# opensatelliteproject/xritdemod

Measured on AMD Instinct MI355X. Metric: Msamples/s in -> soft-symbols/s out (LRIT 293 ksym/s chain); % HBM roofline, higher is better.
Workload: dtype f32

## Files before the change

xritdemod_amd/csrc/clock.hip:

```cpp
#include "kernels.h"

#include <cstdlib>
#include <type_traits>
#include "scan.h"
#include "newton.h"

namespace xrit {

static_assert(CLK_CTL_DONE == NEWTON_CTL_DONE && CLK_CTL_GATED == NEWTON_CTL_GATED && CLK_CTL_TAKEOVER == NEWTON_CTL_TAKEOVER,
              "the words newton.h shares keep their numbers");

constexpr float CLK_H_T = 0.0625f;
constexpr float CLK_H_W = 1e-3f;

struct ClockResult {
    unsigned long long n_symbols;
    long long ii_final;
    int terminal_chain;
    int ok;
};

__global__ void __launch_bounds__(256) clock_om_kernel(const float2 *__restrict__ x, double2 *__restrict__ X,
                                                       long long N, int nb, double inv_sps)
{
    const int wave = threadIdx.x >> 6, lane = threadIdx.x & 63;
    const long long b = (long long)blockIdx.x * 4 + wave;
    if (b >= nb) return;
    float sr = 0.f, si = 0.f;
    for (int i = lane; i < CLK_OM_BLOCK; i += 64) {
        long long j = b * CLK_OM_BLOCK + i;
        if (j < N) {
            float2 v = x[j];
            float p = v.x * v.x + v.y * v.y;
            double ph = (double)j * inv_sps;
            ph -= floor(ph);
            float sn, cs;
            sincosf(-6.28318530717958647692f * (float)ph, &sn, &cs);
            sr += p * cs;
            si += p * sn;
        }
    }
    for (int off = 32; off > 0; off >>= 1) {
        sr += __shfl_down(sr, off, 64);
        si += __shfl_down(si, off, 64);
    }
    if (lane == 0) X[b] = make_double2((double)sr, (double)si);
}

__device__ __forceinline__ double clk_wrap(double x) { return x - 2.0 * XR_PI_D * rint(x / (2.0 * XR_PI_D)); }

struct ClkUnwrapF {
    typedef double T;
    const double2 *X;
    double *cnt;
    int nb;
    double sps;
    double off;
    int BL;
    double rot;
    __device__ T identity() const { return 0.0; }
    __device__ T combine(const T &lo, const T &hi) const { return lo + hi; }
    __device__ double ang(long long b) const
    {
        double sr = 0, si = 0;
        for (long long q = b - 2; q <= b + 2; ++q)
            if (q >= 0 && q < nb) { sr += X[q].x; si += X[q].y; }
        return atan2(si, sr);
    }
    __device__ T reduce_run(long long i0, int n) const
    {
        double s = 0, prev = i0 == 0 ? rot : ang(i0 - 1);
        for (int k = 0; k < n; ++k) {
            const double cur = ang(i0 + k);
            s += clk_wrap(cur - prev);
            prev = cur;
        }
        return s;
    }
    __device__ void apply_run(long long i0, int n, const T &pre) const
    {
        double s = pre, prev = i0 == 0 ? rot : ang(i0 - 1);
        for (int k = 0; k < n; ++k) {
            const double cur = ang(i0 + k);
            s += clk_wrap(cur - prev);
            prev = cur;
            double cb = off + ((double)(i0 + k) + 0.5) * BL;
            cnt[i0 + k] = (cb + s / (2.0 * XR_PI_D) * sps) / sps;
        }
    }
};

__device__ __forceinline__ double clk_count_at(const double *cnt, int nb, double sps, double t, double off, int BL)
{
    double fb = (t - off) / BL - 0.5;
    int b = (int)floor(fb);
    b = max(0, min(nb - 2, b));
    if (nb < 2) return cnt[0] + (t - off - 0.5 * BL) / sps;
    double c0 = cnt[b], c1 = cnt[b + 1];
    return c0 + (c1 - c0) * (fb - b);
}

__global__ void clock_guess_kernel(const double *__restrict__ cnt, int nb, double sps, ClockState *__restrict__ S,
                                   const ClockState *__restrict__ carried, int K, int NS, float omega0,
                                   const float2 *__restrict__ x, const float *__restrict__ table, long long ni,
                                   double off, int BL, int *__restrict__ dirty, int *__restrict__ ctl, int ctl_words,
                                   int *__restrict__ terminal, int *__restrict__ written)
{
    int k = blockIdx.x * blockDim.x + threadIdx.x;
    if (blockIdx.x == 0) {
        for (int i = threadIdx.x; i < ctl_words; i += blockDim.x) ctl[i] = 0;
        if (threadIdx.x == 0) *terminal = 0x7fffffff;
        __syncthreads();
    }
    if (k >= K) return;
    dirty[k] = 1;
    written[k] = 0;
    ClockState s0 = carried[0];
    if (k == 0) { S[0] = s0; ctl[CLK_CTL_GATED] = 1; return; }
    double t0 = (double)s0.ii + (double)s0.mu;
    double ca = clk_count_at(cnt, nb, sps, t0, off, BL) + 3.0 / sps;
    double target = rint(ca) + (double)k * NS;
    double t = (target - cnt[0]) * sps + off + 0.5 * BL;
    for (int it = 0; it < 4; ++it) {
        double c = clk_count_at(cnt, nb, sps, t, off, BL);
        t += (target - c) * sps;
    }
    t -= 3.0;
    if (t < 0) t = 0;
    ClockState s;
    s.ii = (long long)floor(t);
    s.mu = (float)(t - floor(t));
    s.omega = omega0;
    s.p0 = cf32{0.f, 0.f}; s.p1 = cf32{0.f, 0.f};
    s.c0 = cf32{0.f, 0.f}; s.c1 = cf32{0.f, 0.f};
    for (int back = 2; back >= 1; --back) {
        double tb = t - back * (double)omega0;
        if (tb < 0) continue;
        long long ib = (long long)floor(tb);
        if (ib >= ni) continue;
        float mub = (float)(tb - floor(tb));
        int imu = (int)rintf(mub * (float)XR_MM_NSTEPS);
        const float *row = table + imu * XR_MM_NTAPS;
        float ar = 0.f, ai = 0.f;
        for (int q = 0; q < XR_MM_NTAPS; ++q) {
            float2 v = x[ib + q];
            ar += row[XR_MM_NTAPS - 1 - q] * v.x;
            ai += row[XR_MM_NTAPS - 1 - q] * v.y;
        }
        s.p1 = s.p0; s.c1 = s.c0;
        s.p0 = cf32{ar, ai};
        s.c0 = cf32{ar > 0.f ? 1.f : 0.f, ai > 0.f ? 1.f : 0.f};
    }
    S[k] = s;
}

struct ClockPolicy {
    ClockState *S;
    const ClockState *E;
    const float4 *J;
    int *dirty;
    const int *nrun;
    unsigned *cnt;
    float trust_t, trust_w, tol_t, tol_w;
    int min_passes;
    const float4 *jmean;
    float floor_sq;
    int relay_after;

    struct Elem { ClockState e, s; float4 j; int nrun; };
    __device__ float4 jac_of(long long k) const { return jmean ? jmean[0] : J[k]; }
    __device__ Elem fetch(long long k) const { return Elem{E[k], S[k + 1], jac_of(k), nrun[k]}; }
    __device__ bool active(const Elem &el) const { return el.nrun > 0; }
    __device__ void residual(const Elem &el, float &r1, float &r2, int &aux) const
    {
        float rt = clock_tdiff(el.e, el.s);
        float m = rintf(rt / el.e.omega);
        r1 = rt - m * el.e.omega;
        r2 = el.e.omega - el.s.omega;
        aux = (int)m;
    }
    __device__ float4 jac(const Elem &el) const
    {
        float4 j = el.j;
        if (!(fabsf(j.x) < 4.f) || !(fabsf(j.y) < 16384.f) || !(fabsf(j.z) < 1.f) || !(fabsf(j.w) < 4.f))
            j = make_float4(0.f, 0.f, 0.f, 0.f);
        return j;
    }
    __device__ bool outside_trust(float d1, float d2) const
    {
        return !(fabsf(d1) <= trust_t) || !(fabsf(d2) <= trust_w);
    }
    __device__ bool distrust(float r1, float) const { return !(fabsf(r1) <= 0.5f); }
    __device__ void update(long long k, const Elem &el, float j1, float j2, float n1, float n2, int slip, int slip_k,
                           float r1, NewtonStat &st) const
    {
        const ClockState ek = el.e, old = el.s;
        const bool hist_same = ek.p0.x == old.p0.x && ek.p0.y == old.p0.y && ek.p1.x == old.p1.x &&
                               ek.p1.y == old.p1.y && ek.c0.x == old.c0.x && ek.c0.y == old.c0.y &&
                               ek.c1.x == old.c1.x && ek.c1.y == old.c1.y;
        if (!active(el)) {
            const bool same = old.ii == ek.ii && old.mu == ek.mu && old.omega == ek.omega && hist_same;
            if (!same) { S[k + 1] = ek; dirty[k + 1] = 1; st.changed += 1; }
            return;
        }
        const bool frozen = fabsf(n1) <= tol_t && fabsf(n2) <= tol_w && slip == 0 && slip_k == 0 && hist_same;
        if (frozen) return;
        ClockState nw = ek;
        clock_shift(nw, (float)slip * ek.omega + j1);
        nw.omega = ek.omega + j2;
        if (nw.ii < 0) { nw.ii = 0; nw.mu = 0.f; }
        st.open_ += 1;
        st.max_r = fmaxf(st.max_r, fabsf(r1));
        if (fabsf(r1) > 0.02f || slip_k != 0) st.large += 1;
        st.sum_sq += newton_fix(r1 * r1);
        const bool same = old.ii == nw.ii && old.mu == nw.mu && old.omega == nw.omega && hist_same;
        if (!same) { S[k + 1] = nw; dirty[k + 1] = 1; st.changed += 1; }
    }
    __device__ void decide(int *ctl) const
    {
        const unsigned changed = newton_cnt_load(cnt + CLK_CNT_CHANGED), open_ = newton_cnt_load(cnt + CLK_CNT_OPEN);
        const unsigned mr = newton_cnt_load(cnt + CLK_CNT_MAX_R), large = newton_cnt_load(cnt + CLK_CNT_LARGE);
        const unsigned long long sq = (unsigned long long)newton_cnt_load(cnt + CLK_CNT_SUM_SQ) |
                                      ((unsigned long long)newton_cnt_load(cnt + CLK_CNT_SUM_SQ + 1) << 32);
        ctl[CLK_CTL_PASSES] += 1;
        ctl[CLK_CTL_OPEN] = (int)open_;
        ctl[CLK_CTL_MAX_RESIDUAL] = (int)mr;
        const float q = newton_unfix(sq);
        const float q_prev = ctl[CLK_CTL_PASSES] == 1 ? INFINITY : __int_as_float(ctl[CLK_CTL_SUM_SQ]);
        ctl[CLK_CTL_SUM_SQ] = __float_as_int(q);
        ctl[CLK_CTL_GATED] = (large != 0 || __uint_as_float(mr) > 0.02f) ? 1 : 0;
        ctl[CLK_CTL_LARGE] = (int)large;
        const int open_prev = ctl[CLK_CTL_PASSES] == 1 ? 0x7fffffff : ctl[CLK_CTL_OPEN_LAST];
        ctl[CLK_CTL_OPEN_LAST] = (int)open_;
        if (changed == 0) { ctl[CLK_CTL_DONE] = 1; ctl[CLK_CTL_OPEN] = 0; return; }
        if (relay_after > 0 && ctl[CLK_CTL_PASSES] >= relay_after && large == 0 && !(__uint_as_float(mr) > 0.02f)) { ctl[CLK_CTL_DONE] = 1; return; }
        int memo = ctl[CLK_CTL_STALL_MEMO];
        if (ctl[CLK_CTL_PASSES] >= 3 && large != 0) memo |= 0x100;
        const bool acquiring = (memo & 0x100) != 0;
        const bool above_floor = open_ != 0u && (acquiring || q > floor_sq * (float)open_);
        const bool freezing = above_floor && open_prev != 0x7fffffff && (long long)open_prev - (long long)open_ >= 1 &&
                              200ll * ((long long)open_prev - (long long)open_) >= (long long)open_prev;
        const bool flat = q > 0.55f * q_prev;
        const int flat_runs = flat ? (memo & 0xff) + 1 : 0;
        ctl[CLK_CTL_STALL_MEMO] = (memo & 0x100) | (flat_runs > 0xff ? 0xff : flat_runs);
        const bool stalled = !freezing && (open_ >= 4096u ? flat : flat_runs >= 2);
        if (ctl[CLK_CTL_PASSES] >= min_passes && large == 0 && stalled) ctl[CLK_CTL_DONE] = 1;
    }
};

#ifndef XR_NOSTORE
#define XR_NOSTORE 0
#endif
#ifndef XR_LOAD_AUX
#define XR_LOAD_AUX 0
#endif

struct ClockTile {
    float *table;
    int *wb;
    float2 *tile;
    float2 *dump;
};

__device__ __forceinline__ ClockTile clock_tile_carve(char *smem, int grp, int ngroups, int WS)
{
    ClockTile t;
    t.table = reinterpret_cast<float *>(smem);
    t.wb = reinterpret_cast<int *>(smem + 4160) + 64 * grp;
    float2 *tiles = reinterpret_cast<float2 *>(smem + 4160 + 256 * ngroups);
    t.tile = tiles + (size_t)grp * 64 * WS;
    t.dump = tiles + (size_t)ngroups * 64 * WS + threadIdx.x;
    return t;
}

struct ClockSrc {
    __amdgpu_buffer_rsrc_t rsrc;
    int omin;
};
__device__ __forceinline__ ClockSrc clock_src(const float2 *x, long long N, int omin)
{
    ClockSrc c;
    omin = __builtin_amdgcn_readfirstlane(omin);
    c.omin = omin;
    const long long left = (N - (long long)omin) * 8;
    const unsigned bytes = left <= 0 ? 0u : (left > 0xffffffffLL ? 0xffffffffu : (unsigned)left);
    c.rsrc = __builtin_amdgcn_make_buffer_rsrc((void *)(x + omin), 0, bytes, 0x00020000);
    return c;
}

template <int NV, int IT> struct ClockFill {
    unsigned gb[IT];
    int lc[IT];
    typedef unsigned v2u __attribute__((ext_vector_type(2)));
    v2u v[IT];
    __device__ __forceinline__ void prepare(const int *origin, int nc, int WS, int omin)
    {
        const int lane = threadIdx.x & 63, wave = NV > 1 ? threadIdx.x >> 6 : 0;
        const int magic = 65536 / nc + 1;
#pragma unroll
        for (int it = 0; it < IT; ++it) {
            const int e = (it * NV + wave) * 64 + lane;
            const int row = (e * magic) >> 16, col = e - row * nc;
            const bool ok = row < 64 && origin[min(row, 63)] >= 0;
            gb[it] = ok ? (unsigned)(origin[min(row, 63)] - omin + col) * 8u : 0u;
            lc[it] = ok ? ((row * WS) << 8) | col : -1;
        }
    }
    __device__ __forceinline__ void issue(int first, const ClockSrc &src)
    {
#pragma unroll
        for (int it = 0; it < IT; ++it) v[it] = __builtin_amdgcn_raw_buffer_load_b64(src.rsrc, gb[it], first * 8, XR_LOAD_AUX);
    }
    template <int R> __device__ __forceinline__ void commit(float2 *tile, float2 *dump, int first, int ncol) const
    {
#pragma unroll
        for (int it = 0; it < IT; ++it) {
            const bool ok = (unsigned)(lc[it] & 255) < (unsigned)ncol && lc[it] >= 0;
            const int slot = (first + lc[it]) & (R - 1);
            float2 *p = tile + (lc[it] >> 8) + slot;
            const float2 val = make_float2(__uint_as_float(v[it].x), __uint_as_float(v[it].y));
            *(ok ? p : dump) = val;
            if (CLK_MIR > 0) *((ok && slot < CLK_MIR) ? p + R : dump) = val;
        }
    }
};

__device__ __forceinline__ int clock_cum(int jj, int STEP) { return (int)(((long long)jj * STEP) >> 16); }

template <int R>
__device__ __forceinline__ cf32 clock_step_ring(const cf32 *row, int &off, const float *table, ClockState &s,
                                                const ClockPar &par)
{
    cf32 wl[XR_MM_NTAPS];
    const cf32 *w = row + (off & (R - 1));
    if (CLK_MIR == 0) {
#pragma unroll
        for (int k = 0; k < XR_MM_NTAPS; ++k) wl[k] = row[(off + k) & (R - 1)];
        w = wl;
    }
    ClockState t = s;
    t.ii = 0;
    cf32 p = clock_step_w(w, table, t, par);
    off += (int)t.ii;
    t.ii = s.ii;
    s = t;
    return p;
}

__device__ __forceinline__ void clock_table_to_lds(float *dst, const float *__restrict__ src)
{
    constexpr int NEL = (XR_MM_NSTEPS + 1) * XR_MM_NTAPS;
    constexpr int NIT = (NEL + 63) / 64;
    const int nthr = blockDim.x;
    float tv[NIT];
#pragma unroll
    for (int q = 0; q < NIT; ++q) tv[q] = src[min((int)threadIdx.x + q * nthr, NEL - 1)];
#pragma unroll
    for (int q = 0; q < NIT; ++q) {
        const int i = (int)threadIdx.x + q * nthr;
        if (i < NEL) dst[i] = tv[q];
    }
}

}
#include "clock_relay.h"
namespace xrit {
struct ClockResult;
__device__ __forceinline__ double clk_count_at(const double *cnt, int nb, double sps, double t, double off, int BL);
}
#include "clock_overlap.h"
#ifdef XRIT_EXPERIMENTS
#include "../../experiments/csrc/clock_relay_wide.h"
#else
namespace xrit { constexpr int RW_REC_PAD = 0; }
#endif
namespace xrit {

__device__ __forceinline__ void clock_put(cf32 &d, const cf32 &p) { d = p; }
__device__ __forceinline__ void clock_put(float &d, const cf32 &p) { d = p.x; }

template <int WP, bool OUT, typename OutT>
__device__ __forceinline__ void clock_substep(const ClockTile &t, const float2 *__restrict__ x, int WS, int lane,
                                              int origin, int cum, int lim, int SS, int A, long long ni,
                                              const ClockPar &par, ClockState &s, int &off, bool &alive,
                                              int &produced, OutT *orow)
{
    const int rel = off - cum;
    const bool safe = !alive || (lim == SS && rel >= 0 && rel + A + XR_MM_NTAPS <= WP &&
                                 (long long)origin + off + A < ni);
    if (__all(safe)) {
        if (alive) {
            const cf32 *rowp = reinterpret_cast<const cf32 *>(t.tile + lane * WS);
            if (SS == 4) {
#pragma unroll
                for (int i = 0; i < 4; ++i) {
                    cf32 p = clock_step_ring<WP>(rowp, off, t.table, s, par);
                    if (OUT) clock_put(orow[i], p);
                }
            } else {
                for (int i = 0; i < SS; ++i) {
                    cf32 p = clock_step_ring<WP>(rowp, off, t.table, s, par);
                    if (OUT) {
#pragma unroll
                        for (int q = 0; q < 4; ++q)
                            if (q == i) clock_put(orow[q], p);
                    }
                }
            }
            s.ii = (long long)origin + off;
            produced += SS;
        }
    } else {
        for (int i = 0; i < lim; ++i) {
            if (alive && (s.ii >= ni || s.ii < 0)) alive = false;
            if (alive) {
                cf32 p = clock_step_w(reinterpret_cast<const cf32 *>(x) + s.ii, t.table, s, par);
                if (OUT) {
#pragma unroll
                    for (int q = 0; q < 4; ++q)
                        if (q == i) clock_put(orow[q], p);
                }
                ++produced;
            }
        }
        off = (int)(s.ii - origin);
    }
}

template <int NV> __device__ __forceinline__ void clock_tile_barrier()
{
    if (NV > 1) lds_barrier();
    else __builtin_amdgcn_wave_barrier();
}

template <int NV, int WP, int IT, typename Compute>
__device__ __forceinline__ void clock_pipeline(const ClockTile &t, const ClockSrc &src, int WS, int nsub, int STEP,
                                               Compute &&compute)
{
    {
        ClockFill<NV, (WP + NV - 1) / NV> w;
        w.prepare(t.wb, WP, WS, src.omin);
        w.issue(0, src);
        w.template commit<WP>(t.tile, t.dump, 0, WP);
    }
    const int nc = (STEP >> 16) + 1;
    if constexpr (IT * NV > 32) {
        ClockFill<NV, IT> f;
        f.prepare(t.wb, nc, WS, src.omin);
        clock_tile_barrier<NV>();
        int c0 = 0;
        for (int j = 0; j < nsub; ++j) {
            const int c1 = clock_cum(j + 1, STEP);
            if (j + 1 < nsub) f.issue(c0 + WP, src);
            compute(j, c0);
            clock_tile_barrier<NV>();
            if (j + 1 < nsub) f.template commit<WP>(t.tile, t.dump, c0 + WP, c1 - c0);
            clock_tile_barrier<NV>();
            c0 = c1;
        }
        return;
    }
    ClockFill<NV, IT> f0, f1;
    f0.prepare(t.wb, nc, WS, src.omin);
#pragma unroll
    for (int it = 0; it < IT; ++it) { f1.gb[it] = f0.gb[it]; f1.lc[it] = f0.lc[it]; }
    clock_tile_barrier<NV>();
    int c0 = 0, c1 = clock_cum(1, STEP);
    if (nsub > 1) f1.issue(c0 + WP, src);
    for (int j = 0; j < nsub; j += 2) {
        const int c2 = clock_cum(j + 2, STEP), c3 = clock_cum(j + 3, STEP);
        if (j + 2 < nsub) f0.issue(c1 + WP, src);
        compute(j, c0);
        clock_tile_barrier<NV>();
        if (j + 1 < nsub) f1.template commit<WP>(t.tile, t.dump, c0 + WP, c1 - c0);
        clock_tile_barrier<NV>();
        if (j + 1 >= nsub) break;
        if (j + 3 < nsub) f1.issue(c2 + WP, src);
        compute(j + 1, c1);
        clock_tile_barrier<NV>();
        if (j + 2 < nsub) f0.template commit<WP>(t.tile, t.dump, c1 + WP, c2 - c1);
        clock_tile_barrier<NV>();
        c0 = c2;
        c1 = c3;
    }
}

__device__ __forceinline__ int clock_origin_min(const int *wb)
{
    int o = wb[threadIdx.x & 63];
    o = o < 0 ? 0x7fffffff : o;
    for (int off = 32; off > 0; off >>= 1) o = min(o, __shfl_xor(o, off, 64));
    return o == 0x7fffffff ? 0 : o;
}

struct ClockPassOut {
    float *soft;
    float2 *sym;
    unsigned long long cap;
    int *valid;
    int *written;
    float4 *stage;
};

template <int NV, int WP, int NCM, bool OUTP = false>
__global__ void __launch_bounds__(NV > 1 ? 64 * NV : 512) clock_pass_kernel(const float2 *__restrict__ x, const float *__restrict__ table_g,
                                                             const ClockState *__restrict__ S, ClockState *__restrict__ E,
                                                             float4 *__restrict__ J, int *__restrict__ dirty,
                                                             int *__restrict__ nrun, long long N, long long ni, int K,
                                                             int NS, ClockPar par, int SS, int W, int WS, int A,
                                                             int STEP, const int *__restrict__ ctl, ClockPolicy pol,
                                                             AffMap *__restrict__ aggs, ClockPassOut po = ClockPassOut{})
{
    if (ctl[CLK_CTL_DONE] || (aggs != nullptr && ctl[CLK_CTL_TAKEOVER])) return;
    if (OUTP && blockIdx.x == 0 && threadIdx.x == 0) *po.valid = 1;
    extern __shared__ __attribute__((aligned(16))) char smem[];
    __shared__ float2 endv[2][NV > 1 ? 64 : 1];
    __shared__ long long ref_ii[NV > 1 ? 64 : 1];
    __shared__ int any_run;
    const int ngroups = NV > 1 ? 1 : (int)(blockDim.x >> 6);
    const int variant = NV > 1 ? threadIdx.x >> 6 : 0, grp = NV > 1 ? 0 : threadIdx.x >> 6, lane = threadIdx.x & 63;
    const ClockTile t = clock_tile_carve(smem, grp, ngroups, WS);
    const int wv = blockIdx.x * ngroups + grp;
    const int k = wv * 64 + lane;
    bool run = k < K;
    if (run) run = dirty[k] != 0 || (OUTP && po.written[k] == 0);
    if (threadIdx.x == 0) any_run = 0;
    __syncthreads();
    if (run && variant == 0) any_run = 1;
    clock_table_to_lds(t.table, table_g);
    __syncthreads();
    if (!any_run && aggs == nullptr) return;
    ClockState s{};
    int produced = 0;
    float4 jk = make_float4(0.f, 0.f, 0.f, 0.f);
    const bool walk = NV > 1 ? any_run != 0 : __any(run);
    if (walk) {
        bool alive = run;
        if (run) {
            s = S[k];
            if (NV > 1 && variant == 1) clock_shift(s, CLK_H_T);
            if (NV > 1 && variant == 2) s.omega += CLK_H_W;
        }
        if (variant == 0) t.wb[lane] = alive ? max((int)s.ii - CLK_M, 0) : -1;
        if (NV > 1) __syncthreads();
        else __builtin_amdgcn_wave_barrier();
        const int origin = t.wb[lane];
        int off = (int)(s.ii - origin);
        const int nsub = (NS + SS - 1) / SS;
        const ClockSrc src = clock_src(x, N, clock_origin_min(t.wb));
        const unsigned long long obase = (unsigned long long)k * NS;
        clock_pipeline<NV, WP, (NCM + NV - 1) / NV>(t, src, WS, nsub, STEP, [&](int j, int cum) {
            if (!OUTP) {
                clock_substep<WP, false>(t, x, WS, lane, origin, cum, min(SS, NS - j * SS), SS, A, ni, par, s, off, alive,
                                         produced, (float *)nullptr);
                return;
            }
            cf32 ps[4];
#pragma unroll
            for (int i = 0; i < 4; ++i) ps[i] = cf32{0.f, 0.f};
            const int before = produced;
            clock_substep<WP, true>(t, x, WS, lane, origin, cum, min(SS, NS - j * SS), SS, A, ni, par, s, off, alive,
                                    produced, ps);
            const int nv = produced - before;
            const unsigned long long o = obase + (unsigned long long)j * SS;
            if (po.soft && run) po.stage[((size_t)wv * nsub + j) * 64 + lane] = make_float4(ps[0].x, ps[1].x, ps[2].x, ps[3].x);
            if (nv == 4 && (NS & 3) == 0 && o + 3 < po.cap) {
                if (po.sym) {
                    *reinterpret_cast<float4 *>(po.sym + o) = make_float4(ps[0].x, ps[0].y, ps[1].x, ps[1].y);
                    *reinterpret_cast<float4 *>(po.sym + o + 2) = make_float4(ps[2].x, ps[2].y, ps[3].x, ps[3].y);
                }
            } else {
#pragma unroll
                for (int i = 0; i < 4; ++i) {
                    if (i < nv && o + i < po.cap) {
                        if (po.sym) po.sym[o + i] = make_float2(ps[i].x, ps[i].y);
                    }
                }
            }
        });
        if (NV > 1) {
            if (variant == 0) ref_ii[lane] = s.ii;
            __syncthreads();
            if (variant > 0) endv[variant - 1][lane] = make_float2((float)(s.ii - ref_ii[lane]) + s.mu, s.omega);
            __syncthreads();
        }
        if (variant == 0 && run) {
            if (NV > 1) {
                float2 et = endv[0][lane], ew = endv[1][lane];
                float tb = s.mu;
                jk.x = (et.x - tb) / CLK_H_T;
                jk.y = (ew.x - tb) / CLK_H_W;
                jk.z = (et.y - s.omega) / CLK_H_T;
                jk.w = (ew.y - s.omega) / CLK_H_W;
                J[k] = jk;
            }
            E[k] = s;
            nrun[k] = produced;
            dirty[k] = 0;
            if (OUTP) po.written[k] = 1;
        }
    }
    if (aggs == nullptr || variant != 0 || wv * 64 >= K) return;
    AffMap e = aff_identity();
    if (k < K - 1) {
        ClockPolicy::Elem el;
        el.s = S[k + 1];
        if (run) {
            el.e = s;
            el.nrun = produced;
            el.j = NV > 1 ? jk : pol.jac_of(k);
        } else {
            el.e = E[k];
            el.nrun = nrun[k];
            el.j = pol.jac_of(k);
        }
        e = newton_element(pol, el, false);
    }
    newton_wave_aggregate(e, wv, aggs);
}

template <int WP, int NCM, bool SYM>
__global__ void __launch_bounds__(512) clock_output_kernel(const float2 *__restrict__ x, const float *__restrict__ table_g,
                                                          const ClockState *__restrict__ S, ClockState *__restrict__ E,
                                                          int *__restrict__ counts, float *__restrict__ soft,
                                                          float2 *__restrict__ sym, unsigned long long cap, long long N,
                                                          long long ni, int K, int NS, ClockPar par,
                                                          int *__restrict__ terminal, int SS, int W, int WS, int A,
                                                          int STEP, const int *__restrict__ ctl)
{
    if (ctl[CLK_CTL_SYMBOLS]) return;
    extern __shared__ __attribute__((aligned(16))) char smem[];
    const int ngroups = (int)(blockDim.x >> 6), grp = threadIdx.x >> 6, lane = threadIdx.x & 63;
    const ClockTile t = clock_tile_carve(smem, grp, ngroups, WS);
    clock_table_to_lds(t.table, table_g);
    __syncthreads();
    const int k = (blockIdx.x * ngroups + grp) * 64 + lane;
    const bool mine = k < K;
    if (!__any(mine)) return;
    ClockState s{};
    if (mine) s = S[k];
    int produced = 0;
    bool alive = mine;
    t.wb[lane] = alive ? max((int)s.ii - CLK_M, 0) : -1;
    __builtin_amdgcn_wave_barrier();
    const int origin = t.wb[lane];
    int off = (int)(s.ii - origin);
    const int nsub = (NS + SS - 1) / SS;
    const ClockSrc src = clock_src(x, N, clock_origin_min(t.wb));
    const unsigned long long obase = (unsigned long long)k * NS;
    clock_pipeline<1, WP, NCM>(t, src, WS, nsub, STEP, [&](int j, int cum) {
        cf32 ps[4];
#pragma unroll
        for (int i = 0; i < 4; ++i) ps[i] = cf32{0.f, 0.f};
        const int before = produced;
        clock_substep<WP, true>(t, x, WS, lane, origin, cum, min(SS, NS - j * SS), SS, A, ni, par, s, off, alive,
                                produced, ps);
        const int nv = produced - before;
        const unsigned long long o = obase + (unsigned long long)j * SS;
        if (nv == 4 && (NS & 3) == 0 && SS == 4 && o + 3 < cap) {
            if (soft && !XR_NOSTORE) *reinterpret_cast<float4 *>(soft + o) = make_float4(ps[0].x, ps[1].x, ps[2].x, ps[3].x);
            if (SYM && sym) {
                *reinterpret_cast<float4 *>(sym + o) = make_float4(ps[0].x, ps[0].y, ps[1].x, ps[1].y);
                *reinterpret_cast<float4 *>(sym + o + 2) = make_float4(ps[2].x, ps[2].y, ps[3].x, ps[3].y);
            }
        } else {
#pragma unroll
            for (int i = 0; i < 4; ++i) {
                if (i < nv && o + i < cap) {
                    if (soft) soft[o + i] = ps[i].x;
                    if (SYM && sym) sym[o + i] = make_float2(ps[i].x, ps[i].y);
                }
            }
        }
    });
    if (!mine) return;
    E[k] = s;
    counts[k] = produced;
    if (produced < NS) atomicMin(terminal, k);
}

constexpr int CLK_STAGE_MAX_NS = 512;
__global__ void __launch_bounds__(256) clock_unstage_kernel(const float4 *__restrict__ stage, float *__restrict__ soft,
                                                            const int *__restrict__ nrun, const int *__restrict__ ctl,
                                                            unsigned long long cap, int K, int NS)
{
    if (!ctl[CLK_CTL_SYMBOLS]) return;
    extern __shared__ __attribute__((aligned(16))) char smem[];
    float *tile = reinterpret_cast<float *>(smem);
    int *cnt = reinterpret_cast<int *>(tile + 64 * (NS + 1));
    const int wv = blockIdx.x, nsub = NS / 4;
    if (threadIdx.x < 64) cnt[threadIdx.x] = wv * 64 + (int)threadIdx.x < K ? nrun[wv * 64 + threadIdx.x] : 0;
    for (int e = threadIdx.x; e < nsub * 64; e += 256) {
        const float4 v = stage[(size_t)wv * nsub * 64 + e];
        const int j = e >> 6, c = e & 63;
        float *row = tile + c * (NS + 1) + 4 * j;
        row[0] = v.x; row[1] = v.y; row[2] = v.z; row[3] = v.w;
    }
    __syncthreads();
    const unsigned long long base = (unsigned long long)wv * 64 * NS;
    for (int e = threadIdx.x; e < 64 * NS; e += 256) {
        const int c = e / NS, i = e - c * NS;
        if (i < cnt[c] && base + e < cap) soft[base + e] = tile[c * (NS + 1) + i];
    }
}

__global__ void __launch_bounds__(256) clock_terminal_kernel(const int *__restrict__ nrun, const int *__restrict__ ctl,
                                                             int *__restrict__ terminal, int K, int NS)
{
    if (!ctl[CLK_CTL_SYMBOLS]) return;
    const int k = blockIdx.x * 256 + threadIdx.x;
    const bool short_ = k < K && nrun[k] < NS;
    const unsigned long long m = __ballot(short_);
    if (m && (threadIdx.x & 63) == 0) atomicMin(terminal, k + __builtin_ctzll(m));
}

__global__ void __launch_bounds__(1024) clock_finalize_kernel(const ClockState *__restrict__ E,
                                                              const int *__restrict__ counts_out,
                                                              const int *__restrict__ nrun,
                                                              const int *__restrict__ terminal,
                                                              const int *__restrict__ ctl,
                                                              const ClockState *__restrict__ carried_in,
                                                              ClockState *__restrict__ carried_out,
                                                              ClockResult *__restrict__ res,
                                                              const float2 *__restrict__ x,
                                                              float2 *__restrict__ tail_out, long long N, int K, int NS)
{
    __shared__ long long s_ii;
    const int *counts = ctl[CLK_CTL_SYMBOLS] ? nrun : counts_out;
    if (threadIdx.x == 0) {
        int k = *terminal;
        ClockState s;
        if (k < 0 || k >= K) {
            res->ok = 0;
            res->n_symbols = 0;
            res->terminal_chain = -1;
            s = carried_in[0];
        } else {
            res->ok = 1;
            res->terminal_chain = k;
            res->n_symbols = (unsigned long long)k * NS + (unsigned long long)counts[k];
            s = E[k];
        }
        long long ii = s.ii;
        if (ii > N) ii = N;
        if (ii < 0) ii = 0;
        res->ii_final = ii;
        s_ii = ii;
        s.ii = 0;
        carried_out[0] = s;
    }
    __syncthreads();
    const long long ii = s_ii;
    const long long carry = N - ii;
    if (threadIdx.x < carry) tail_out[threadIdx.x] = x[ii + threadIdx.x];
}

__global__ void __launch_bounds__(1024) clock_tail_kernel(const float2 *__restrict__ tail, float2 *__restrict__ x, int carry)
{
    if ((int)threadIdx.x < carry) x[threadIdx.x] = tail[threadIdx.x];
}

constexpr int CLK_SER_W = 2048;

__global__ void __launch_bounds__(64) clock_serial_kernel(const float2 *__restrict__ x, const float *__restrict__ table_g,
                                                          const ClockState *__restrict__ carried_in,
                                                          ClockState *__restrict__ carried_out,
                                                          ClockResult *__restrict__ res, float *__restrict__ soft,
                                                          float2 *__restrict__ sym, unsigned long long cap, long long N,
                                                          long long ni, ClockPar par, float2 *__restrict__ tail_out)
{
    __shared__ float table[(XR_MM_NSTEPS + 1) * XR_MM_NTAPS];
    __shared__ cf32 win[CLK_SER_W];
    clock_table_to_lds(table, table_g);
    const int lane = threadIdx.x;
    ClockState s = carried_in[0];
    long long base = -(long long)CLK_SER_W;
    unsigned long long oo = 0;
    __syncthreads();
    while (s.ii < ni && s.ii >= 0 && oo < cap) {
        if (s.ii < base || s.ii + XR_MM_NTAPS > base + CLK_SER_W) {
            __syncthreads();
            base = s.ii;
            for (int i = lane; i < CLK_SER_W; i += 64) {
                const long long j = base + i;
                const float2 v = x[j < N ? j : N - 1];
                win[i] = cf32{v.x, v.y};
            }
            __syncthreads();
        }
        ClockState t = s;
        t.ii = 0;
        const cf32 p = clock_step_w(win + (int)(s.ii - base), table, t, par);
        s.ii += t.ii;
        t.ii = s.ii;
        s = t;
        if (lane == 0) {
            if (soft) soft[oo] = p.x;
            if (sym) sym[oo] = make_float2(p.x, p.y);
        }
        ++oo;
    }
    long long ii = s.ii;
    if (ii > N) ii = N;
    if (ii < 0) ii = 0;
    if (lane == 0) {
        res->ok = (s.ii >= ni || s.ii < 0) ? 1 : 0;
        res->terminal_chain = 0;
        res->n_symbols = oo;
        res->ii_final = ii;
        ClockState c = s;
        c.ii = 0;
        carried_out[0] = c;
    }
    const long long carry = N - ii;
    for (long long i = lane; i < carry && i < 1024; i += 64) tail_out[i] = x[ii + i];
}


__global__ void clk_fill_int_kernel(int *p, int v, int n)
{
    int i = blockIdx.x * blockDim.x + threadIdx.x;
    if (i < n) p[i] = v;
}

__global__ void __launch_bounds__(256) clock_reset_kernel(unsigned *counters, int words, int *terminal)
{
    for (int i = threadIdx.x; i < words; i += 256) counters[i] = 0u;
    if (threadIdx.x == 0 && terminal) *terminal = 0x7fffffff;
}

__global__ void __launch_bounds__(256) clock_jmean_kernel(const float4 *__restrict__ J, int K, float4 *__restrict__ out)
{
    __shared__ double acc[4][256];
    __shared__ int cnt[256];
    const int k0 = K / 8, k1 = K - K / 8;
    double a = 0, b = 0, c = 0, d = 0;
    int n = 0;
    for (int k = k0 + (int)threadIdx.x; k < k1; k += 256) {
        const float4 j = J[k];
        if (fabsf(j.x) < 4.f && fabsf(j.y) < 16384.f && fabsf(j.z) < 1.f && fabsf(j.w) < 4.f) {
            a += j.x; b += j.y; c += j.z; d += j.w;
            ++n;
        }
    }
    acc[0][threadIdx.x] = a; acc[1][threadIdx.x] = b; acc[2][threadIdx.x] = c; acc[3][threadIdx.x] = d;
    cnt[threadIdx.x] = n;
    __syncthreads();
    for (int off = 128; off > 0; off >>= 1) {
        if ((int)threadIdx.x < off) {
            for (int q = 0; q < 4; ++q) acc[q][threadIdx.x] += acc[q][threadIdx.x + off];
            cnt[threadIdx.x] += cnt[threadIdx.x + off];
        }
        __syncthreads();
    }
    if (threadIdx.x == 0) {
        const double inv = cnt[0] > 0 ? 1.0 / cnt[0] : 0.0;
        out[0] = make_float4((float)(acc[0][0] * inv), (float)(acc[1][0] * inv), (float)(acc[2][0] * inv), (float)(acc[3][0] * inv));
        reinterpret_cast<int *>(out + 1)[0] = cnt[0];
    }
}

int ClockStage::init(float omega, float gain_omega, float mu, float gain_mu, float omega_rel_limit, int chain_syms,
                     int max_passes_)
{
    sps = omega;
    par.omega_mid = omega;
    par.omega_lim = omega * omega_rel_limit;
    par.gain_omega = gain_omega;
    par.gain_mu = gain_mu;
    mu0 = mu;
    NS = chain_syms > 0 ? (chain_syms < 32 ? 32 : chain_syms) : 64;
    auto_ns = chain_syms <= 0;
    max_passes = max_passes_ > 0 ? max_passes_ : 192;
    min_passes = max_passes < 4 ? max_passes : 4;
    std::vector<float> tb((XR_MM_NSTEPS + 1) * XR_MM_NTAPS);
    design_mmse_table(tb.data());
    XR_TRY(table.reserve(tb.size() * sizeof(float)));
    XR_HIP(hipMemcpy(table.p, tb.data(), tb.size() * sizeof(float), hipMemcpyHostToDevice));
    XR_TRY(st.reserve(2 * sizeof(ClockState)));
    ClockState s0{};
    s0.ii = 0; s0.mu = mu; s0.omega = omega;
    ClockState both[2] = {s0, s0};
    XR_HIP(hipMemcpy(st.p, both, sizeof both, hipMemcpyHostToDevice));
    XR_TRY(tail.reserve(2 * 1024 * sizeof(float2)));
    XR_TRY(jmean.reserve(64));
    jmean_valid = false;
    XR_TRY(counters.reserve((size_t)(max_passes + 12) * 8 * sizeof(unsigned)));
    XR_HIP(hipHostMalloc((void **)&h_res, 128));
    {
        int dev = 0, v = 0;
        XR_HIP(hipGetDevice(&dev));
        if (hipDeviceGetAttribute(&v, hipDeviceAttributeMultiprocessorCount, dev) == hipSuccess && v > 0) cu_count = v;
        if (hipDeviceGetAttribute(&v, hipDeviceAttributeMaxSharedMemoryPerMultiprocessor, dev) == hipSuccess && v >= 65536)
            lds_per_cu = v;
    }
    ov_enabled = getenv("XRIT_NO_OVERLAP") == nullptr;
    if (const char *e = getenv("XRIT_OV_HIST")) { const int v = atoi(e); if (v >= 1024) ov_hist = v; }
#ifdef XRIT_EXPERIMENTS
    if (const char *e = getenv("XRIT_OV_MIN")) { const long long v = atoll(e); if (v > 0) ov_min = v; }
    if (const char *e = getenv("XRIT_OV_SMALL_RING")) ov_small_ring = atoi(e) != 0;
    if (const char *e = getenv("XRIT_OV_MINL")) { const int v = atoi(e); if (v >= 1024) ov_min_range = v; }
    if (const char *e = getenv("XRIT_OV_MINW")) { const int v = atoi(e); if (v >= 1) ov_min_walkers = v; }
    if (const char *e = getenv("XRIT_OV_LRATIO")) { const double v = atof(e); if (v >= 0.125 && v <= 16.0) ov_lratio = v; }
#endif
    {
        ov_pad_need = clock_ov_pad_need(*this);
        xpad = clock_xpad(*this);
        XR_TRY(ov_claim.reserve(RELAY_CLAIM_WORDS * sizeof(unsigned)));
        XR_HIP(hipMemset(ov_claim.p, 0, RELAY_CLAIM_WORDS * sizeof(unsigned)));
        for (auto &j : ov)
            if (hipEventCreateWithFlags(&j.ev_walk, hipEventDisableTiming) != hipSuccess ||
                hipEventCreateWithFlags(&j.ev_guess, hipEventDisableTiming) != hipSuccess) { set_error("hipEventCreate failed"); return XRIT_E_HIP; }
    }
    force_gated = getenv("XRIT_GATED_SOLVE") != nullptr;
    relay_global = getenv("XRIT_RELAY_GLOBAL") != nullptr;
    trace_env = getenv("XRIT_TRACE") != nullptr;
#ifdef XRIT_EXPERIMENTS
    if (const char *e = getenv("XRIT_NO_HANDOFF")) relay_no_handoff = atoi(e) != 0 ? 1 : 0;
    if (const char *e = getenv("XRIT_RELAY_WAVES")) relay_waves = atoi(e);
    if (const char *e = getenv("XRIT_RELAY_TEAMS")) relay_teams_per_cu = atoi(e) > 0 ? atoi(e) : 1;
    relay_no_rec = getenv("XRIT_RELAY_NO_REC") != nullptr;
    relay_no_claim = getenv("XRIT_RELAY_NO_CLAIM") != nullptr;
    if (const char *e = getenv("XRIT_RELAY_REC01")) relay_rec01 = atoi(e) != 0;
    if (const char *e = getenv("XRIT_RELAY_APX")) { int a0 = -1, a1 = -1; if (sscanf(e, "%d,%d", &a0, &a1) >= 1) { relay_apx_cfg[0] = a0; relay_apx_cfg[1] = a1; } }
    if (const char *e = getenv("XRIT_AUTO_PASSES")) auto_passes = atoi(e);
    if (const char *e = getenv("XRIT_AUTO_LONG_SEG")) auto_long_seg = atoi(e);
    if (const char *e = getenv("XRIT_RELAY_PER_CU")) { relay_per_cu = atoi(e) > 0 ? atoi(e) : 3; relay_per_cu_set = true; }
    no_meanj = getenv("XRIT_NO_MEANJ") != nullptr;
    pass_writes = getenv("XRIT_NO_PASS_OUTPUT") == nullptr;
    ng_max = getenv("XRIT_CLOCK_NG") ? atoi(getenv("XRIT_CLOCK_NG")) : 8;
#endif
    return XRIT_OK;
}

__global__ void clock_state_reset_kernel(ClockState *st, float mu, float omega)
{
    ClockState s{};
    s.ii = 0; s.mu = mu; s.omega = omega;
    st[0] = s;
    st[1] = s;
}

int ClockStage::reset(hipStream_t s)
{
    hipLaunchKernelGGL(clock_state_reset_kernel, dim3(1), dim3(1), 0, s, st.as<ClockState>(), mu0, par.omega_mid);
    jobs.reset();
    if (ov_claim.p) (void)hipMemsetAsync(ov_claim.p, 0, RELAY_CLAIM_WORDS * sizeof(unsigned), s);
    passes = 0;
    last_passes = -1;
    batch = 7;
    relay_batch = 96;
    jmean_valid = false;
    last_symbols = 0;
    return XRIT_OK;
}

void ClockStage::release()
{
#ifdef XRIT_RELAY_TIMING
    if (getenv("XRIT_WALKER_PHASES")) {
        unsigned long long hd[16] = {0}, z[16] = {0};
        if (hipDeviceSynchronize() == hipSuccess && hipMemcpyFromSymbol(hd, HIP_SYMBOL(relay_dbg), sizeof hd) == hipSuccess && hd[6]) {
            (void)hipMemcpyToSymbol(HIP_SYMBOL(relay_dbg), z, sizeof z);
            const double st = (double)hd[6];
            fprintf(stderr, "[xrit] overlap walkers over the handle's life, cycles per step: ring wait %.0f, setup %.0f, guess rounds %.0f, literal step + verdict %.0f, "
                            "stage + commit %.0f, loop %.0f; sum %.0f (%llu steps; the ring's fill level read %.3f times per step, %.3f sleeps per step)\n", hd[0] / st, hd[1] / st, hd[2] / st, hd[3] / st, hd[4] / st,
                    hd[5] / st, (hd[0] + hd[1] + hd[2] + hd[3] + hd[4] + hd[5]) / st, hd[6], hd[7] / st, hd[8] / st);
        }
    }
#endif
    for (auto &b : xbuf) b.release();
    for (auto &j : ov) {
        j.om.release(); j.om_work.release(); j.segs.release(); j.S.release(); j.stage.release(); j.aux.release();
        if (j.ev_walk) (void)hipEventDestroy(j.ev_walk);
        if (j.ev_guess) (void)hipEventDestroy(j.ev_guess);
        j.ev_walk = nullptr; j.ev_guess = nullptr;
    }
    ov_claim.release();
    table.release(); st.release(); S.release(); E.release(); J.release(); om.release();
    work.release(); counters.release(); sym.release(); dlin.release(); flags.release(); tail.release(); wsolve.release(); jmean.release();
    relay.release(); relay_rec.release(); alt.release(); stage.release(); om_work.release();
    if (h_res) (void)hipHostFree(h_res);
    h_res = nullptr;
}

double2 *ClockStage::om_slot(int nb, int BL)
{
    const int owner = jobs.om_owner();
    DevBuf &buf = owner >= 0 ? ov[owner].om : om;
    if (nb < 1 || buf.reserve((size_t)nb * (sizeof(double2) + sizeof(double))) != XRIT_OK) return nullptr;
    jobs.om_noted(nb, BL);
    return buf.as<double2>();
}

static int clock_unwrap(DevBuf &buf, DevBuf &wk, int nb, int BL, double sps, hipStream_t s)
{
    const int nbB = scan_blocks(nb);
    XR_TRY(wk.reserve((size_t)(nbB + 2) * sizeof(double)));
    double2 *X = buf.as<double2>();
    double *cnt = reinterpret_cast<double *>(buf.as<char>() + (size_t)nb * sizeof(double2));
    ClkUnwrapF uf{X, cnt, nb, sps, 0.0, BL, 0.0};
    hipLaunchKernelGGL(scan_reduce_kernel<ClkUnwrapF>, dim3(nbB), dim3(SCAN_BLOCK), 0, s, uf, (long long)nb, wk.as<double>());
    hipLaunchKernelGGL(scan_apply_lookback_kernel<ClkUnwrapF>, dim3(nbB), dim3(SCAN_BLOCK), 0, s, uf, (long long)nb, wk.as<double>());
    XR_HIP(hipGetLastError());
    return XRIT_OK;
}

int ClockStage::om_scan(hipStream_t s)
{
    if (!jobs.om_scan_here()) return XRIT_OK;
    XR_TRY(clock_unwrap(om, om_work, jobs.om_nb, jobs.om_BL, (double)sps, s));
    jobs.om_scan_done();
    return XRIT_OK;
}

int ClockStage::input_slot(size_t n, float2 **slot, hipStream_t s)
{
    const ClockSlotPick p = jobs.pick_buffer();
    if (p.b < 0) { set_error("%s", p.err); return XRIT_E_INVALID; }
    for (int q = 0; q < NXB; ++q)
        if (p.wait_guess[q]) XR_HIP(hipStreamWaitEvent(s, ov[q].ev_guess, 0));
    if (p.forget) jobs.hist.forget();
    XR_TRY(xbuf[p.b].reserve((xpad + n + 64 + 16) * sizeof(float2)));
    *slot = xbuf[p.b].as<float2>() + xpad;
    jobs.hand_out(p.b, n, ov_eligible(n));
    return XRIT_OK;
}

static inline int *clock_ctl(const DevBuf &b) { return b.as<int>(); }
static inline ClockResult *clock_res(const DevBuf &b) { return reinterpret_cast<ClockResult *>(b.as<unsigned>() + CLK_RES_WORD); }
static inline unsigned *clock_cnt(const DevBuf &b, int pass) { return b.as<unsigned>() + CLK_CTL_WORDS + (size_t)pass * CLK_CNT_WORDS; }

template <typename KernelT> static void clock_allow_lds(KernelT kernel, size_t bytes)
{
    if (bytes > 48 * 1024)
        (void)hipFuncSetAttribute(reinterpret_cast<const void *>(kernel), hipFuncAttributeMaxDynamicSharedMemorySize, (int)bytes);
}

__global__ void __launch_bounds__(256) clock_relay_finalize_kernel(const RelaySeg *__restrict__ e0,
                                                                    const RelaySeg *__restrict__ e1,
                                                                    const unsigned *__restrict__ changed, int enq, int G,
                                                                    int Lseg, const ClockState *__restrict__ carried_in,
                                                                    ClockState *__restrict__ carried_out,
                                                                    ClockResult *__restrict__ res,
                                                                    const float2 *__restrict__ x,
                                                                    float2 *__restrict__ tail_out, long long N, int *ctl, int force,
                                                                    const unsigned long long *__restrict__ moments)
{
    if (!ctl[CLK_CTL_DONE] && !force) return;
    __shared__ int s_term, s_buf, s_stuck;
    __shared__ long long s_ii;
    if (threadIdx.x == 0) {
        int ran = enq, closed = 0;
        for (int p = 0; p < enq; ++p)
            if (changed[RELAY_STAT * p + RELAY_STAT_CHANGED] == 0u) { ran = p + 1; closed = 1; break; }
        ctl[CLK_CTL_RELAY_PASSES] = ran;
        ctl[CLK_CTL_RELAY_CLOSED] = closed;
        {
            const unsigned *c = changed + RELAY_STAT * (ran - 1);
            const unsigned long long sq = (unsigned long long)c[RELAY_STAT_MOVE_SQ] | ((unsigned long long)c[RELAY_STAT_MOVE_SQ + 1] << 32);
            ctl[CLK_CTL_RELAY_SHIFT_SQ] = __float_as_int(c[RELAY_STAT_MOVED] ? (float)((double)sq / 1099511627776.0 / (double)c[RELAY_STAT_MOVED]) : 0.0f);
            ctl[CLK_CTL_RELAY_MOVE_MAX] = (int)(c[RELAY_STAT_MOVE_MAX] >= 0x80000000u ? 0x7f800000u : c[RELAY_STAT_MOVE_MAX]);
        }
        s_buf = (ran - 1) & 1;
        s_term = 0x7fffffff;
        s_stuck = 0;
    }
    __syncthreads();
    const RelaySeg *e = s_buf ? e1 : e0;
    for (int i = threadIdx.x; i < G; i += (int)blockDim.x) {
        if (e[i].flags & RELAY_EXHAUSTED) atomicMin(&s_term, i);
        if (e[i].flags & RELAY_STUCK) s_stuck = 1;
    }
    __syncthreads();
    if (threadIdx.x == 0) {
        ClockState s;
        const int k = s_stuck ? G : s_term;
        ctl[CLK_CTL_STUCK] = s_stuck;
        if (k >= G) {
            res->ok = 0;
            res->n_symbols = 0;
            res->terminal_chain = -1;
            s = carried_in[0];
        } else {
            res->ok = 1;
            res->terminal_chain = k;
            res->n_symbols = (unsigned long long)k * (unsigned long long)Lseg + (unsigned long long)e[k].n_done;
            s = e[k].s;
        }
        {
            const double nsym = res->ok ? (double)res->n_symbols : 0.0;
            const double a1 = nsym > 0 ? (double)moments[0] / 1048576.0 / nsym : 0.0, a2 = nsym > 0 ? (double)moments[1] / 1048576.0 / nsym : 0.0;
            const double var = a2 - a1 * a1;
            ctl[CLK_CTL_SNR2] = __float_as_int(nsym > 0 && var > 0 ? (float)(a1 * a1 / var) : 1e30f);
        }
        long long ii = s.ii;
        if (ii > N) ii = N;
        if (ii < 0) ii = 0;
        res->ii_final = ii;
        s_ii = ii;
        s.ii = 0;
        carried_out[0] = s;
    }
    __syncthreads();
    const long long ii = s_ii;
    long long carry = N - ii;
    if (carry > 1024) {
        carry = 1024;
        if (threadIdx.x == 0) res->ok = 0;
    }
    for (long long i = threadIdx.x; i < carry; i += blockDim.x) tail_out[i] = x[ii + i];
}

int ClockStage::relay_w_plan() const
{
#ifdef XRIT_EXPERIMENTS
    if (!relay_global && relay_waves >= 2) {
        if (relay_waves >= 4 && relay_span(par, RW_OWN * 4) + 8 <= RelayWide<4>::MAX_SPAN) return 4;
        if (relay_span(par, RW_OWN * 2) + 8 <= RelayWide<2>::MAX_SPAN) return 2;
    }
#endif
    return 0;
}

int ClockStage::relay_cut()
{
    Job &j = job;
    j.cps = j.segs.cps;
    j.G = j.segs.G;
    XR_TRY(relay.reserve((size_t)j.G * 3 * sizeof(RelaySeg) + ((size_t)j.G + 1 + 8) * RELAY_STAT * sizeof(unsigned) + 2 * sizeof(unsigned long long) +
                         RELAY_CLAIM_WORDS * sizeof(unsigned)));
    if (!relay_no_rec) XR_TRY(relay_rec.reserve(((size_t)j.G * j.cps * NS + RW_REC_PAD) * sizeof(unsigned)));
    relay_segments = j.G;
    relay_seg_chains = j.cps;
    return XRIT_OK;
}

int ClockStage::enqueue_relay(int count, bool restart, hipStream_t s, Profiler *prof)
{
    Job &j = job;
    const int limit = clock_relay_limit(j.G, j.relay_budget);
    RelaySeg *segs = relay.as<RelaySeg>();
    unsigned *changed = reinterpret_cast<unsigned *>(segs + 3 * (size_t)j.G);
    RelayArgs a{};
    a.x = xbase(); a.table = table.as<float>(); a.N = j.N; a.ni = j.ni;
    a.first = st.as<ClockState>() + jobs.cur; a.S = S.as<ClockState>();
    a.K = j.K; a.cps = j.cps; a.NS = NS; a.G = j.G;
    a.start = segs; a.ends[0] = segs + j.G; a.ends[1] = segs + 2 * (size_t)j.G;
    const ClockLattice lat = clock_lattice(par.omega_mid);
    a.q_om = lat.q_om; a.q_mu = lat.q_mu;
    a.soft = j.soft; a.sym = j.sym; a.cap = (unsigned long long)j.cap; a.par = par;
    a.changed = changed; a.ctl = j.relay_force ? nullptr : clock_ctl(counters);
    a.rec = relay_no_rec ? nullptr : relay_rec.as<unsigned>();
    a.moments = reinterpret_cast<unsigned long long *>(changed + ((size_t)j.G + 1 + 8) * RELAY_STAT);
    a.simd_claim = relay_no_claim ? nullptr : reinterpret_cast<unsigned *>(a.moments + 2);

    if (restart) {
        j.relay_enq = 0;
        const int words = RELAY_STAT * (j.G + 3) > RELAY_CLAIM_WORDS ? RELAY_STAT * (j.G + 3) : RELAY_CLAIM_WORDS;
        hipLaunchKernelGGL(clock_relay_init_kernel, dim3(div_up((size_t)words, 256)), dim3(256), 0, s, segs, j.G, changed,
                           j.G + 3, clock_ctl(counters), a.moments, a.simd_claim);
    }
    const int span = relay_span(par, 64);
    const bool lds_walk = relay_ring_ok(par) && !relay_global;
    {
        ProfScope ps(prof, "clock_relay", s);
        for (int q = 0; q < count && j.relay_enq < limit; ++q, ++j.relay_enq) {
            const int apx = j.relay_enq < 2 ? j.relay_apx[j.relay_enq] : 0;
            a.sym_skip = j.no_handoff && j.relay_enq == 0 && limit >= 2 && !apx;
            a.rec_write = relay_rec01 || !(j.no_handoff && j.relay_enq == 0);
            a.rec_use = (relay_rec01 || !(j.no_handoff && j.relay_enq == 1)) ? 3 : 0;
#ifdef XRIT_EXPERIMENTS
#define XR_RELAY_WIDE(WV)                                                                                             \
    do {                                                                                                              \
        const int wspan = relay_span(par, RW_OWN * WV);                                                               \
        if (j.sym) hipLaunchKernelGGL((clock_relay_wide_kernel<true, WV>), dim3(j.G), dim3(64 * WV), 0, s, a, j.relay_enq, wspan);       \
        else hipLaunchKernelGGL((clock_relay_wide_kernel<false, WV>), dim3(j.G), dim3(64 * WV), 0, s, a, j.relay_enq, wspan);            \
    } while (0)
            if (j.relay_w == 4) XR_RELAY_WIDE(4);
            else if (j.relay_w == 2) XR_RELAY_WIDE(2);
            else
#undef XR_RELAY_WIDE
#endif
            if (lds_walk && j.sym) hipLaunchKernelGGL((clock_relay_kernel<true, true>), dim3(j.G), dim3(128), 0, s, a, j.relay_enq, span, apx);
            else if (lds_walk) hipLaunchKernelGGL((clock_relay_kernel<false, true>), dim3(j.G), dim3(128), 0, s, a, j.relay_enq, span, apx);
            else if (j.sym) hipLaunchKernelGGL((clock_relay_kernel<true, false>), dim3(j.G), dim3(64), 0, s, a, j.relay_enq, span, apx);
            else hipLaunchKernelGGL((clock_relay_kernel<false, false>), dim3(j.G), dim3(64), 0, s, a, j.relay_enq, span, apx);
        }
        hipLaunchKernelGGL(clock_relay_finalize_kernel, dim3(1), dim3(64), 0, s, a.ends[0], a.ends[1], changed,
                           j.relay_enq, j.G, j.cps * NS, st.as<ClockState>() + jobs.cur, st.as<ClockState>() + (jobs.cur ^ 1),
                           clock_res(counters), a.x, tail.as<float2>() + 1024 * (jobs.cur ^ 1), j.N, clock_ctl(counters), j.relay_force ? 1 : 0,
                           a.moments);
    }
    XR_HIP(hipGetLastError());
    XR_HIP(hipMemcpyAsync(h_res, counters.p, CLK_CTL_WORDS * sizeof(unsigned), hipMemcpyDeviceToHost, s));
    return XRIT_OK;
}

int ClockStage::enqueue_passes(int count, hipStream_t s, Profiler *prof)
{
    const Job &j = job;
    ClockPolicy pol{S.as<ClockState>(), E.as<ClockState>(), J.as<float4>(), j.dirty, j.nrun, nullptr,
                    0.75f, 0.01f, tol_t, tol_w, min_passes, j.mean_j ? jmean.as<float4>() : nullptr,
                    9e-8f * (sps > 4.2534f ? (sps / 4.2534f) * (sps / 4.2534f) : 1.0f),
                    j.relay && (long long)j.cps * NS >= 2048 ? 2 : 0};
    const unsigned nw = div_up((size_t)j.K, 64);
    const float2 *x = xbase();
    const bool wave = !job.gated;
    AffMap *aggs = wave ? wsolve.as<AffMap>() : nullptr;
    NewtonStat *wslots = reinterpret_cast<NewtonStat *>(wsolve.as<AffMap>() + nw + 1);
    for (int q = 0; q < count && job.enqueued < max_passes; ++q, ++job.enqueued) {
        const int p = job.enqueued;
        pol.cnt = clock_cnt(counters, p);
        const bool jac = p < jac_passes && !j.mean_j;
        {
            ProfScope ps(prof, jac ? "clock_pass_jac" : "clock_pass", s);
#define XR_CLK_PASS(NV, WPV, NCM, OUTV)                                                                               \
    do {                                                                                                              \
        const size_t lds = NV > 1 ? j.tile_bytes3 : j.tile_bytes;                                                     \
        clock_allow_lds(clock_pass_kernel<NV, WPV, NCM, OUTV>, lds);                                                  \
        hipLaunchKernelGGL((clock_pass_kernel<NV, WPV, NCM, OUTV>), dim3(NV > 1 ? nw : div_up(nw, j.NG)),             \
                           dim3(NV > 1 ? 64 * NV : 64 * j.NG), lds, s, x, table.as<float>(), S.as<ClockState>(),      \
                           E.as<ClockState>(), J.as<float4>(), j.dirty, j.nrun, j.N, j.ni, j.K, NS, par, j.SS, j.W,   \
                           j.WS, j.A, j.STEP, clock_ctl(counters), pol, aggs, po);                                    \
    } while (0)
#define XR_CLK_PASS_NV(NV, OUTV)                                                                                      \
    do {                                                                                                              \
        if (!j.wide && narrow) XR_CLK_PASS(NV, 32, 20, OUTV);                                                         \
        else if (!j.wide) XR_CLK_PASS(NV, 32, 32, OUTV);                                                              \
        else XR_CLK_PASS(NV, 64, 64, OUTV);                                                                           \
    } while (0)
            const bool narrow = (j.STEP >> 16) + 1 <= 20;
            const bool writes = !jac && !j.relay && p >= j.write_from && j.SS == 4 && (NS & 3) == 0 && NS <= CLK_STAGE_MAX_NS;
            const ClockPassOut po{j.soft, j.sym, (unsigned long long)j.cap, clock_ctl(counters) + CLK_CTL_SYMBOLS, j.written,
                                  stage.as<float4>()};
            if (jac) XR_CLK_PASS_NV(3, false);
            else if (writes) XR_CLK_PASS_NV(1, true);
            else XR_CLK_PASS_NV(1, false);
#undef XR_CLK_PASS_NV
#undef XR_CLK_PASS
        }
        {
            ProfScope ps(prof, "clock_solve", s);
            if (wave) {
                newton_apply_waves(pol, (long long)j.K - 1, aggs, clock_ctl(counters), wslots, s);
            } else if (newton_solve(pol, (long long)j.K - 1, work.as<AffMap>(), dlin.as<float2>(), clock_ctl(counters), s) != 0) {
                set_error("clock hand-off: %d chains exceed the solver's block budget", j.K);
                return XRIT_E_INVALID;
            }
        }
    }
    XR_HIP(hipGetLastError());
    return XRIT_OK;
}

int ClockStage::enqueue_output(hipStream_t s, Profiler *prof, bool again)
{
    const Job &j = job;
    const float2 *x = xbase();
    const ClockState *st_in = st.as<ClockState>() + jobs.cur;
    ClockState *st_out = st.as<ClockState>() + (jobs.cur ^ 1);
    float2 *tail_out = tail.as<float2>() + 1024 * (jobs.cur ^ 1);
    const unsigned nw = div_up((size_t)j.K, 64);
    {
        ProfScope ps(prof, "clock_output", s);
        if (again) hipLaunchKernelGGL(clk_fill_int_kernel, dim3(1), dim3(1), 0, s, j.terminal, 0x7fffffff, 1);
#define XR_CLK_OUT_S(WPV, NCM, SYMV)                                                                                  \
    do {                                                                                                              \
        clock_allow_lds(clock_output_kernel<WPV, NCM, SYMV>, j.tile_bytes);                                           \
        hipLaunchKernelGGL((clock_output_kernel<WPV, NCM, SYMV>), dim3(div_up(nw, j.NG)), dim3(64 * j.NG),            \
                           j.tile_bytes, s, x, table.as<float>(), S.as<ClockState>(), E.as<ClockState>(), j.counts,   \
                           j.soft, j.sym, (unsigned long long)j.cap, j.N, j.ni, j.K, NS, par, j.terminal, j.SS, j.W,  \
                           j.WS, j.A, j.STEP, clock_ctl(counters));                                                   \
    } while (0)
#define XR_CLK_OUT(WPV, NCM)                              \
    do {                                                  \
        if (j.sym) XR_CLK_OUT_S(WPV, NCM, true);          \
        else XR_CLK_OUT_S(WPV, NCM, false);               \
    } while (0)
        const bool narrow = (j.STEP >> 16) + 1 <= 20;
        if (!j.wide && narrow) XR_CLK_OUT(32, 20);
        else if (!j.wide) XR_CLK_OUT(32, 32);
        else XR_CLK_OUT(64, 64);
#undef XR_CLK_OUT_S
#undef XR_CLK_OUT
        if (j.soft && j.SS == 4 && (NS & 3) == 0 && pass_writes && NS <= CLK_STAGE_MAX_NS) {
            const size_t lds = (size_t)64 * (NS + 1) * sizeof(float) + 64 * sizeof(int);
            clock_allow_lds(clock_unstage_kernel, lds);
            hipLaunchKernelGGL(clock_unstage_kernel, dim3(nw), dim3(256), lds, s, stage.as<float4>(), j.soft, j.nrun,
                               clock_ctl(counters), (unsigned long long)j.cap, j.K, NS);
        }
        hipLaunchKernelGGL(clock_terminal_kernel, dim3(div_up((size_t)j.K, 256)), dim3(256), 0, s, j.nrun, clock_ctl(counters),
                           j.terminal, j.K, NS);
        hipLaunchKernelGGL(clock_finalize_kernel, dim3(1), dim3(1024), 0, s, E.as<ClockState>(), j.counts, j.nrun, j.terminal,
                           clock_ctl(counters), st_in, st_out, clock_res(counters), x, tail_out, j.N, j.K, NS);
    }
    XR_HIP(hipGetLastError());
    XR_HIP(hipMemcpyAsync(h_res, counters.p, CLK_CTL_WORDS * sizeof(unsigned), hipMemcpyDeviceToHost, s));
    return XRIT_OK;
}


static inline unsigned *ov_stat(ClockStage::OvJob &d) { return d.aux.as<unsigned>(); }
static inline unsigned long long *ov_moments(ClockStage::OvJob &d) { return reinterpret_cast<unsigned long long *>(d.aux.as<unsigned>() + 8); }
static inline unsigned long long *ov_offs(ClockStage::OvJob &d) { return reinterpret_cast<unsigned long long *>(d.aux.as<char>() + 64); }
static inline int *ov_j0(ClockStage::OvJob &d, int G) { return reinterpret_cast<int *>(d.aux.as<char>() + 64 + (size_t)G * sizeof(unsigned long long)); }

int ClockStage::ov_launch(int job, hipStream_t sw, bool ahead, Profiler *prof)
{
    const ClockJob &j = jobs.job[job];
    OvJob &d = ov[job];
    const ClockLaunchHist h = jobs.launch_hist(job, ahead, ov_pad_need);
    if (h.err) { set_error("%s", h.err); return XRIT_E_INVALID; }
    if (h.wait_guess >= 0) XR_HIP(hipStreamWaitEvent(sw, ov[h.wait_guess].ev_guess, 0));
    size_t h_n = 0;
    {
        const ClockOvPlan plan = clock_ov_plan(*this, j.n, jobs.carry, h.have, ahead);
        if (plan.err[0]) { set_error("%s", plan.err); return XRIT_E_INVALID; }
        jobs.planned(job, plan, ahead);
        XR_TRY(d.segs.reserve((size_t)j.G * sizeof(OverlapSeg)));
        XR_TRY(d.S.reserve((size_t)j.G * sizeof(ClockState)));
        XR_TRY(d.stage.reserve((size_t)j.G * (size_t)j.stride * sizeof(float) + 256));
        XR_TRY(d.aux.reserve(64 + (size_t)j.G * sizeof(int) + 8 + (size_t)j.G * sizeof(unsigned long long)));
    }
    float2 *data = xbuf[job].as<float2>() + xpad;
    float2 *base = data - j.padN;
    if (!j.w0_carried) {
        if (const char *e = ClockJobs::hist_refusal(h, j)) { set_error("%s", e); return XRIT_E_INVALID; }
        h_n = jobs.job[h.job].n;
        const float2 *hend = xbuf[h.xb].as<float2>() + xpad + h_n;
        XR_HIP(hipMemcpyAsync(base, hend - j.padN, (size_t)j.padN * sizeof(float2), hipMemcpyDeviceToDevice, sw));
    } else if (j.padN > 0) {
        hipLaunchKernelGGL(clock_tail_kernel, dim3(1), dim3(1024), 0, sw, tail.as<float2>() + 1024 * jobs.cur, base, j.padN);
    }
    int nb = j.nb;
    const int BL = j.om_ext ? j.BL : CLK_OM_BLOCK;
    if (!j.om_ext) {
        nb = (int)((j.n + CLK_OM_BLOCK - 1) / CLK_OM_BLOCK);
        XR_TRY(d.om.reserve((size_t)nb * (sizeof(double2) + sizeof(double))));
        hipLaunchKernelGGL(clock_om_kernel, dim3(div_up((size_t)nb, 4)), dim3(256), 0, sw, data, d.om.as<double2>(), (long long)j.n, nb,
                           1.0 / (double)sps);
    }
    if (!j.om_scanned && nb >= 1) XR_TRY(clock_unwrap(d.om, d.om_work, nb, BL, (double)sps, sw));
    const double *cnt = reinterpret_cast<const double *>(d.om.as<char>() + (size_t)nb * sizeof(double2));
    const double *cnt_prev = nullptr;
    int nb_prev = 0;
    if (!j.w0_carried && h.job >= 0) {
        const ClockJob &p = jobs.job[h.job];
        cnt_prev = reinterpret_cast<const double *>(ov[h.job].om.as<char>() + (size_t)p.nb * sizeof(double2));
        nb_prev = p.nb;
        if (p.BL != BL) { set_error("clock recovery: timing curves of consecutive calls differ in their block length"); return XRIT_E_INVALID; }
    }
    OverlapArgs a{};
    a.x = base; a.table = table.as<float>(); a.N = j.N; a.ni = j.ni;
    a.start = d.S.as<ClockState>(); a.G = j.G; a.store0 = j.store0; a.first_bound = j.first_bound; a.Ls = j.Ls; a.early = j.early;
    a.stride = j.stride; a.stage = d.stage.as<float>(); a.segs = d.segs.as<OverlapSeg>(); a.par = par;
    const ClockLattice lat = clock_lattice(par.omega_mid);
    a.q_om = lat.q_om; a.q_mu = lat.q_mu;
    a.stat = ov_stat(d); a.moments = ov_moments(d); a.simd_claim = relay_no_claim ? nullptr : ov_claim.as<unsigned>();
    const int span = relay_span(par, 64);
    {
        ProfScope ps(prof, "clock_guess", sw);
        hipLaunchKernelGGL(clock_overlap_guess_kernel, dim3(div_up((size_t)j.G, 256)), dim3(256), 0, sw, cnt, nb, cnt_prev, nb_prev,
                           (long long)h_n, BL, (double)sps, par.omega_mid, base, table.as<float>(), j.ni, j.padN, j.hist, j.G, j.store0,
                           j.first_bound, j.Ls, st.as<ClockState>() + jobs.cur, j.w0_carried ? 1 : 0, j.w0_ii, 0, d.S.as<ClockState>(),
                           a.stat, a.moments);
    }
    XR_HIP(hipEventRecord(d.ev_guess, sw));
    {
        ProfScope ps(prof, "clock_overlap", sw);
        if (ov_small_ring && span + 8 <= 1024 - RELAY_XCH - 72) hipLaunchKernelGGL(clock_overlap_kernel<1024>, dim3(j.G), dim3(128), 0, sw, a, span);
        else hipLaunchKernelGGL(clock_overlap_kernel<RELAY_RX>, dim3(j.G), dim3(128), 0, sw, a, span);
    }
    XR_HIP(hipGetLastError());
    XR_HIP(hipEventRecord(d.ev_walk, sw));
    jobs.launched(job, h, nb, BL);
    return XRIT_OK;
}

int ClockStage::ov_restart(int job)
{
    if (jobs.restart_waits(job)) XR_HIP(hipEventSynchronize(ov[job].ev_walk));
    jobs.restarted(job);
    return XRIT_OK;
}

int ClockStage::ov_fallback(size_t *n_out, hipStream_t s, Profiler *prof, bool to_closure)
{
    const int job = jobs.overlap_fell_back();
    const int rc = run_chains(xbuf[job].as<float2>() + xpad - jobs.carry, to_closure ? 1 : 0, jobs.job[job].n, ov_soft, nullptr, ov_cap, n_out, s, prof);
    if (rc == XRIT_OK) jobs.ended_fallback(job);
    ov_fell_back = true;
    return rc;
}

int ClockStage::ov_finalize(int job, float *soft_out, size_t cap, hipStream_t s, Profiler *prof)
{
    const ClockJob &j = jobs.job[job];
    OvJob &d = ov[job];
    XR_HIP(hipStreamWaitEvent(s, d.ev_walk, 0));
    jobs.w0_known(job);
    {
        ProfScope ps(prof, "clock_joints", s);
        hipLaunchKernelGGL(clock_reset_kernel, dim3(1), dim3(256), 0, s, counters.as<unsigned>(), CLK_CTL_WORDS, (int *)nullptr);
        hipLaunchKernelGGL(clock_overlap_scan_kernel, dim3(1), dim3(256), 0, s, d.segs.as<OverlapSeg>(), j.G, j.stride,
                           st.as<ClockState>() + jobs.cur, j.w0_ii, j.w0_carried ? 1 : 0, par.omega_mid, ov_j0(d, j.G), ov_offs(d),
                           st.as<ClockState>() + (jobs.cur ^ 1), clock_res(counters), xbuf[job].as<float2>() + xpad - j.padN,
                           tail.as<float2>() + 1024 * (jobs.cur ^ 1), j.N, clock_ctl(counters), ov_moments(d), (unsigned long long)cap);
        if (soft_out)
            hipLaunchKernelGGL(clock_overlap_copy_kernel, dim3(div_up((size_t)j.stride, 1024), j.G), dim3(256), 0, s, d.stage.as<float>(),
                               d.segs.as<OverlapSeg>(), ov_j0(d, j.G), ov_offs(d), j.stride, soft_out, (unsigned long long)cap, clock_res(counters));
    }
    XR_HIP(hipGetLastError());
    XR_HIP(hipMemcpyAsync(h_res, counters.p, CLK_CTL_WORDS * sizeof(unsigned), hipMemcpyDeviceToHost, s));
    jobs.finalizing(job);
    return XRIT_OK;
}

void ClockStage::call_reset(size_t n)
{
    passes = 0;
    unconverged = 0;
    large_open = 0;
    max_residual = 0;
    ov_fell_back = false;
    jobs.call_reset(n);
}

int ClockStage::begin(size_t n, float *soft_out, float2 *sym_out, size_t cap, hipStream_t s, Profiler *prof)
{
    call_reset(n);
    if (const char *e = jobs.call_job(n, sym_out != nullptr)) { set_error("%s", e); return XRIT_E_INVALID; }
    if (jobs.ov_cur >= 0) return begin_overlap(n, soft_out, cap, s, prof);
    return begin_chains(nullptr, exact, n, soft_out, sym_out, cap, s, prof);
}

int ClockStage::begin_overlap(size_t n, float *soft_out, size_t cap, hipStream_t s, Profiler *prof)
{
    job = Job{};
    job.n = n; job.soft = soft_out; job.cap = cap; job.exact = exact;
    jobs.begun_overlap();
    ov_soft = soft_out; ov_cap = cap;
    const int q = jobs.ov_cur;
    if (jobs.job[q].state == CLK_JOB_SLOT) XR_TRY(ov_launch(q, s, false, prof));
    return ov_finalize(q, soft_out, cap, s, prof);
}

int ClockStage::begin_chains(float2 *base, int exact_, size_t n, float *soft_out, float2 *sym_out, size_t cap, hipStream_t s, Profiler *prof)
{
    ClockKnobs k = *this;
    k.exact = exact_;
    const int relay_w = relay_w_plan();
    job = Job{};
    Job &j = job;
    static_cast<ClockChainPlan &>(j) = clock_chain_plan(k, n, jobs.carry, last_passes, relay_w);
    j.n = n; j.soft = soft_out; j.sym = sym_out; j.cap = cap; j.base = base; j.exact = exact_; j.relay_w = relay_w;
    if (j.N >= (1LL << 31)) { set_error("%s", j.err); return XRIT_E_INVALID; }
    jobs.chains_buffer(!base);
    if (!base) XR_TRY(xbuf[jobs.xb].reserve((size_t)(xpad + n + 64 + 16) * sizeof(float2)));
    const ClockOm om_in = jobs.begun_chains();
    if (jobs.carry)
        hipLaunchKernelGGL(clock_tail_kernel, dim3(1), dim3(1024), 0, s, tail.as<float2>() + 1024 * jobs.cur, xbase(), (int)jobs.carry);
    if (j.err[0]) { set_error("%s", j.err); return XRIT_E_INVALID; }
    if (j.short_input) return begin_short(s);
    if (serial) return begin_serial(s, prof);
    NS = j.NS;
    return launch_chains(om_in.ext, om_in.scanned, s, prof);
}

int ClockStage::begin_short(hipStream_t s)
{
    const Job &j = job;
    if (j.N > 0)
        XR_HIP(hipMemcpyAsync(tail.as<float2>() + 1024 * (jobs.cur ^ 1), xbase(), (size_t)j.N * sizeof(float2),
                              hipMemcpyDeviceToDevice, s));
    XR_HIP(hipMemcpyAsync(st.as<ClockState>() + (jobs.cur ^ 1), st.as<ClockState>() + jobs.cur, sizeof(ClockState),
                          hipMemcpyDeviceToDevice, s));
    return XRIT_OK;
}

int ClockStage::begin_serial(hipStream_t s, Profiler *prof)
{
    const Job &j = job;
    hipLaunchKernelGGL(clock_reset_kernel, dim3(1), dim3(256), 0, s, counters.as<unsigned>(), CLK_CTL_WORDS, (int *)nullptr);
    {
        ProfScope ps(prof, "clock_serial", s);
        hipLaunchKernelGGL(clock_serial_kernel, dim3(1), dim3(64), 0, s, xbase(), table.as<float>(),
                           st.as<ClockState>() + jobs.cur, st.as<ClockState>() + (jobs.cur ^ 1), clock_res(counters), j.soft,
                           j.sym, (unsigned long long)j.cap, j.N, j.ni, par, tail.as<float2>() + 1024 * (jobs.cur ^ 1));
    }
    XR_HIP(hipGetLastError());
    XR_HIP(hipMemcpyAsync(h_res, counters.p, CLK_CTL_WORDS * sizeof(unsigned), hipMemcpyDeviceToHost, s));
    return XRIT_OK;
}

int ClockStage::launch_chains(bool ext, bool scanned, hipStream_t s, Profiler *prof)
{
    Job &j = job;
    const int K = j.K;
    float2 *x = xbase();
    const int BL = ext ? jobs.om_BL : CLK_OM_BLOCK;
    const double om_off = ext ? (double)jobs.carry : 0.0;
    const int nb = ext ? jobs.om_nb : (int)((j.N + CLK_OM_BLOCK - 1) / CLK_OM_BLOCK);
    XR_TRY(S.reserve((size_t)K * sizeof(ClockState)));
    XR_TRY(E.reserve((size_t)K * sizeof(ClockState)));
    XR_TRY(J.reserve((size_t)K * sizeof(float4)));
    XR_TRY(flags.reserve((size_t)(4 * K + 4) * sizeof(int)));
    if (pass_writes) XR_TRY(stage.reserve(((size_t)div_up((size_t)K, 64) * 64 * NS + 64) * sizeof(float)));
    XR_TRY(om.reserve((size_t)nb * (sizeof(double2) + sizeof(double))));
    const int nbK = scan_blocks(K), nbB = scan_blocks(nb);
    const int nbmax = nbK > nbB ? nbK : nbB;
    XR_TRY(dlin.reserve((size_t)(K + 1) * sizeof(float2)));
    const int nbN = newton_blocks(K) > nbmax ? newton_blocks(K) : nbmax;
    XR_TRY(work.reserve((size_t)(3 * nbN + 8) * sizeof(AffMap)));
    {
        const size_t nw = div_up((size_t)K, 64);
        XR_TRY(wsolve.reserve(newton_waves_bytes(nw)));
        j.gated = force_gated;
        j.mean_j = jmean_valid && jmean_ns == NS && K >= 256 && !force_gated && !no_meanj;
    }
    if (j.relay) XR_TRY(relay_cut());
    j.dirty = flags.as<int>();
    j.counts = flags.as<int>() + K;
    j.nrun = flags.as<int>() + 2 * K;
    j.terminal = flags.as<int>() + 3 * K;
    j.written = flags.as<int>() + 3 * K + 4;
    double2 *X = om.as<double2>();
    double *cnt = reinterpret_cast<double *>(om.as<char>() + (size_t)nb * sizeof(double2));
    const ClockState *st_in = st.as<ClockState>() + jobs.cur;
    if (K <= 1) hipLaunchKernelGGL(clock_reset_kernel, dim3(1), dim3(256), 0, s, counters.as<unsigned>(), (max_passes + 5) * 8, j.terminal);
    if (K > 1) {
        {
            ProfScope ps(prof, "clock_guess", s);
            if (!ext)
                hipLaunchKernelGGL(clock_om_kernel, dim3(div_up((size_t)nb, 4)), dim3(256), 0, s, x, X, j.N, nb,
                                   1.0 / (double)sps);
            if (!scanned) XR_TRY(clock_unwrap(om, work, nb, BL, (double)sps, s));
            hipLaunchKernelGGL(clock_guess_kernel, dim3(div_up((size_t)K, 256)), dim3(256), 0, s, cnt, nb, (double)sps,
                               S.as<ClockState>(), st_in, K, NS, par.omega_mid, x, table.as<float>(), j.ni, om_off, BL, j.dirty,
                               clock_ctl(counters), (max_passes + 5) * 8, j.terminal, j.written);
        }
        if (j.no_handoff) j.relay_force = true;
        else XR_TRY(enqueue_passes(batch < max_passes ? batch : max_passes, s, prof));
    } else {
        XR_HIP(hipMemcpyAsync(S.p, st_in, sizeof(ClockState), hipMemcpyDeviceToDevice, s));
    }
    if (j.relay && K > 1) {
        if (before_relay) XR_TRY(before_relay(0));
        int rc_relay = enqueue_relay(relay_batch, true, s, prof);
        if (rc_relay == XRIT_OK && before_relay) rc_relay = before_relay(1);
        return rc_relay;
    }
    return enqueue_output(s, prof);
}

bool ClockStage::closed() const
{
    if (job.short_input || job.K <= 1 || job.no_handoff) return true;
    return reinterpret_cast<const int *>(h_res)[CLK_CTL_DONE] != 0;
}

int ClockStage::finish(size_t *n_out, hipStream_t s, Profiler *prof)
{
    *n_out = 0;
    jobs.call_ended();
    if (jobs.ov_cur >= 0) return finish_overlap(n_out, s, prof);
    if (job.short_input) {
        jobs.ended_short(job.N);
        last_symbols = 0;
        return XRIT_OK;
    }
    return finish_chains(n_out, s, prof);
}

int ClockStage::finish_overlap(size_t *n_out, hipStream_t s, Profiler *prof)
{
    const ClockJob &oj = jobs.job[jobs.ov_cur];
    const int *hc = reinterpret_cast<const int *>(h_res);
    ClockResult r;
    memcpy(&r, reinterpret_cast<const unsigned *>(h_res) + CLK_RES_WORD, sizeof r);
    snr_estimate = clock_ctl_float(hc, CLK_CTL_SNR2);
    ov_walkers = oj.G;
    ov_joint_max = clock_ctl_float(hc, CLK_CTL_OV_JOINT_MAX);
    relay_passes = 1;
    relay_closed = false;
    relay_auto = false;
    relay_segments = oj.G;
    relay_seg_chains = 0;
    passes = 0;
    unconverged = 0; max_residual = 0; large_open = 0;
    if (trace_env) XR_TRY(trace_overlap(jobs.ov_cur, r));
    const ClockOvVerdict v = clock_overlap_look(*this, hc);
    if (v == CLK_OV_WATCHDOG) { set_error("clock recovery: a walker gave up waiting for its sample ring (watchdog)"); (void)jobs.overlap_released(); return XRIT_E_HIP; }
    if (v != CLK_OV_TAKE) return ov_fallback(n_out, s, prof, v == CLK_OV_FALLBACK_TO_CLOSURE);
    const int jb = jobs.overlap_released();
    if (!r.ok) {
        if ((size_t)r.n_symbols > ov_cap) { set_error("clock recovery produced %zu symbols, capacity %zu", (size_t)r.n_symbols, ov_cap); return XRIT_E_CAPACITY; }
        set_error("clock recovery: the walkers did not reach the end of the input");
        return XRIT_E_INVALID;
    }
    jobs.flip();
    if (const char *e = jobs.carried(oj.N - r.ii_final)) { set_error("%s", e); return XRIT_E_INVALID; }
    last_symbols = (size_t)r.n_symbols;
    *n_out = last_symbols;
    jobs.ended_overlap(jb);
    return XRIT_OK;
}

int ClockStage::finish_handoff(hipStream_t s, Profiler *prof)
{
    const int *hctl = reinterpret_cast<const int *>(h_res);
    const int give_up = job.exact != -1 && max_passes > 48 ? 48 : max_passes;
    while (hctl[CLK_CTL_DONE] == 0 && job.enqueued < give_up) {
        if (hctl[CLK_CTL_TAKEOVER]) job.gated = true;
        XR_TRY(enqueue_passes(4, s, prof));
        XR_HIP(hipMemcpyAsync(h_res, counters.p, CLK_CTL_WORDS * sizeof(unsigned), hipMemcpyDeviceToHost, s));
        XR_HIP(hipStreamSynchronize(s));
    }
    job.relay_force = hctl[CLK_CTL_DONE] == 0;
    if (job.relay && job.K > 1) XR_TRY(enqueue_relay(relay_batch, true, s, prof));
    else XR_TRY(enqueue_output(s, prof, true));
    XR_HIP(hipStreamSynchronize(s));
    return XRIT_OK;
}

int ClockStage::finish_relay(hipStream_t s, Profiler *prof)
{
    const int *hctl = reinterpret_cast<const int *>(h_res);
    const ClockKnobs k = call_knobs();
    ClockRelayLook c;
    c.relay_force = job.relay_force; c.no_handoff = job.no_handoff; c.relay_long = job.relay_long; c.G = job.G;
    for (;;) {
        c.relay_auto = relay_auto; c.relay_enq = job.relay_enq; c.relay_budget = job.relay_budget;
        const ClockRelayStep v = clock_relay_look(k, hctl, c);
        c.first = false;
        relay_auto = v.relay_auto;
        job.relay_budget = v.relay_budget;
        if (v.snr_seen) snr_estimate = v.snr2;
        if (v.verdict == CLK_RELAY_TAKE || v.verdict == CLK_RELAY_NO_SIGNAL) break;
        if (v.verdict == CLK_RELAY_TO_CLOSURE) continue;
        XR_TRY(enqueue_relay(v.verdict == CLK_RELAY_FOUR_MORE ? 4 : (relay_batch < 32 ? 32 : relay_batch), false, s, prof));
        XR_HIP(hipStreamSynchronize(s));
    }
    relay_passes = hctl[CLK_CTL_RELAY_PASSES];
    relay_closed = hctl[CLK_CTL_RELAY_CLOSED] != 0;
    if (trace_env) XR_TRY(trace_relay());
    relay_batch = clock_next_relay_batch(relay_passes);
    return XRIT_OK;
}

int ClockStage::finish_chains(size_t *n_out, hipStream_t s, Profiler *prof)
{
    const int *hctl = reinterpret_cast<const int *>(h_res);
    const bool in_batch = closed();
    if (!in_batch) XR_TRY(finish_handoff(s, prof));
    relay_passes = 0;
    relay_closed = false;
    relay_auto = false;
    if (clock_handoff_to_closure(call_knobs(), hctl, job.K, job.relay)) {
        job.relay = relay_auto = true;
        job.relay_force = hctl[CLK_CTL_DONE] == 0;
        job.relay_budget = 0;
        job.segs = clock_relay_segments(call_knobs(), job.K, NS, job.no_handoff, job.relay_budget, job.relay_w);
        XR_TRY(relay_cut());
        XR_TRY(enqueue_relay(relay_batch, true, s, prof));
        XR_HIP(hipStreamSynchronize(s));
    }
    if (job.relay && job.K > 1) XR_TRY(finish_relay(s, prof));
    passes = job.K > 1 ? hctl[CLK_CTL_PASSES] : 0;
    if (job.K > 1) {
        last_passes = passes;
        batch = clock_next_batch(passes, job.relay);
    }
    if (job.K > 1) {
        const bool clean = in_batch && hctl[CLK_CTL_TAKEOVER] == 0 && hctl[CLK_CTL_LARGE] == 0 && passes <= 12;
        if (job.mean_j && !clean) jmean_valid = false;
        else if (!job.mean_j && !job.gated && clean && job.K >= 1024 && jac_passes > 0 && !job.no_handoff) {
            hipLaunchKernelGGL(clock_jmean_kernel, dim3(1), dim3(256), 0, s, J.as<float4>(), job.K, jmean.as<float4>());
            jmean_valid = true;
            jmean_ns = NS;
        }
    }
    unconverged = job.K > 1 ? (unsigned)hctl[CLK_CTL_OPEN] : 0;
    large_open = job.K > 1 ? (unsigned)hctl[CLK_CTL_LARGE] : 0;
    max_residual = clock_ctl_float(hctl, CLK_CTL_MAX_RESIDUAL);
    if (trace_env && job.K > 1) XR_TRY(trace_passes());
    ClockResult r;
    memcpy(&r, reinterpret_cast<const unsigned *>(h_res) + CLK_RES_WORD, sizeof r);
    jobs.flip();
    if (!r.ok && serial) {
        set_error("clock recovery produced more than the %zu symbols the output holds", job.cap);
        return XRIT_E_CAPACITY;
    }
    if (!r.ok && job.relay && hctl[CLK_CTL_STUCK]) {
        set_error("clock recovery: a relay walker gave up waiting for its sample ring or its team (watchdog)");
        return XRIT_E_HIP;
    }
    if (!r.ok) {
        set_error("clock recovery: chain budget exhausted before the end of the input");
        return XRIT_E_INVALID;
    }
    if (const char *e = jobs.carried(job.N - r.ii_final)) { set_error("%s", e); return XRIT_E_INVALID; }
    last_symbols = (size_t)r.n_symbols;
    *n_out = last_symbols;
    if (last_symbols > job.cap) {
        set_error("clock recovery produced %zu symbols, capacity %zu", last_symbols, job.cap);
        return XRIT_E_CAPACITY;
    }
    jobs.ended_chains(!job.base);
    return XRIT_OK;
}

int ClockStage::trace_overlap(int job, const ClockResult &r) const
{
    const ClockJob &oj = jobs.job[job];
    const int *hc = reinterpret_cast<const int *>(h_res);
    unsigned hs[8];
    XR_HIP(hipMemcpy(hs, ov[job].aux.p, sizeof hs, hipMemcpyDeviceToHost));
    fprintf(stderr, "[xrit] overlap: %d walkers over ranges of %d samples behind %d samples of history (%s), %u steps, %.2f guess rounds per step; "
                    "joints: %d do not fit, largest distance %.3e sample; 2 Es/N0 = %.1f; %llu symbols%s\n",
            oj.G, oj.Ls, oj.hist, oj.w0_carried ? "walker 0 from the carried state" : "walker 0 warms up in the burst before", hs[0],
            hs[0] ? (double)hs[1] / hs[0] : 0.0, hc[CLK_CTL_OV_BAD_JOINTS], (double)ov_joint_max, (double)snr_estimate, (unsigned long long)r.n_symbols, r.ok ? "" : " -- NOT taken");
#ifdef XRIT_RELAY_TIMING
    unsigned long long hd[16] = {0}, z[16] = {0};
    XR_HIP(hipMemcpyFromSymbol(hd, HIP_SYMBOL(relay_dbg), sizeof hd));
    XR_HIP(hipMemcpyToSymbol(HIP_SYMBOL(relay_dbg), z, sizeof z));
    const double st = hd[6] ? (double)hd[6] : 1.0;
    fprintf(stderr, "[xrit] overlap walkers, cycles per step: ring wait %.0f, setup %.0f, guess rounds %.0f, literal step + verdict %.0f, "
                    "stage + commit %.0f, loop %.0f; sum %.0f (%llu steps)\n", hd[0] / st, hd[1] / st, hd[2] / st, hd[3] / st, hd[4] / st,
            hd[5] / st, (hd[0] + hd[1] + hd[2] + hd[3] + hd[4] + hd[5]) / st, hd[6]);
#endif
    return XRIT_OK;
}

int ClockStage::trace_relay() const
{
    if (job.exact == 0) fprintf(stderr, "[xrit] relay: the first pass's soft symbols show 2 Es/N0 = %.1f (to closure below %.1f)\n", (double)snr_estimate, (double)auto_snr);
    std::vector<unsigned> hc((size_t)relay_passes * RELAY_STAT);
    const unsigned *changed = reinterpret_cast<const unsigned *>(relay.as<RelaySeg>() + 3 * (size_t)job.G);
    XR_HIP(hipMemcpy(hc.data(), changed, hc.size() * sizeof(unsigned), hipMemcpyDeviceToHost));
    for (int p = 0; p < relay_passes; ++p) {
        const unsigned *c = &hc[(size_t)RELAY_STAT * p];
        float mv;
        memcpy(&mv, &c[RELAY_STAT_MOVE_MAX], sizeof mv);
        const unsigned long long sq = (unsigned long long)c[RELAY_STAT_MOVE_SQ] | ((unsigned long long)c[RELAY_STAT_MOVE_SQ + 1] << 32);
        const bool mark = c[RELAY_STAT_MOVE_MAX] >= 0x80000000u;
        fprintf(stderr, "[xrit] relay pass %d: segments walked %u of %d, steps %u, rounds %u (%.2f per step); starts moved by %.3e sample rms, %.3e at most%s\n", p,
                c[RELAY_STAT_CHANGED], job.G, c[RELAY_STAT_STEPS], c[RELAY_STAT_ROUNDS], c[RELAY_STAT_STEPS] ? (double)c[RELAY_STAT_ROUNDS] / c[RELAY_STAT_STEPS] : 0.0,
                c[RELAY_STAT_MOVED] ? sqrt((double)sq / 1099511627776.0 / (double)c[RELAY_STAT_MOVED]) : 0.0,
                mark ? 0.0 : (double)mv, mark ? " (watchdog mark)" : "");
    }
#ifdef XRIT_RELAY_TIMING
    unsigned long long hd[16] = {0}, z[16] = {0};
    XR_HIP(hipMemcpyFromSymbol(hd, HIP_SYMBOL(relay_dbg), sizeof hd));
    XR_HIP(hipMemcpyToSymbol(HIP_SYMBOL(relay_dbg), z, sizeof z));
    std::vector<unsigned> wd((size_t)RELAY_WDBG_PASSES * RELAY_WDBG_SEGS * RELAY_WDBG_WORDS);
    XR_HIP(hipMemcpyFromSymbol(wd.data(), HIP_SYMBOL(relay_wdbg), wd.size() * sizeof(unsigned)));
    for (int p = 0; p < relay_passes && p < RELAY_WDBG_PASSES && job.relay_w == 0; ++p)
        for (int g = 0; g < job.G && g < RELAY_WDBG_SEGS; ++g) {
            const unsigned *w = &wd[((size_t)p * RELAY_WDBG_SEGS + g) * RELAY_WDBG_WORDS];
            fprintf(stderr, "[xrit] walker %d %d %u %u %u %u %u %u\n", p, g, w[0], w[1], w[2], w[3], w[4], w[5]);
        }
    if (job.relay_w > 0) {
        const double st = hd[7] ? (double)hd[7] : 1.0, un = hd[9] ? (double)hd[9] : 1.0;
        (void)un;
        fprintf(stderr, "[xrit] relay team (wave 1) cycles per step: rings %.0f, setup %.0f, interpolate..scan %.0f, meeting + sums %.0f, "
                        "positions..verdict %.0f, meeting + verdicts %.0f, commit + loop %.0f (%llu steps)\n",
                hd[0] / st, hd[1] / st, hd[2] / st, hd[3] / st, hd[4] / st, hd[5] / st, hd[6] / st, hd[7]);
    }
    for (int o = 0; o < 16 && job.relay_w == 0; o += 8) {
        const double st = hd[o + 6] ? (double)hd[o + 6] : 1.0;
        fprintf(stderr, "[xrit] relay walker cycles per step, passes %s: wait %.0f, setup %.0f, rounds %.0f, verify %.0f, commit %.0f, loop head %.0f (%llu steps)\n",
                o ? ">= 8" : "< 8", hd[o] / st, hd[o + 1] / st, hd[o + 2] / st, hd[o + 3] / st, hd[o + 4] / st, hd[o + 5] / st, hd[o + 6]);
    }
#endif
    return XRIT_OK;
}

int ClockStage::trace_passes() const
{
    std::vector<unsigned> hc((size_t)passes * CLK_CNT_WORDS);
    XR_HIP(hipMemcpy(hc.data(), clock_cnt(counters, 0), hc.size() * sizeof(unsigned), hipMemcpyDeviceToHost));
    for (int p = 0; p < passes; ++p) {
        const unsigned *c = &hc[(size_t)p * CLK_CNT_WORDS];
        float mr;
        unsigned long long qf;
        memcpy(&mr, &c[CLK_CNT_MAX_R], 4);
        memcpy(&qf, &c[CLK_CNT_SUM_SQ], 8);
        const float q = (float)((double)qf / 1099511627776.0);
        fprintf(stderr, "[xrit] clock pass %d: K=%d changed=%u open=%u max_r=%.3e large=%u rms_r=%.3e\n", p, job.K,
                c[CLK_CNT_CHANGED], c[CLK_CNT_OPEN], mr, c[CLK_CNT_LARGE], c[CLK_CNT_OPEN] ? sqrtf(q / c[CLK_CNT_OPEN]) : 0.f);
    }
    return XRIT_OK;
}

__global__ void __launch_bounds__(256) clock_negate_kernel(float2 *__restrict__ x, size_t n)
{
    const size_t i = (size_t)blockIdx.x * 256 + threadIdx.x;
    if (i < n) { float2 v = x[i]; x[i] = make_float2(-v.x, -v.y); }
}

__global__ void clock_flip_state_kernel(ClockState *st)
{
    ClockState s = st[0];
    s.p0 = cf32{-s.p0.x, -s.p0.y};
    s.p1 = cf32{-s.p1.x, -s.p1.y};
    s.c0 = cf32{s.p0.x > 0.f ? 1.f : 0.f, s.p0.y > 0.f ? 1.f : 0.f};
    s.c1 = cf32{s.p1.x > 0.f ? 1.f : 0.f, s.p1.y > 0.f ? 1.f : 0.f};
    st[0] = s;
}

int ClockStage::run(size_t n, float *soft_out, float2 *sym_out, size_t cap, size_t *n_out, hipStream_t s,
                    Profiler *prof)
{
    XR_TRY(begin(n, soft_out, sym_out, cap, s, prof));
    XR_HIP(hipStreamSynchronize(s));
    return finish(n_out, s, prof);
}

int ClockStage::run_chains(float2 *base, int exact_, size_t n, float *soft_out, float2 *sym_out, size_t cap, size_t *n_out, hipStream_t s, Profiler *prof)
{
    call_reset(n);
    XR_TRY(begin_chains(base, exact_, n, soft_out, sym_out, cap, s, prof));
    XR_HIP(hipStreamSynchronize(s));
    const int rc = finish(n_out, s, prof);
    job.base = nullptr;
    return rc;
}

static constexpr size_t CLK_ALT_SLOT = sizeof(ClockState) + 1024 * sizeof(float2);

int ClockStage::redo_flipped(float *soft_out, float2 *sym_out, size_t cap, size_t *n_out, hipStream_t s, Profiler *prof)
{
    *n_out = 0;
    if (!jobs.redo_ok) { set_error("clock recovery: no finished call to run again"); return XRIT_E_INVALID; }
    const bool from_alt = jobs.step_back_flipped();
    float2 *data = xdata();
    const size_t n = jobs.prev_n, carry = jobs.carry;
    if (from_alt) {
        XR_HIP(hipMemcpyAsync(st.as<ClockState>() + jobs.cur, alt.p, sizeof(ClockState), hipMemcpyDeviceToDevice, s));
        XR_HIP(hipMemcpyAsync(tail.as<float2>() + 1024 * jobs.cur, alt.as<char>() + sizeof(ClockState), 1024 * sizeof(float2),
                              hipMemcpyDeviceToDevice, s));
    } else {
        hipLaunchKernelGGL(clock_flip_state_kernel, dim3(1), dim3(1), 0, s, st.as<ClockState>() + jobs.cur);
        if (carry) hipLaunchKernelGGL(clock_negate_kernel, dim3(div_up(carry, 256)), dim3(256), 0, s, tail.as<float2>() + 1024 * jobs.cur, carry);
    }
    if (n) hipLaunchKernelGGL(clock_negate_kernel, dim3(div_up(n, 256)), dim3(256), 0, s, data, n);
    XR_HIP(hipGetLastError());
    return run_chains(data - carry, exact, n, soft_out, sym_out, cap, n_out, s, prof);
}

__global__ void __launch_bounds__(1024) clock_carry_pack_kernel(unsigned char *__restrict__ rec, const ClockState *__restrict__ st,
                                                                const float2 *__restrict__ tail, int carry)
{
    if (threadIdx.x == 0) {
        unsigned *h = reinterpret_cast<unsigned *>(rec);
        h[0] = 1u; h[1] = (unsigned)carry; h[2] = 0u; h[3] = 0u;
        *reinterpret_cast<ClockState *>(rec + 16) = *st;
    }
    float2 *t = reinterpret_cast<float2 *>(rec + ClockStage::CARRY_HEAD);
    t[threadIdx.x] = (int)threadIdx.x < carry ? tail[threadIdx.x] : make_float2(0.f, 0.f);
}

__global__ void __launch_bounds__(1024) clock_carry_unpack_kernel(const unsigned char *__restrict__ rec, ClockState *__restrict__ st,
                                                                  float2 *__restrict__ tail, int carry)
{
    if (threadIdx.x == 0) *st = *reinterpret_cast<const ClockState *>(rec + 16);
    const float2 *t = reinterpret_cast<const float2 *>(rec + ClockStage::CARRY_HEAD);
    if ((int)threadIdx.x < carry) tail[threadIdx.x] = t[threadIdx.x];
}

static_assert(16 + sizeof(ClockState) <= ClockStage::CARRY_HEAD, "the carried record's head holds a ClockState");

int ClockStage::export_carry(void *d_rec, int which, hipStream_t s)
{
    if (jobs.in_flight) { set_error("clock recovery: a call is in flight"); return XRIT_E_INVALID; }
    if (which != 0 && !jobs.redo_ok) { set_error("clock recovery: no finished call whose start state is still held"); return XRIT_E_INVALID; }
    const int slot = which == 0 ? jobs.cur : jobs.cur ^ 1;
    const size_t c = which == 0 ? jobs.carry : jobs.prev_carry;
    hipLaunchKernelGGL(clock_carry_pack_kernel, dim3(1), dim3(1024), 0, s, static_cast<unsigned char *>(d_rec), st.as<ClockState>() + slot,
                       tail.as<float2>() + 1024 * slot, (int)c);
    XR_HIP(hipGetLastError());
    return XRIT_OK;
}

bool ClockStage::last_walk_exact() const
{
    if (!jobs.redo_ok || jobs.ov_cur >= 0 || job.short_input) return false;
    return serial || (job.relay && (relay_closed || job.G == 1));
}

int ClockStage::redo_from(const void *d_rec, size_t carry_rec, float *soft_out, float2 *sym_out, size_t cap, size_t *n_out, hipStream_t s, Profiler *prof)
{
    *n_out = 0;
    if (!jobs.redo_ok) { set_error("clock recovery: no finished call to run again"); return XRIT_E_INVALID; }
    if (carry_rec > 1024) { set_error("clock recovery: a carried record with %zu unread samples", carry_rec); return XRIT_E_INVALID; }
    jobs.step_back_from(carry_rec);
    float2 *data = xdata();
    hipLaunchKernelGGL(clock_carry_unpack_kernel, dim3(1), dim3(1024), 0, s, static_cast<const unsigned char *>(d_rec), st.as<ClockState>() + jobs.cur,
                       tail.as<float2>() + 1024 * jobs.cur, (int)carry_rec);
    XR_HIP(hipGetLastError());
    return run_chains(data - carry_rec, exact, jobs.prev_n, soft_out, sym_out, cap, n_out, s, prof);
}

int ClockStage::make_alt(hipStream_t s, Profiler *prof)
{
    jobs.alt_valid = false;
    if (!jobs.redo_ok) { set_error("clock recovery: no finished call to run again"); return XRIT_E_INVALID; }
    XR_TRY(alt.reserve(2 * CLK_ALT_SLOT));
    char *keep = alt.as<char>() + CLK_ALT_SLOT;
    const size_t carry_keep = jobs.carry;
    XR_HIP(hipMemcpyAsync(keep, st.as<ClockState>() + jobs.cur, sizeof(ClockState), hipMemcpyDeviceToDevice, s));
    XR_HIP(hipMemcpyAsync(keep + sizeof(ClockState), tail.as<float2>() + 1024 * jobs.cur, 1024 * sizeof(float2), hipMemcpyDeviceToDevice, s));
    size_t k = 0;
    XR_TRY(redo_flipped(nullptr, nullptr, (size_t)1 << 40, &k, s, prof));
    XR_HIP(hipMemcpyAsync(alt.p, st.as<ClockState>() + jobs.cur, sizeof(ClockState), hipMemcpyDeviceToDevice, s));
    XR_HIP(hipMemcpyAsync(alt.as<char>() + sizeof(ClockState), tail.as<float2>() + 1024 * jobs.cur, 1024 * sizeof(float2), hipMemcpyDeviceToDevice, s));
    XR_HIP(hipMemcpyAsync(st.as<ClockState>() + jobs.cur, keep, sizeof(ClockState), hipMemcpyDeviceToDevice, s));
    XR_HIP(hipMemcpyAsync(tail.as<float2>() + 1024 * jobs.cur, keep + sizeof(ClockState), 1024 * sizeof(float2), hipMemcpyDeviceToDevice, s));
    jobs.alt_made(carry_keep);
    return XRIT_OK;
}

}
```

xritdemod_amd/csrc/clock_overlap.h:

```cpp
#pragma once

#include "clock_relay.h"

namespace xrit {

constexpr int OV_HEAD = 8;
constexpr int OV_EXHAUSTED = 2;
constexpr int OV_EMPTY = 4;
constexpr int OV_STUCK = 8;

struct OverlapSeg {
    ClockState end;
    int count;
    int flags;
    int head_ii[OV_HEAD];
    float head_mu[OV_HEAD];
    int pad_[2];
};
static_assert(sizeof(OverlapSeg) == 128, "OverlapSeg is a 128-byte record");

struct OverlapArgs {
    const float2 *x;
    const float *table;
    long long N, ni;
    const ClockState *start;
    int G;
    int store0;
    int first_bound, Ls;
    int early;
    int stride;
    float *stage;
    OverlapSeg *segs;
    ClockPar par;
    int q_om, q_mu;
    unsigned *stat;
    unsigned long long *moments;
    unsigned *simd_claim;
};

__device__ __forceinline__ int overlap_bound(const OverlapArgs &a, int s)
{
    return s <= 0 ? a.store0 : (s >= a.G ? 0x7fffffff : a.first_bound + (s - 1) * a.Ls);
}

template <int RX>
__global__ void __launch_bounds__(128) clock_overlap_kernel(OverlapArgs a, int span)
{
    __shared__ float table[(XR_MM_NSTEPS + 1) * XR_MM_NTAPS];
    __shared__ cf32 xr[RX + RELAY_XMIR];
    __shared__ int sh_xhi, sh_pos_ii, sh_done, sh_simd[2], sh_swap, sh_claim;
    clock_table_to_lds(table, a.table);
    const int s = blockIdx.x, lane = threadIdx.x & 63;
    int role = __builtin_amdgcn_readfirstlane((int)(threadIdx.x >> 6));

    ClockState T = a.start[s];
    T.ii = __builtin_amdgcn_readfirstlane((int)T.ii);
    T.mu = relay_lane(T.mu, 0); T.omega = relay_lane(T.omega, 0);
    T.p0 = cf32{relay_lane(T.p0.x, 0), relay_lane(T.p0.y, 0)}; T.p1 = cf32{relay_lane(T.p1.x, 0), relay_lane(T.p1.y, 0)};
    const int ni_w = (int)(a.ni < 0x7fffffffLL ? a.ni : 0x7fffffffLL);
    const int lo = s == 0 ? a.store0 : overlap_bound(a, s) - a.early;
    const int hi = overlap_bound(a, s + 1);
    const int x_lo = (int)(T.ii > 4 ? T.ii - 4 : 0);
    if (threadIdx.x == 0) { sh_xhi = x_lo; sh_pos_ii = (int)T.ii; sh_done = 0; }
    __syncthreads();
    if ((int)T.ii >= ni_w || (int)T.ii < 0) {
        if (threadIdx.x == 0) {
            OverlapSeg e{};
            e.end = T;
            e.flags = OV_EMPTY;
            a.segs[s] = e;
        }
        return;
    }
    unsigned *claim = nullptr;
    if (a.simd_claim) {
        const unsigned hw = __builtin_amdgcn_s_getreg((4) | (0 << 6) | (31 << 11));
        const unsigned xcc = __builtin_amdgcn_s_getreg((20) | (0 << 6) | (31 << 11));
        if (lane == 0) sh_simd[threadIdx.x >> 6] = (int)((hw >> 4) & 3u);
        __syncthreads();
        claim = a.simd_claim + ((((xcc & 7u) << 8) | ((hw >> 8) & 255u)) & (RELAY_CLAIM_WORDS - 1));
        if (threadIdx.x == 0) {
            const unsigned b0 = 1u << sh_simd[0], b1 = 1u << sh_simd[1];
            int swap = 0, mine = -1;
            if (!(atomicOr(claim, b0) & b0)) mine = sh_simd[0];
            else if (b1 != b0 && !(atomicOr(claim, b1) & b1)) { mine = sh_simd[1]; swap = 1; }
            sh_swap = swap;
            sh_claim = mine;
        }
        __syncthreads();
        role ^= __builtin_amdgcn_readfirstlane(sh_swap);
    }
    const cf32 *xs = reinterpret_cast<const cf32 *>(a.x);

    if (role == 1) {
        const long long nlast = a.N > 0 ? a.N - 1 : 0;
        const long long xend = hi < 0x7fffffff ? (long long)hi + span + 16 : nlast + span + 16;
        int x_hi = x_lo;
        unsigned rounds = 0;
        while (!relay_ld(&sh_done)) {
            if (++rounds > (1u << 24)) { if (lane == 0) a.stat[2] = 0xc0000000u | (unsigned)s; break; }
            const int pii = relay_ld(&sh_pos_ii);
            const bool fx = x_hi + RELAY_XCH - RX <= pii && (long long)x_hi <= xend && (long long)x_hi <= nlast + span + 16;
            if (!fx) { __builtin_amdgcn_s_sleep(4); continue; }
            cf32 vx[RELAY_XCH / 64];
#pragma unroll
            for (int q = 0; q < RELAY_XCH / 64; ++q) {
                const long long i = (long long)x_hi + lane + 64 * q;
                vx[q] = xs[i < nlast ? i : nlast];
            }
#pragma unroll
            for (int q = 0; q < RELAY_XCH / 64; ++q) {
                const int slot = (x_hi + lane + 64 * q) & (RX - 1);
                xr[slot] = vx[q];
                if (slot < RELAY_XMIR) xr[RX + slot] = vx[q];
            }
            x_hi += RELAY_XCH;
            if (lane == 0) relay_st(&sh_xhi, x_hi);
        }
        return;
    }

    const float gkw = a.par.gain_omega * (16777216.0f / (float)a.q_om), gkm = a.par.gain_mu * (16777216.0f / (float)a.q_mu);
    const int sh_om = 31 - __builtin_clz((unsigned)a.q_om), sh_mu = 31 - __builtin_clz((unsigned)a.q_mu);
    const int stride = __builtin_amdgcn_readfirstlane(a.stride);
    float *stage = a.stage + (size_t)s * (size_t)stride;
    OverlapSeg *seg = a.segs + s;
    int n_st = 0;
    unsigned steps = 0, rounds_total = 0;
    bool exhausted = false, stuck = false;
    int x_hi = x_lo;
    float m1 = 0.f, m2 = 0.f;
#ifdef XRIT_RELAY_TIMING
    unsigned long long tacc[6] = {0, 0, 0, 0, 0, 0}, tlast = __builtin_amdgcn_s_memtime();
    unsigned n_refresh = 0, n_spin = 0;
#endif
    for (;;) {
        RELAY_TICK(5);
        const int ii0 = (int)T.ii;
        if ((unsigned)ii0 >= (unsigned)ni_w) { exhausted = true; break; }
        if (ii0 >= hi) break;
        ++steps;
        const int need_x = ii0 + span + 8;
        if (x_hi < need_x) {
            int spins = 0;
#ifdef XRIT_RELAY_TIMING
            ++n_refresh;
#endif
#pragma nounroll
            while (x_hi < need_x) {
                x_hi = relay_ld(&sh_xhi);
                if (x_hi >= need_x) break;
#ifdef XRIT_RELAY_TIMING
                ++n_spin;
#endif
                __builtin_amdgcn_s_sleep(2);
                if (++spins > (1 << 22)) { if (lane == 0) a.stat[2] = 0x80000000u | (unsigned)s; stuck = true; break; }
            }
            if (stuck) break;
        }
        RELAY_TICK(0);
        const int mu0u = (int)(T.mu * 16777216.0f), W0 = (int)(T.omega * 16777216.0f);
        const int wint = W0 >> 24, wfrac = W0 & 0xffffff;
        const int fr0 = mu0u + lane * wfrac, bii = ii0 + lane * wint;
        int cii = bii + (fr0 >> 24), carm;
        float cmu = (float)(fr0 & 0xffffff) * (1.0f / 16777216.0f), com = T.omega;
        if (lane == 0) cmu = T.mu;
        carm = (int)rintf(cmu * (float)XR_MM_NSTEPS);
        cf32 p0{0.f, 0.f};
        float mm = 0.f;
        ClockState hs{};
        bool stale = false, inrange = true;
        RELAY_TICK(1);
        for (int round = 0; round < RELAY_ROUNDS; ++round) {
            ++rounds_total;
            inrange = cii >= ii0 && cii + XR_MM_NTAPS <= need_x;
            cf32 w[XR_MM_NTAPS];
            const cf32 *wp = xr + (cii & (RX - 1));
#pragma unroll
            for (int q = 0; q < XR_MM_NTAPS; ++q) w[q] = wp[q];
            p0 = clock_interp_arm(w, table, carm);
            hs.p0 = cf32{relay_shr1_from(p0.x, T.p0.x), relay_shr1_from(p0.y, T.p0.y)};
            hs.p1 = cf32{relay_shr1_from(hs.p0.x, T.p1.x), relay_shr1_from(hs.p0.y, T.p1.y)};
            hs.c0 = cf32{hs.p0.x > 0.f ? 1.f : 0.f, hs.p0.y > 0.f ? 1.f : 0.f};
            hs.c1 = cf32{hs.p1.x > 0.f ? 1.f : 0.f, hs.p1.y > 0.f ? 1.f : 0.f};
            mm = clock_timing_error(p0, hs);
            const int dW = (int)rintf(mm * gkw) << sh_om;
            const int dM = (int)rintf(mm * gkm) << sh_mu;
            const int C = relay_scan(dW, lane);
            const int E = C + dM;
            const int D = relay_scan(E, lane) - E;
            const int fr = fr0 + D;
            int nii = bii + (fr >> 24);
            float nmu = (float)(fr & 0xffffff) * (1.0f / 16777216.0f);
            float nom = (float)(W0 + C - dW) * (1.0f / 16777216.0f);
            if (lane == 0) { nii = ii0; nmu = T.mu; nom = T.omega; }
            const int narm = (int)rintf(nmu * (float)XR_MM_NSTEPS);
            stale = nii != cii || narm != carm;
            cii = nii; carm = narm; cmu = nmu; com = nom;
            if (!__any(stale)) break;
        }
        RELAY_TICK(2);
        ClockState st = hs;
        st.ii = cii; st.mu = cmu; st.omega = com;
        clock_advance(mm, p0, st, a.par);
        const int nxt_ii = relay_dpp<0x130>(cii);
        const float nxt_mu = relay_shl1(cmu), nxt_om = relay_shl1(com);
        const bool exists = (unsigned)cii < (unsigned)ni_w;
        const bool good = !stale && inrange;
        const bool ok = good && exists && lane < 63 && (int)st.ii == nxt_ii && st.mu == nxt_mu && st.omega == nxt_om;
        const unsigned long long okm = __ballot(ok), exm = __ballot(exists), gdm = __ballot(good), him = __ballot(cii >= hi),
                                 lom = __ballot(cii >= lo);
        const int m = ~okm ? __builtin_ctzll(~okm) : 64;
        const int e = ~exm ? __builtin_ctzll(~exm) : 64;
        const int g = ~gdm ? __builtin_ctzll(~gdm) : 64;
        const int h = him ? __builtin_ctzll(him) : 64;
        int nv = m + 1 < 64 ? m + 1 : 64;
        nv = nv < g ? nv : g;
        nv = nv < h ? nv : h;
        if (e < nv) { nv = e; exhausted = true; }
        RELAY_TICK(3);
        if (nv > 0) {
            const int l0 = lom ? __builtin_ctzll(lom) : 64;
            if (lane >= l0 && lane < nv) {
                const int o = n_st + lane - l0;
                if (o < stride) stage[o] = p0.x;
                if (o < OV_HEAD) { seg->head_ii[o] = cii; seg->head_mu[o] = cmu; }
                m1 += fabsf(p0.x);
                m2 += p0.x * p0.x;
            }
            if (l0 < nv) n_st += nv - l0;
            const int src = nv - 1;
            ClockState nt;
            nt.ii = __builtin_amdgcn_readlane((int)st.ii, src);
            nt.mu = relay_lane(st.mu, src);
            nt.omega = relay_lane(st.omega, src);
            nt.p0 = cf32{relay_lane(st.p0.x, src), relay_lane(st.p0.y, src)};
            nt.p1 = cf32{relay_lane(st.p1.x, src), relay_lane(st.p1.y, src)};
            T = nt;
            if (lane == 0) relay_st(&sh_pos_ii, (int)T.ii);
        }
        RELAY_TICK(4);
        if (exhausted || nv == 0) { exhausted = true; break; }
    }
#ifdef XRIT_RELAY_TIMING
    if (lane == 0) {
        for (int q = 0; q < 6; ++q) atomicAdd(&relay_dbg[q], tacc[q]);
        atomicAdd(&relay_dbg[6], (unsigned long long)steps);
        atomicAdd(&relay_dbg[7], (unsigned long long)n_refresh);
        atomicAdd(&relay_dbg[8], (unsigned long long)n_spin);
    }
#endif
    for (int off = 32; off > 0; off >>= 1) { m1 += __shfl_xor(m1, off, 64); m2 += __shfl_xor(m2, off, 64); }
    if (lane == 0) {
        relay_st(&sh_done, 1);
        if (claim && sh_claim >= 0) atomicAnd(claim, ~(1u << sh_claim));
        atomicAdd(&a.stat[0], steps);
        atomicAdd(&a.stat[1], rounds_total);
        atomicAdd(&a.stat[3], 1u);
        atomicAdd(&a.moments[0], (unsigned long long)((double)m1 * 1048576.0));
        atomicAdd(&a.moments[1], (unsigned long long)((double)m2 * 1048576.0));
        T.c0 = cf32{T.p0.x > 0.f ? 1.f : 0.f, T.p0.y > 0.f ? 1.f : 0.f};
        T.c1 = cf32{T.p1.x > 0.f ? 1.f : 0.f, T.p1.y > 0.f ? 1.f : 0.f};
        seg->end = T;
        seg->count = n_st < stride ? n_st : stride;
        seg->flags = (stuck ? OV_STUCK : 0) | (exhausted && !stuck ? OV_EXHAUSTED : 0) | (n_st > stride ? OV_STUCK : 0);
    }
}

__global__ void clock_overlap_guess_kernel(const double *__restrict__ cnt, int nb, const double *__restrict__ cnt_prev, int nb_prev,
                                           long long n_prev, int BL, double sps, float omega0, const float2 *__restrict__ x,
                                           const float *__restrict__ table, long long ni, int padN, int hist, int G,
                                           int store0, int first_bound, int Ls, const ClockState *__restrict__ carried,
                                           int w0_carried, int w0_ii, int valid_lo, ClockState *__restrict__ S,
                                           unsigned *__restrict__ stat, unsigned long long *__restrict__ moments)
{
    const int s = blockIdx.x * blockDim.x + threadIdx.x;
    if (blockIdx.x == 0) {
        if (threadIdx.x < 8) stat[threadIdx.x] = 0u;
        if (threadIdx.x < 2) moments[threadIdx.x] = 0ull;
    }
    if (s >= G) return;
    if (s == 0 && w0_carried) {
        ClockState c = carried[0];
        c.ii = w0_ii;
        S[0] = c;
        return;
    }
    const int bound = s == 0 ? store0 : first_bound + (s - 1) * Ls;
    double t = (double)bound - (double)hist;
    if (t < (double)valid_lo + 3.0 + 2.0 * sps) t = (double)valid_lo + 3.0 + 2.0 * sps;
    const bool prev = t < (double)padN && cnt_prev != nullptr && nb_prev > 0;
    const double *c = prev ? cnt_prev : cnt;
    const int nbc = prev ? nb_prev : nb;
    const double org = prev ? (double)padN - (double)n_prev : (double)padN;
    double u = t - org;
    const double target = rint(clk_count_at(c, nbc, sps, u, 0.0, BL));
    for (int it = 0; it < 4; ++it) u += (target - clk_count_at(c, nbc, sps, u, 0.0, BL)) * sps;
    t = u + org - 3.0;
    if (t < (double)valid_lo) t = (double)valid_lo;
    ClockState st;
    st.ii = (long long)floor(t);
    st.mu = (float)(t - floor(t));
    st.omega = omega0;
    st.p0 = cf32{0.f, 0.f}; st.p1 = cf32{0.f, 0.f};
    st.c0 = cf32{0.f, 0.f}; st.c1 = cf32{0.f, 0.f};
    if (st.ii >= ni) { st.ii = 0x7fffffff; S[s] = st; return; }
    for (int back = 2; back >= 1; --back) {
        const double tb = t - back * (double)omega0;
        if (tb < (double)valid_lo) continue;
        const long long ib = (long long)floor(tb);
        if (ib >= ni) continue;
        const float mub = (float)(tb - floor(tb));
        const int imu = (int)rintf(mub * (float)XR_MM_NSTEPS);
        const float *row = table + imu * XR_MM_NTAPS;
        float ar = 0.f, ai = 0.f;
        for (int q = 0; q < XR_MM_NTAPS; ++q) {
            const float2 v = x[ib + q];
            ar += row[XR_MM_NTAPS - 1 - q] * v.x;
            ai += row[XR_MM_NTAPS - 1 - q] * v.y;
        }
        st.p1 = st.p0; st.c1 = st.c0;
        st.p0 = cf32{ar, ai};
        st.c0 = cf32{ar > 0.f ? 1.f : 0.f, ai > 0.f ? 1.f : 0.f};
    }
    S[s] = st;
}

__global__ void __launch_bounds__(256) clock_overlap_scan_kernel(const OverlapSeg *__restrict__ segs, int G, int stride,
                                                                  const ClockState *__restrict__ carried_in, int w0_ii,
                                                                  int w0_carried, float omega_mid, int *__restrict__ j0,
                                                                  unsigned long long *__restrict__ offs,
                                                                  ClockState *__restrict__ carried_out, ClockResult *__restrict__ res,
                                                                  const float2 *__restrict__ x, float2 *__restrict__ tail_out,
                                                                  long long N, int *__restrict__ ctl,
                                                                  const unsigned long long *__restrict__ moments,
                                                                  unsigned long long cap)
{
    __shared__ unsigned long long part[256];
    __shared__ int s_term, s_bad, s_stuck;
    __shared__ unsigned s_far;
    __shared__ long long s_ii;
    if (threadIdx.x == 0) { s_term = 0x7fffffff; s_bad = 0; s_stuck = 0; s_far = 0u; }
    __syncthreads();
    for (int s = threadIdx.x; s < G; s += blockDim.x) {
        const OverlapSeg e = segs[s];
        int pick = 0;
        if (e.flags & OV_STUCK) s_stuck = 1;
        if (e.flags & (OV_EXHAUSTED | OV_EMPTY)) atomicMin(&s_term, s);
        if (!(e.flags & OV_EMPTY) && !(s == 0 && w0_carried)) {
            double want;
            if (s == 0) want = (double)w0_ii + (double)carried_in[0].mu;
            else { const ClockState p = segs[s - 1].end; want = (double)p.ii + (double)p.mu; }
            double best = 1e30;
            const int nh = e.count < OV_HEAD ? e.count : OV_HEAD;
            for (int q = 0; q < nh; ++q) {
                const double d = fabs((double)e.head_ii[q] + (double)e.head_mu[q] - want);
                if (d < best) { best = d; pick = q; }
            }
            const bool front_ended = s > 0 && (segs[s - 1].flags & (OV_EXHAUSTED | OV_EMPTY)) != 0;
            if (!front_ended) {
                if (nh == 0 || !(best < 0.25 * (double)omega_mid)) atomicAdd(&s_bad, 1);
                else atomicMax(&s_far, __float_as_uint((float)best));
            }
        }
        j0[s] = pick;
    }
    __syncthreads();
    const int term = s_term;
    unsigned long long run = 0;
    {
        const int per = (G + (int)blockDim.x - 1) / (int)blockDim.x;
        const int b = threadIdx.x * per, e = b + per < G ? b + per : G;
        unsigned long long sum = 0;
        for (int s = b; s < e; ++s) sum += (s <= term && segs[s].count > j0[s]) ? (unsigned long long)(segs[s].count - j0[s]) : 0ull;
        part[threadIdx.x] = sum;
        __syncthreads();
        if (threadIdx.x == 0) {
            unsigned long long acc = 0;
            for (int q = 0; q < (int)blockDim.x; ++q) { const unsigned long long v = part[q]; part[q] = acc; acc += v; }
            run = acc;
        }
        __syncthreads();
        unsigned long long acc = part[threadIdx.x];
        for (int s = b; s < e; ++s) {
            offs[s] = acc;
            acc += (s <= term && segs[s].count > j0[s]) ? (unsigned long long)(segs[s].count - j0[s]) : 0ull;
            if (s > term) offs[s] = ~0ull;
        }
    }
    __syncthreads();
    if (threadIdx.x == 0) {
        ClockState st;
        ctl[CLK_CTL_RELAY_PASSES] = 1;
        ctl[CLK_CTL_RELAY_CLOSED] = 0;
        ctl[CLK_CTL_RELAY_SHIFT_SQ] = 0;
        ctl[CLK_CTL_STUCK] = s_stuck;
        ctl[CLK_CTL_RELAY_MOVE_MAX] = 0;
        ctl[CLK_CTL_OV_BAD_JOINTS] = s_bad;
        ctl[CLK_CTL_OV_JOINT_MAX] = (int)s_far;
        ctl[CLK_CTL_WALKERS] = G;
        const bool ok = term < G && !s_stuck && s_bad == 0 && run <= cap;
        if (!ok) {
            res->ok = 0;
            res->n_symbols = term < G ? run : 0ull;
            res->terminal_chain = -1;
            st = carried_in[0];
            st.ii = w0_ii;
        } else {
            res->ok = 1;
            res->terminal_chain = term;
            res->n_symbols = run;
            st = segs[term].end;
        }
        {
            const double nsym = (double)run;
            const double a1 = nsym > 0 ? (double)moments[0] / 1048576.0 / nsym : 0.0, a2 = nsym > 0 ? (double)moments[1] / 1048576.0 / nsym : 0.0;
            const double var = a2 - a1 * a1;
            ctl[CLK_CTL_SNR2] = __float_as_int(nsym > 0 && var > 0 ? (float)(a1 * a1 / var) : 1e30f);
        }
        long long ii = st.ii;
        if (ii > N) ii = N;
        if (ii < 0) ii = 0;
        res->ii_final = ii;
        s_ii = ii;
        st.ii = 0;
        carried_out[0] = st;
    }
    __syncthreads();
    const long long ii = s_ii;
    long long carry = N - ii;
    if (carry > 1024) {
        carry = 1024;
        if (threadIdx.x == 0) res->ok = 0;
    }
    for (long long i = threadIdx.x; i < carry; i += blockDim.x) tail_out[i] = x[ii + i];
}

__global__ void __launch_bounds__(256) clock_overlap_copy_kernel(const float *__restrict__ stage, const OverlapSeg *__restrict__ segs,
                                                                  const int *__restrict__ j0, const unsigned long long *__restrict__ offs,
                                                                  int stride, float *__restrict__ soft, unsigned long long cap,
                                                                  const ClockResult *__restrict__ res)
{
    if (!res->ok) return;
    const int s = blockIdx.y;
    const unsigned long long off = offs[s];
    if (off == ~0ull) return;
    const int first = j0[s], len = segs[s].count - first;
    const float *src = stage + (size_t)s * (size_t)stride + first;
#pragma unroll
    for (int q = 0; q < 4; ++q) {
        const int i = (int)blockIdx.x * 1024 + q * 256 + (int)threadIdx.x;
        if (i < len && off + (unsigned long long)i < cap) soft[off + (unsigned long long)i] = src[i];
    }
}

}
```

xritdemod_amd/csrc/clock_plan.h:

```cpp
#pragma once

#include <math.h>
#include <stddef.h>
#include <stdio.h>

#include "clock_ctl.h"

namespace xrit {

#define XR_MM_NTAPS  8
#define XR_MM_NSTEPS 128
#define XR_MM_FUDGE  16
constexpr int CLK_OM_BLOCK = 256;
constexpr int CLK_M = 2;
constexpr int CLK_SLACK = 3;
#ifndef XR_CLK_MIR
#define XR_CLK_MIR (XR_MM_NTAPS - 1)
#endif
constexpr int CLK_MIR = XR_CLK_MIR;
constexpr int CLK_ROW_EXTRA = CLK_MIR > 0 ? CLK_MIR : 1;
constexpr int RELAY_RX = 2048;
constexpr int RELAY_XCH = 512;
constexpr int RELAY_CLAIM_WORDS = 2048;

struct ClockPar { float omega_mid, omega_lim, gain_omega, gain_mu; };

struct ClockKnobs {
    ClockPar par{};
    float sps = 0;
    int NS = 64;
    int cu_count = 256;
    long long lds_per_cu = 160 * 1024;
    bool auto_ns = true;
    bool serial = false;
    int max_passes = 48, min_passes = 4;
    bool pass_writes = true;
    int ng_max = 8;
    int exact = 0;
    float auto_rms = 3e-4f;
    int auto_passes = 3;
    long long auto_guess_min = 6000000;
    int auto_long_seg = 49152;
    int one_walk_max = 0;
    long long one_walk_limit() const { return one_walk_max > 0 ? (long long)one_walk_max : 3LL * (auto_long_seg / 2); }
    float auto_shift = 6e-4f;
    float auto_snr = 10.0f;
    float auto_snr_floor = 2.0f;
    long long auto_min = 1;
    bool relay_by_default() const { return exact >= 1 || (exact == 0 && auto_passes > 0); }
    int relay_window = 0;
    bool relay_global = false;
    int relay_per_cu = 3;
    bool relay_per_cu_set = false;
    int relay_no_handoff = -1;
    bool relay_quick = false;
    int relay_apx_cfg[2] = {-1, -1};
    int relay_waves = 1;
    int relay_teams_per_cu = 1;
    bool ov_allow = true;
    bool ov_enabled = true;
    long long ov_min = 1000000;
    int ov_hist = 49152;
    int ov_min_range = 8192;
    int ov_min_walkers = 240;
    bool ov_small_ring = false;
    double ov_lratio = 1.0;
};

inline size_t clock_tile_bytes(int WS, int ngroups, int threads)
{
    return 4160 + 256 * (size_t)ngroups + ((size_t)ngroups * 64 * WS + threads) * 2 * sizeof(float);
}

inline int relay_span(const ClockPar &par, int symbols)
{
    return (int)ceil((double)symbols * ((double)par.omega_mid + (double)par.omega_lim + 0.004)) + 24;
}
inline bool relay_ring_ok(const ClockPar &par) { return relay_span(par, 64) + 8 <= RELAY_RX - RELAY_XCH - 72; }

struct ClockLattice { int q_om, q_mu; };
inline ClockLattice clock_lattice(float omega_mid)
{
    const float om = omega_mid, su = omega_mid + 0.5f;
    const double u = 1.0 / 16777216.0;
    ClockLattice l;
    l.q_om = (int)((double)(nextafterf(om, INFINITY) - om) / u);
    l.q_mu = (int)((double)(nextafterf(su, INFINITY) - su) / u);
    if (l.q_om < 1) l.q_om = 1;
    if (l.q_mu < 1) l.q_mu = 1;
    return l;
}

struct ClockRelaySegs { int cps = 0, G = 0; };
inline ClockRelaySegs clock_relay_segments(const ClockKnobs &k, int K, int NS, bool no_handoff, int relay_budget, int relay_w)
{
    int auto_per_cu = 2;
    if (no_handoff && k.exact == 0)
        for (int p = 4; p > 2; --p)
            if ((long long)K * NS / ((long long)p * k.cu_count) >= k.auto_long_seg) { auto_per_cu = p; break; }
    const int per_cu = relay_w > 0 ? k.relay_teams_per_cu : (no_handoff && !k.relay_per_cu_set ? auto_per_cu : k.relay_per_cu);
    int cps = k.relay_window > 0 ? k.relay_window : (K + per_cu * k.cu_count - 1) / (per_cu * k.cu_count);
    int min_syms = relay_budget > 0 ? 16384 : 2048;
    if (no_handoff && k.exact == 0 && !k.relay_per_cu_set) {
        const long long all = (long long)K * NS;
        min_syms = all <= k.one_walk_limit() ? (int)all : k.auto_long_seg / 2;
    }
    if (k.relay_window <= 0 && cps * NS < min_syms) cps = (min_syms + NS - 1) / NS;
    if (cps < 1) cps = 1;
    ClockRelaySegs r;
    r.cps = cps;
    r.G = (K + cps - 1) / cps;
    return r;
}
inline int clock_relay_limit(int G, int relay_budget)
{
    const int hard = G + 1;
    return relay_budget > 0 ? (relay_budget < hard ? relay_budget : hard) : hard;
}

struct ClockChainPlan {
    char err[128] = {0};
    long long N = 0, ni = 0;
    bool short_input = false;
    int SS = 0, W = 0, WS = 0, A = 0, STEP = 0; bool wide = false;
    int NG = 1, waves_cu = 0;
    size_t tile_bytes = 0, tile_bytes3 = 0;
    int NS = 64, K = 0;
    bool relay = false;
    bool no_handoff = false;
    int relay_budget = 0;
    int relay_apx[2] = {0, 0};
    bool relay_long = false;
    int write_from = 0x7fffffff;
    ClockRelaySegs segs;
};

inline ClockChainPlan clock_chain_plan(const ClockKnobs &k, size_t n, size_t carry, int last_passes, int relay_w = 0)
{
    ClockChainPlan j;
    const ClockPar &par = k.par;
    j.NS = k.NS;
    j.N = (long long)(carry + n);
    j.ni = j.N - XR_MM_NTAPS - XR_MM_FUDGE;
    if (j.N >= (1LL << 31)) { snprintf(j.err, sizeof j.err, "clock recovery: more than 2^31 samples in one call"); return j; }
    if (j.ni <= 0) {
        j.short_input = true;
        if (j.N > 1024) snprintf(j.err, sizeof j.err, "clock recovery: unread tail exceeds the hand-over buffer");
        return j;
    }
    if (k.serial) { j.K = 1; return j; }
    const double min_omega = (double)par.omega_mid - (double)par.omega_lim;
    const double max_adv = (double)par.omega_mid + (double)par.omega_lim + 0.004;
    static const int tries[6][2] = {{32, 4}, {32, 2}, {32, 1}, {64, 4}, {64, 2}, {64, 1}};
    int SS = 1, A = 0, R = 64;
    for (int q = 0; q < 6; ++q) {
        R = tries[q][0];
        SS = tries[q][1];
        A = (int)ceil(SS * max_adv) + 1;
        if (CLK_M + CLK_SLACK + A + XR_MM_NTAPS <= R) break;
    }
    j.wide = R > 32;
    j.SS = SS; j.W = R; j.A = A;
    j.STEP = (int)floor((double)SS * (double)par.omega_mid * 65536.0);
    j.WS = R + CLK_ROW_EXTRA;
    j.tile_bytes3 = clock_tile_bytes(j.WS, 1, 192);
    j.NG = 1;
    for (int ng = 1; ng <= 8 && ng <= k.ng_max; ++ng) {
        const long long need = (long long)clock_tile_bytes(j.WS, ng, 64 * ng);
        if (need > k.lds_per_cu) break;
        long long wv = (long long)ng * (k.lds_per_cu / need);
        if (wv > 8) wv = 8;
        if (wv >= j.waves_cu) { j.waves_cu = (int)wv; j.NG = ng; }
    }
    if (j.waves_cu < 1) { snprintf(j.err, sizeof j.err, "clock recovery: a ring of %d samples per chain does not fit LDS", R); return j; }
    j.tile_bytes = clock_tile_bytes(j.WS, j.NG, 64 * j.NG);
    if (k.auto_ns) {
        const long long resident = (long long)k.cu_count * j.waves_cu;
        const double symbols = (double)j.N / min_omega;
        j.NS = 64;
        for (int g = 1; g <= 64; ++g) {
            const double chains = (double)(g * resident * 64 - 4);
            int ns = (int)ceil(symbols / chains);
            ns = (ns + 15) & ~15;
            if (ns <= 256) { j.NS = ns < 64 ? 64 : ns; break; }
        }
    }
    const int NS = j.NS;
    const int K = (int)((double)j.N / (min_omega * NS)) + 3;
    j.K = K;
    const int exact = k.exact;
    j.relay = exact >= 1 || (exact == 0 && k.auto_passes > 0 && (long long)K * NS >= k.auto_min);
    j.relay_budget = exact > 1 ? exact : (exact == 1 ? 0 : k.auto_passes);
    const long long all_syms = (long long)K * NS;
    j.no_handoff = j.relay && (k.relay_no_handoff >= 0 ? k.relay_no_handoff != 0
                                                       : exact == 0 && (all_syms <= k.one_walk_limit() || all_syms >= k.auto_guess_min));
    if (j.relay) j.segs = clock_relay_segments(k, K, NS, j.no_handoff, j.relay_budget, relay_w);
    if (j.no_handoff && exact == 0) {
        const long long L = (long long)j.segs.cps * NS;
        j.relay_budget = L >= k.auto_long_seg ? 2 : (L >= k.auto_long_seg / 2 ? 3 : 4);
        if (k.relay_quick && j.relay_budget >= 3 && j.segs.G > j.relay_budget && relay_w == 0) {
            for (int p = 0; p < 2 && p < j.relay_budget - 1; ++p) j.relay_apx[p] = p == j.relay_budget - 2 ? 2 : 1;
        }
    }
    for (int p = 0; p < 2; ++p) if (k.relay_apx_cfg[p] >= 0 && j.relay && j.segs.G > 1) j.relay_apx[p] = k.relay_apx_cfg[p];

    j.relay_long = j.relay && !j.no_handoff && exact == 0 && k.auto_passes >= 3 && (long long)j.segs.cps * NS >= k.auto_long_seg;
    if (j.relay_long) j.relay_budget = 2;
    j.write_from = k.pass_writes ? (last_passes - 1 > 3 ? last_passes - 1 : 3) : 0x7fffffff;
    return j;
}

inline int clock_ov_pad_need(const ClockKnobs &k)
{
    const double wmax = (double)k.par.omega_mid + (double)k.par.omega_lim + 0.004;
    int need = (int)ceil((double)k.ov_hist * wmax) + XR_MM_NTAPS + XR_MM_FUDGE + 6 * (int)ceil(wmax) + 64;
    return (need + 15) & ~15;
}
inline size_t clock_xpad(const ClockKnobs &k)
{
    const int need = clock_ov_pad_need(k);
    return k.ov_enabled && relay_ring_ok(k.par) && (size_t)need > 1024 ? (size_t)need : 1024;
}
inline bool clock_ov_eligible(const ClockKnobs &k, size_t xpad, bool fixed_base, size_t n)
{
    if (!k.ov_enabled || !k.ov_allow || k.exact != 0 || k.relay_quick || k.serial || k.relay_global || fixed_base) return false;
    if (k.relay_no_handoff == 0 || k.auto_passes <= 0) return false;
    if (k.relay_window > 0) return false;
    if ((size_t)clock_ov_pad_need(k) > xpad) return false;
    if (n >= ((size_t)1 << 31) - xpad - 4096) return false;
    return (double)n / (double)k.par.omega_mid >= (double)k.ov_min;
}

struct ClockOvPlan {
    char err[128] = {0};
    long long N = 0, ni = 0;
    int padN = 0;
    int G = 0, Ls = 0, first_bound = 0, store0 = 0, early = 0, stride = 0, hist = 0;
    bool w0_carried = false;
    int w0_ii = 0;
};
inline ClockOvPlan clock_ov_plan(const ClockKnobs &k, size_t n, size_t carry, bool have_hist, bool ahead)
{
    ClockOvPlan j;
    const ClockPar &par = k.par;
    const double wmax = (double)par.omega_mid + (double)par.omega_lim + 0.004, wmin = (double)par.omega_mid - (double)par.omega_lim;
    const int cw = (int)ceil(wmax);
    j.hist = (int)ceil((double)k.ov_hist * (double)par.omega_mid);
    j.early = (int)ceil(1.5 * wmax) + 2;
    if (ahead && !have_hist) { snprintf(j.err, sizeof j.err, "clock recovery: an overlap job cannot start ahead without the history of the call in front"); return j; }
    if (have_hist) {
        j.padN = clock_ov_pad_need(k);
        j.w0_carried = false;
        j.w0_ii = ahead ? 0 : j.padN - (int)carry;
        j.store0 = j.padN - (XR_MM_NTAPS + XR_MM_FUDGE) - cw - 2;
    } else {
        if (carry > 1024) { snprintf(j.err, sizeof j.err, "clock recovery: carry of %zu samples exceeds the hand-over buffer", carry); return j; }
        j.padN = (int)carry;
        j.w0_carried = true;
        j.w0_ii = 0;
        j.store0 = 0;
    }
    j.N = (long long)j.padN + (long long)n;
    j.ni = j.N - XR_MM_NTAPS - XR_MM_FUDGE;
    const double nsym = (double)n / (double)par.omega_mid;
    double gt = nsym / ((double)k.ov_hist * k.ov_lratio);
    if (gt < (double)k.ov_min_walkers) gt = (double)k.ov_min_walkers;
    if (nsym / gt < (double)k.ov_min_range) gt = nsym / (double)k.ov_min_range;
    if (gt > 2.5 * k.cu_count) gt = 2.5 * k.cu_count;
    if (gt < 1.0) gt = 1.0;
    long long Ls = (long long)ceil((double)n / gt);
    Ls = (Ls + 63) & ~63LL;
    if (Ls < 4096) Ls = 4096;
    j.Ls = (int)Ls;
    const long long w0_start = j.w0_carried ? 0 : (long long)j.store0 - j.hist;
    long long fb = w0_start + j.hist + Ls;
    if (fb < (long long)j.padN + Ls) fb = (long long)j.padN + Ls;
    j.first_bound = (int)fb;
    const long long lim = j.N - Ls / 4;
    j.G = fb <= lim ? 2 + (int)((lim - fb) / Ls) : 1;
    const long long last_start = j.G >= 2 ? fb + (long long)(j.G - 2) * Ls : (long long)j.store0;
    long long longest = fb - j.store0;
    if (j.G >= 2 && Ls + j.early > longest) longest = Ls + j.early;
    if (j.N - last_start + j.early > longest) longest = j.N - last_start + j.early;
    if (j.G == 1) longest = j.N - j.store0;
    long long stride = (long long)ceil((double)longest / wmin) + 64;
    stride = (stride + 63) & ~63LL;
    if (stride * j.G >= (1LL << 31)) { snprintf(j.err, sizeof j.err, "clock recovery: call too long for the overlap plan"); return j; }
    j.stride = (int)stride;
    return j;
}

inline bool clock_handoff_to_closure(const ClockKnobs &k, const int *ctl, int K, bool relay)
{
    if (!((k.exact == 0 || k.exact <= -2) && K > 1 && !relay)) return false;
    const float q = clock_ctl_float(ctl, CLK_CTL_SUM_SQ);
    const int open_ = ctl[CLK_CTL_OPEN_LAST];
    return ctl[CLK_CTL_DONE] == 0 || (open_ > 0 && q > k.auto_rms * k.auto_rms * (float)open_);
}

struct ClockRelayLook {
    bool first = true;
    bool relay_auto = false;
    bool relay_force = false, no_handoff = false, relay_long = false;
    int relay_enq = 0, G = 0, relay_budget = 0;
};
enum ClockRelayVerdict {
    CLK_RELAY_TAKE,
    CLK_RELAY_TO_CLOSURE,
    CLK_RELAY_FOUR_MORE,
    CLK_RELAY_NO_SIGNAL,
    CLK_RELAY_CONTINUE,
};
struct ClockRelayStep {
    ClockRelayVerdict verdict;
    bool relay_auto; int relay_budget;
    bool snr_seen; float snr2;
};
inline ClockRelayStep clock_relay_look(const ClockKnobs &k, const int *ctl, const ClockRelayLook &c)
{
    ClockRelayStep r{CLK_RELAY_TAKE, c.relay_auto, c.relay_budget, false, 0.f};
    const bool closed = ctl[CLK_CTL_RELAY_CLOSED] != 0;
    if (c.first && k.exact == 0 && !c.relay_auto && !closed) {
        float shift_sq = clock_ctl_float(ctl, CLK_CTL_RELAY_SHIFT_SQ);
        const float snr2 = clock_ctl_float(ctl, CLK_CTL_SNR2);
        r.snr_seen = true; r.snr2 = snr2;
        const bool signal = snr2 >= k.auto_snr_floor;
        bool to_closure = signal && ((c.relay_force && !c.no_handoff) || !(snr2 >= k.auto_snr));
        if (!signal || to_closure || c.relay_long || c.no_handoff) shift_sq = 0.0f;
        if (c.no_handoff && signal && !to_closure && !(clock_ctl_float(ctl, CLK_CTL_RELAY_MOVE_MAX) < 0.25f * k.sps)) to_closure = true;
        if (to_closure) { r.verdict = CLK_RELAY_TO_CLOSURE; r.relay_auto = true; r.relay_budget = 0; return r; }
        if (!(shift_sq <= k.auto_shift * k.auto_shift) && c.relay_enq < c.G + 1) {
            r.verdict = CLK_RELAY_FOUR_MORE; r.relay_auto = true; r.relay_budget = c.relay_enq + 4;
            return r;
        }
    }
    if (closed || c.relay_enq >= clock_relay_limit(c.G, c.relay_budget)) return r;
    if (c.relay_auto && k.exact != 1 && !(clock_ctl_float(ctl, CLK_CTL_SNR2) >= k.auto_snr_floor)) { r.verdict = CLK_RELAY_NO_SIGNAL; return r; }
    r.verdict = CLK_RELAY_CONTINUE;
    return r;
}

enum ClockOvVerdict { CLK_OV_TAKE, CLK_OV_FALLBACK, CLK_OV_FALLBACK_TO_CLOSURE, CLK_OV_WATCHDOG };
inline ClockOvVerdict clock_overlap_look(const ClockKnobs &k, const int *ctl)
{
    if (ctl[CLK_CTL_STUCK]) return CLK_OV_WATCHDOG;
    const float snr2 = clock_ctl_float(ctl, CLK_CTL_SNR2);
    const bool signal = snr2 >= k.auto_snr_floor;
    if ((signal && !(snr2 >= k.auto_snr)) || ctl[CLK_CTL_OV_BAD_JOINTS] > 0) return signal ? CLK_OV_FALLBACK_TO_CLOSURE : CLK_OV_FALLBACK;
    return CLK_OV_TAKE;
}

inline int clock_next_relay_batch(int relay_passes)
{
    const int want = relay_passes + relay_passes / 4 + 8;
    return want < 32 ? 32 : (want > 4096 ? 4096 : want);
}
inline int clock_next_batch(int passes, bool relay)
{
    const int want = passes + 1;
    const int least = relay && passes <= 2 ? 3 : 5;
    return want < least ? least : (want > 32 ? 32 : want);
}

}
```

xritdemod_amd/csrc/kernels.h:

```cpp
#pragma once

#include <functional>

#include "common.h"
#include "framer_host.h"
#include "lock_host.h"
#include "clock_jobs.h"
#include "clock_plan.h"
#include "loop_core.h"
#include "taps.h"

namespace xrit {

struct FirStage {
    int T = 0, D = 1, RC = 3, W = 0, Wpad = 0, threads = 256, tile_len = 0, cur = 0;
    bool pad = false;
    bool mfma_dec = false;
    bool no_static_dec = false, no_static_mf = false;
    int prio = 0;
    bool poly = false;
    bool exact = false, ex_pad = false;
    int ex_threads = 256, ex_opt = 2, ex_tile_len = 0;
    size_t ex_lds = 0;
    DevBuf rt;
    std::vector<float> taps_host;
    int set_exact(bool on);
#ifndef XRIT_POLY_PR
#define XRIT_POLY_PR 16
#endif
    static constexpr int POLY_PR = XRIT_POLY_PR, POLY_NQ = 32;
    size_t lds_bytes = 0;
    DevBuf g;
    DevBuf mfb;
    DevBuf hist[2];
    int init(const float *taps, int ntaps, int decim);
    int reset(hipStream_t s);
    void release();
    int run(const void *in, int sample_type, float2 *out, size_t n_out, hipStream_t s, Profiler *prof,
            float2 *stat = nullptr, int statL = 0, const struct AgcEpilogue *agc = nullptr,
            const struct AgcFill *fill = nullptr, bool use_exact = false);
    FirStage *twin = nullptr;
    bool last_twin = false;
    FirStage() = default;
    FirStage(const FirStage &) = delete;
    FirStage &operator=(const FirStage &) = delete;
    bool agc_fill_supported(int per_lane) const;
    bool stat_supported(int statL) const;
    bool agc_supported() const;
};

constexpr int AGC_RUN_MAX_PER_LANE = 5;
struct AgcFill {
    const float2 *x;
    const struct AgcMap *pre_run;
    const float *state_in;
    float *state_out;
    float rate, ref, maxg;
    int per_lane;
};
struct AgcEpilogue {
    struct AgcMap *maps;
    float *state_out;
    float rate, ref, maxg;
};

struct RtlIngestStage {
    float alpha = 0;
    DevBuf state;
    DevBuf aggs;
    int cur = 0;
    int init(float sample_rate);
    int reset(hipStream_t s);
    void release();
    int run(const void *in_u8, float2 *out, size_t n_complex, hipStream_t s, Profiler *prof);
};

struct AgcStage {
    float rate = 0, ref = 0, maxg = 0;
    DevBuf state;
    DevBuf aggs;
    int cur = 0;
    int init(float rate, float reference, float gain, float max_gain);
    int reset(hipStream_t s);
    float gain0 = 1.0f;
    void release();
    int run(const float2 *in, float2 *out, size_t n, hipStream_t s, Profiler *prof, bool use_exact = false);
    bool exact = false;
    DevBuf joints;
    int ex_walkers = 2048, ex_mode = 3;
    int run_exact(const float2 *in, float2 *out, size_t n, hipStream_t s, Profiler *prof);
    unsigned *ex_cnt = nullptr;
    int exact_counters(unsigned *out8, hipStream_t s);
    int fused_begin(size_t n, int per_lane, hipStream_t s, AgcEpilogue *epi);
    int fused_finish(const float2 *in, float2 *out, size_t n, int per_lane, hipStream_t s, Profiler *prof);
    int fused_reduce(const float2 *in, size_t n, int per_lane, hipStream_t s, Profiler *prof);
    int fused_scan(const float2 *in, float2 *fallback, size_t n, int per_lane, hipStream_t s, Profiler *prof, AgcFill *fill);
    int gain(float *g, hipStream_t s);
    int fallback_flag(float *flag, hipStream_t s);
    int request_flag(hipStream_t s);
    int request_flag_at(const float *flag, hipStream_t s);
    float requested_flag() const { return h_flag ? *h_flag : 0.0f; }
    float *h_flag = nullptr;
};

struct CostasStage {
    CostasGains gains{};
    int L = 256;
    int max_passes = 32;
    float trust = 1.0f, tol_phase = 1e-5f, tol_freq = 3e-8f;
    DevBuf state;
    DevBuf S, E, J, stat, sub, dlin, work, flags, counters, wsolve, rescue;
    bool model_step = true;
    float model_accept = 5e-3f;
    bool force_gated = false;
    int final_warm = 0;
    bool keep_spare = false, trace_env = false, no_serial_walk = false;
    int rescue_after = 32;
    long long rescue_max_samples = 4 << 20;
    unsigned rescues = 0;
    bool walked = false;
    int serial_rescue(hipStream_t s, Profiler *prof);
    unsigned *h_counters = nullptr;
    int cur = 0;
    int passes = 0;
    unsigned unconverged = 0;
    float max_residual = 0;
    int init(float loop_bw, int chain_len, int max_passes);
    int reset(hipStream_t s);
    void release();
    int run(const float2 *in, float2 *out, size_t n, hipStream_t s, Profiler *prof, const float2 *sub_ext = nullptr,
            double2 *om = nullptr, long long om_off = 0, double inv_sps = 0.0);
    int begin(const float2 *in, float2 *out, size_t n, hipStream_t s, Profiler *prof, const float2 *sub_ext,
              double2 *om, long long om_off, double inv_sps, bool use_exact = false);
    bool closed() const;
    int finish(hipStream_t s, Profiler *prof, bool *redone);
    int enqueue_passes(int count, hipStream_t s, Profiler *prof);
    int enqueue_final(hipStream_t s, Profiler *prof);
    struct Job {
        const float2 *in = nullptr; float2 *out = nullptr; size_t n = 0; int K = 0; int enqueued = 0;
        double2 *om = nullptr; long long om_off = 0; double inv_sps = 0;
        bool gated = false;
        bool rescued = false;
        bool exact = false;
        float model_accept = 0;
    } job;
    int batch = 4;
    int stable = 0, last_passes = -1;
    int get_state(float *phase, float *freq, hipStream_t s);
    bool exact = false;
    int ex_mode = 3;
    int ex_hist = -1;
    int ex_prio = 1;
    int ex_walkers = 2048;
    DevBuf xj, xbs, xcnt;
    unsigned *h_xcnt = nullptr;
    int ex_W = 0, ex_rounds = 0;
    bool ex_args_valid = false;
    unsigned ex_open = 0, ex_nonconverged = 0;
    unsigned long long ex_blocks = 0, ex_picard = 0, ex_segs = 0, ex_fallbacks = 0;
    int exact_plan(size_t n, int *Lw, int *W, int *H) const;
    int enqueue_exact(hipStream_t s, Profiler *prof);
    int finish_exact(hipStream_t s, Profiler *prof, bool *redone);
    int flip_phase(hipStream_t s);
};

int launch_loop_sincosf(const float *d_x, float *d_sin, float *d_cos, size_t n, hipStream_t s);

struct ClockResult;
struct ClockStage : ClockKnobs {
    float mu0 = 0.5f;
    int jac_passes = 1;
    float tol_t = 2e-6f, tol_w = 2e-7f;
    bool force_gated = false;
    bool relay_no_rec = false;
    bool relay_no_claim = false;
    bool relay_rec01 = true;
    bool trace_env = false;
    bool no_meanj = false;
    std::function<int(int)> before_relay;
    static constexpr size_t CARRY_HEAD = 64, CARRY_BYTES = 64 + 1024 * sizeof(float2);
    size_t xpad = 1024;
    int ov_pad_need = 0;

    int batch = 7;
    int last_passes = -1;
    int relay_batch = 96;
    bool jmean_valid = false;
    int jmean_ns = 0;

    ClockJobs jobs;

    struct Job : ClockChainPlan {
        size_t n = 0, cap = 0; float *soft = nullptr; float2 *sym = nullptr;
        float2 *base = nullptr;
        int exact = 0;
        int enqueued = 0;
        bool mean_j = false;
        bool gated = false;
        int *dirty = nullptr, *counts = nullptr, *nrun = nullptr, *terminal = nullptr, *written = nullptr;
        int G = 0, cps = 0, relay_enq = 0;
        int relay_w = 0;
        bool relay_force = false;
    } job;
    struct OvJob {
        DevBuf om, om_work, segs, S, stage, aux;
        hipEvent_t ev_walk = nullptr;
        hipEvent_t ev_guess = nullptr;
    } ov[NXB];
    float *ov_soft = nullptr; size_t ov_cap = 0;

    int passes = 0;
    unsigned unconverged = 0;
    unsigned large_open = 0;
    float max_residual = 0;
    size_t last_symbols = 0;
    float snr_estimate = 0.f;
    bool relay_auto = false;
    int relay_passes = 0;
    bool relay_closed = false;
    int relay_segments = 0, relay_seg_chains = 0;
    bool ov_fell_back = false;
    int ov_walkers = 0;
    float ov_joint_max = 0.f;

    DevBuf table;
    DevBuf xbuf[NXB];
    DevBuf st;
    DevBuf S, E, J, om, work, counters, sym, dlin, flags, wsolve, jmean;
    DevBuf om_work;
    DevBuf tail;
    void *h_res = nullptr;
    DevBuf relay;
    DevBuf relay_rec;
    DevBuf stage;
    DevBuf alt;
    DevBuf ov_claim;
    float2 *xdata() const { return xbuf[jobs.xb].as<float2>() + xpad; }
    float2 *xbase() const { return job.base ? job.base : xdata() - jobs.carry; }

    int init(float omega, float gain_omega, float mu, float gain_mu, float omega_rel_limit, int chain_syms,
             int max_passes);
    int reset(hipStream_t s);
    void release();
    int input_slot(size_t n, float2 **slot, hipStream_t s);
    double2 *om_slot(int nb, int BL);
    int om_scan(hipStream_t s);
    int run(size_t n, float *soft_out, float2 *sym_out, size_t cap, size_t *n_out, hipStream_t s, Profiler *prof);
    int redo_flipped(float *soft_out, float2 *sym_out, size_t cap, size_t *n_out, hipStream_t s, Profiler *prof);
    int export_carry(void *d_rec, int which, hipStream_t s);
    int redo_from(const void *d_rec, size_t carry_rec, float *soft_out, float2 *sym_out, size_t cap, size_t *n_out, hipStream_t s, Profiler *prof);
    bool last_walk_exact() const;
    int make_alt(hipStream_t s, Profiler *prof);
    int begin(size_t n, float *soft_out, float2 *sym_out, size_t cap, hipStream_t s, Profiler *prof);
    bool closed() const;
    int finish(size_t *n_out, hipStream_t s, Profiler *prof);
    bool ov_eligible(size_t n) const { return clock_ov_eligible(*this, xpad, false, n); }
    int ov_launch(int job, hipStream_t sw, bool ahead, Profiler *prof);
    int ov_restart(int job);

    int run_chains(float2 *base, int exact_, size_t n, float *soft_out, float2 *sym_out, size_t cap, size_t *n_out, hipStream_t s, Profiler *prof);
    int begin_chains(float2 *base, int exact_, size_t n, float *soft_out, float2 *sym_out, size_t cap, hipStream_t s, Profiler *prof);
    int begin_short(hipStream_t s);
    int begin_serial(hipStream_t s, Profiler *prof);
    void call_reset(size_t n);
    ClockKnobs call_knobs() const { ClockKnobs k = *this; k.exact = job.exact; return k; }
    int begin_overlap(size_t n, float *soft_out, size_t cap, hipStream_t s, Profiler *prof);
    int launch_chains(bool ext, bool scanned, hipStream_t s, Profiler *prof);
    int finish_overlap(size_t *n_out, hipStream_t s, Profiler *prof);
    int finish_chains(size_t *n_out, hipStream_t s, Profiler *prof);
    int finish_handoff(hipStream_t s, Profiler *prof);
    int finish_relay(hipStream_t s, Profiler *prof);
    int enqueue_passes(int count, hipStream_t s, Profiler *prof);
    int enqueue_output(hipStream_t s, Profiler *prof, bool again = false);
    int enqueue_relay(int count, bool restart, hipStream_t s, Profiler *prof);
    int relay_w_plan() const;
    int relay_cut();
    int ov_finalize(int job, float *soft_out, size_t cap, hipStream_t s, Profiler *prof);
    int ov_fallback(size_t *n_out, hipStream_t s, Profiler *prof, bool to_closure);
    int trace_overlap(int job, const struct ClockResult &r) const;
    int trace_relay() const;
    int trace_passes() const;
};

int launch_sync_correlate(const int8_t *data, size_t n, const unsigned long long *words, int nwords, unsigned frame,
                          xrit_sync_hit *hits, hipStream_t s);
int launch_sync_fix(const int8_t *data, size_t n, const xrit_sync_hit *hits, unsigned frame, unsigned min_corr,
                    int8_t *frames, unsigned char *valid, hipStream_t s);
int launch_quantize_i8(const float *in, int8_t *out, size_t n, hipStream_t s);
constexpr int FRAME_SYMBOLS = 16384, CADU_BYTES = 1024, BLOCK_BYTES = 1020, VCDU_BYTES = 892, ZONE_BYTES = 884;
constexpr int NVC = 64;
constexpr size_t MAX_ROWS_PER_CALL = (size_t)1 << 24;
struct Carver {
    char *p;
    size_t n = 0;
    template <class T> T *take(size_t count, size_t align)
    {
        T *r = p ? reinterpret_cast<T *>(p + n) : nullptr;
        n += (count * sizeof(T) + align - 1) & ~(align - 1);
        return r;
    }
    size_t used() const { return n; }
};
size_t viterbi_slot_bytes();
int launch_viterbi(const int8_t *frames, const unsigned char *valid, size_t nf, int hrit, int8_t *carry, int *prev, int *last,
                   unsigned long long *dec, unsigned slots, unsigned char *cadu, unsigned *verr, hipStream_t s);
int launch_rs(const unsigned char *cadu, const unsigned char *valid, const unsigned *verr, size_t nf, unsigned char *block,
              xrit_frame_info *info, hipStream_t s);
constexpr int DEMUX_TILE = 1024;
struct DemuxState {
    long long last[NVC], received[NVC], lost[NVC];
    unsigned long long frames, dropped, sum_vit, sum_rs, lost_total;
};
struct DemuxScratch {
    unsigned *cnt; int *firstc, *lastc; unsigned *tsum;
    unsigned *base; int *P; unsigned long long *tin;
    long long *vcb;
};
size_t demux_scratch_carve(void *p, size_t nf, DemuxScratch &sc);
int launch_demux(const xrit_sync_hit *hits, const unsigned char *cadu, size_t cadu_stride, const unsigned char *block,
                 const xrit_frame_info *info, size_t nf, DemuxState *state, DemuxScratch &sc, unsigned char *vcdu,
                 unsigned *offsets, xrit_frame_stats *records, hipStream_t s);
struct FramerCall {
    unsigned long long base;
    unsigned carry, total, cursor, count;
};
struct FramerScratch {
    unsigned *bits;
    unsigned *bmax;
    uint4 *rec;
    unsigned *nrec;
    uint2 *wout;
    uint4 *rows;
    unsigned char *flags;
    FramerCall *call;
};
struct LockPar {
    unsigned recheck;
    unsigned span;
    unsigned first;
    unsigned r0;
    unsigned short0;
};
size_t framer_scratch_carve(void *p, size_t n, unsigned frame, unsigned seg_chunks, FramerScratch &sc);
int launch_framer_bits(const FramerPar &par, const FramerState *state, const int8_t *carry_in, const int8_t *symbols,
                       FramerScratch &sc, hipStream_t s);
int launch_framer_gather(const FramerPar &par, const FramerCall *call, const int8_t *carry_in, const int8_t *symbols,
                         const uint4 *rows, int8_t *carry_out, int8_t *frames, unsigned char *valid, xrit_sync_hit *hits,
                         unsigned long long *start, hipStream_t s);
int launch_plain_joints(const FramerPar &par, FramerState *state, FramerScratch &sc, unsigned *count, hipStream_t s);
int launch_lock_walk(const FramerPar &par, const LockPar &lp, const LockState *state, FramerScratch &sc, hipStream_t s);
int launch_lock_joints(const FramerPar &par, const LockPar &lp, LockState *state, FramerScratch &sc, unsigned *count, hipStream_t s);
int launch_lock_commit(const FramerPar &par, const LockPar &lp, LockState *state, FramerScratch &sc, const xrit_frame_info *info,
                       unsigned char *mode, hipStream_t s);
constexpr unsigned PACKETS_PEND_MAX = 65541;
constexpr unsigned PACKETS_TILE = 1024;
constexpr unsigned PACKETS_PEND_STRIDE = 65544;
struct PacketsState {
    unsigned long long packets[64], crc_failures[64], fill_packets[64], discarded[64], bad_fhp[64], rows[64];
    int last[64];
    unsigned pend_len[64], first_counter[64];
};
struct PacketsScratch {
    unsigned *rowA;
    uint2 *spanB;
    uint2 *newp;
    unsigned *state_disc;
    unsigned *plocal, *blocal;
    uint2 *tsum;
    unsigned *tbase_c;
    unsigned long long *tbase_b;
    unsigned *crcfail;
};
size_t packets_scratch_carve(void *p, size_t max_rows, PacketsScratch &sc);
int launch_packets(const unsigned char *vcdu, const unsigned *offsets, size_t max_rows, PacketsState *state,
                   unsigned char *pend, PacketsScratch &sc, unsigned char *bytes, size_t max_bytes, xrit_packet *packets,
                   size_t max_packets, unsigned *pkt_offsets, xrit_packets_summary *summary, hipStream_t s);
constexpr unsigned FILES_KEYS = 64 * 2048;
constexpr unsigned FILES_TILE = 2048;
constexpr unsigned FILES_TSUM = 10;
struct FilesScratch {
    unsigned *order;
    unsigned *kstart, *kcount;
    unsigned *kpieces, *krecs;
    unsigned long long *kbytes;
    unsigned long long *tsum, *tbase;
    unsigned *kcnt;
    unsigned long long *psrc, *pdst;
    unsigned *plen;
};
size_t files_scratch_carve(void *p, size_t max_in, FilesScratch &sc);
int launch_files(const unsigned char *in_bytes, size_t n_in_bytes, const xrit_packet *packets, const unsigned *pkt_offsets,
                 size_t max_in, xrit_file_key *keys, xrit_files_counters *counters, FilesScratch &sc, unsigned char *bytes,
                 size_t max_bytes, xrit_file_piece *pieces, size_t max_pieces, xrit_file_record *files, size_t max_files,
                 xrit_files_summary *summary, hipStream_t s);
constexpr int RICE_FORM_LANE = 1, RICE_FORM_WAVE = 2;
int launch_rice(const unsigned char *bytes, size_t n_bytes, const void *desc, size_t stride, size_t n_lines, int n, int J, int S,
                void *out, unsigned char *status, int form, hipStream_t s);
constexpr unsigned IMAGES_TILE = 1024;
constexpr unsigned IMAGES_TSUM = 6;
struct ImageMark;
struct ImagesScratch {
    ImageMark *mark;
    unsigned *rlines;
    unsigned long long *rbytes;
    unsigned *rfaults;
    unsigned long long *tsum, *tbase;
    unsigned long long *call;
    unsigned char *lstatus;
};
size_t images_scratch_carve(void *p, size_t max_files_in, size_t max_pieces_in, ImagesScratch &sc);
int launch_images(const unsigned char *bytes, size_t n_bytes, const xrit_file_piece *pieces, size_t max_pieces_in,
                  const xrit_file_record *files, size_t max_files_in, const xrit_files_summary *fsum, xrit_image_key *keys,
                  xrit_images_counters *counters, ImagesScratch &sc, unsigned char *out, size_t max_bytes, xrit_image_line *lines,
                  size_t max_lines, xrit_image_file *image_files, xrit_images_summary *summary, hipStream_t s);
struct CanvasHead;
struct CanvasPlace;
struct CanvasBounds {
    unsigned long long n_bytes, max_pieces, max_files, n_image_bytes, max_lines;
};
struct CanvasState {
    xrit_canvas_slot *slots;
    xrit_canvas_segment *segs;
    xrit_canvas_key_state *keys;
    xrit_canvas_counters *counters;
    unsigned char *pixels;
    unsigned n_slots;
    size_t slot_bytes;
};
struct CanvasScratch {
    CanvasHead *heads;
    CanvasPlace *place;
    unsigned long long *call;
};
size_t canvas_scratch_carve(void *p, size_t max_files_in, CanvasScratch &sc);
int launch_canvas(const unsigned char *bytes, const xrit_file_piece *pieces, const xrit_file_record *files, const xrit_files_summary *fsum,
                  const unsigned char *image_bytes, const xrit_image_line *lines, const xrit_image_file *image_files,
                  const xrit_images_summary *isum, const CanvasBounds &b, const CanvasState &st, CanvasScratch &sc,
                  xrit_canvas_file *canvas_files, xrit_canvas_slot *out_slots, xrit_canvas_summary *summary, hipStream_t s);
int launch_canvas_release(const CanvasState &st, unsigned slot, hipStream_t s);
struct AcquireScratch {
    float2 *spectra;
    double *power;
};
size_t acquire_scratch_carve(void *p, unsigned segments, AcquireScratch &sc);
int launch_acquire_mix(const void *in, int type, size_t n, float2 *out, xrit_acquire_state *st, hipStream_t s);
int launch_acquire_set_inc(xrit_acquire_state *st, long long inc, hipStream_t s);
int launch_acquire_estimate(const void *in, int type, unsigned segments, const xrit_acquire_params &par, const float2 *tw, const float *win,
                            const AcquireScratch &sc, int apply, xrit_acquire_state *st, xrit_acquire_estimate_record *rec, hipStream_t s);
int launch_convert(const void *in, int type, float2 *out, size_t n, hipStream_t s);
int launch_synth(const xrit_synth_params &p, uint64_t start, size_t n, float2 *out, hipStream_t s);
int launch_read_bw(const void *buf, size_t bytes, int reps, hipStream_t s, double *gbs);

}
```

Baseline: 154,400.

## Add guided two-phase overlap walkers that replay the next walker's recorded symbol positions

```diff
diff --git a/xritdemod_amd/csrc/clock.hip b/xritdemod_amd/csrc/clock.hip
--- a/xritdemod_amd/csrc/clock.hip
+++ b/xritdemod_amd/csrc/clock.hip
@@ -896,6 +896,7 @@
     }
     ov_enabled = getenv("XRIT_NO_OVERLAP") == nullptr;
     if (const char *e = getenv("XRIT_OV_HIST")) { const int v = atoi(e); if (v >= 1024) ov_hist = v; }
+    if (const char *e = getenv("XRIT_OV_GUIDE")) { const int v = atoi(e); if (v >= 0 && v <= 2) ov_guide = v; }
 #ifdef XRIT_EXPERIMENTS
     if (const char *e = getenv("XRIT_OV_MIN")) { const long long v = atoll(e); if (v > 0) ov_min = v; }
     if (const char *e = getenv("XRIT_OV_SMALL_RING")) ov_small_ring = atoi(e) != 0;
@@ -972,6 +973,7 @@
     for (auto &b : xbuf) b.release();
     for (auto &j : ov) {
         j.om.release(); j.om_work.release(); j.segs.release(); j.S.release(); j.stage.release(); j.aux.release();
+        j.rec.release(); j.anchor.release(); j.hand.release();
         if (j.ev_walk) (void)hipEventDestroy(j.ev_walk);
         if (j.ev_guess) (void)hipEventDestroy(j.ev_guess);
         j.ev_walk = nullptr; j.ev_guess = nullptr;
@@ -1319,7 +1321,7 @@
         if (plan.err[0]) { set_error("%s", plan.err); return XRIT_E_INVALID; }
         jobs.planned(job, plan, ahead);
         XR_TRY(d.segs.reserve((size_t)j.G * sizeof(OverlapSeg)));
-        XR_TRY(d.S.reserve((size_t)j.G * sizeof(ClockState)));
+        XR_TRY(d.S.reserve(((size_t)j.G + 1) * sizeof(ClockState)));
         XR_TRY(d.stage.reserve((size_t)j.G * (size_t)j.stride * sizeof(float) + 256));
         XR_TRY(d.aux.reserve(64 + (size_t)j.G * sizeof(int) + 8 + (size_t)j.G * sizeof(unsigned long long)));
     }
@@ -1358,19 +1360,36 @@
     const ClockLattice lat = clock_lattice(par.omega_mid);
     a.q_om = lat.q_om; a.q_mu = lat.q_mu;
     a.stat = ov_stat(d); a.moments = ov_moments(d); a.simd_claim = relay_no_claim ? nullptr : ov_claim.as<unsigned>();
+    a.guide = ov_guide;
+    if (ov_guide) {
+        const ClockOvGuide g = clock_ov_guide_plan(*this, j);
+        XR_TRY(d.rec.reserve(g.entries * sizeof(unsigned)));
+        XR_TRY(d.anchor.reserve(g.anchors * sizeof(int)));
+        XR_TRY(d.hand.reserve(((size_t)j.G + 1) * sizeof(OverlapHand)));
+        a.rec = d.rec.as<unsigned>(); a.anchor = d.anchor.as<int>(); a.hand = d.hand.as<OverlapHand>();
+        a.rec_stride = g.rec_stride; a.guide_cap = g.guide_cap; a.guide_span = g.guide_span;
+    }
     const int span = relay_span(par, 64);
     {
         ProfScope ps(prof, "clock_guess", sw);
-        hipLaunchKernelGGL(clock_overlap_guess_kernel, dim3(div_up((size_t)j.G, 256)), dim3(256), 0, sw, cnt, nb, cnt_prev, nb_prev,
+        hipLaunchKernelGGL(clock_overlap_guess_kernel, dim3(div_up((size_t)j.G + 1, 256)), dim3(256), 0, sw, cnt, nb, cnt_prev, nb_prev,
                            (long long)h_n, BL, (double)sps, par.omega_mid, base, table.as<float>(), j.ni, j.padN, j.hist, j.G, j.store0,
                            j.first_bound, j.Ls, st.as<ClockState>() + jobs.cur, j.w0_carried ? 1 : 0, j.w0_ii, 0, d.S.as<ClockState>(),
-                           a.stat, a.moments);
+                           a.stat, a.moments, ov_guide ? 1 : 0, clock_ov_guide_bound(j));
     }
     XR_HIP(hipEventRecord(d.ev_guess, sw));
     {
         ProfScope ps(prof, "clock_overlap", sw);
-        if (ov_small_ring && span + 8 <= 1024 - RELAY_XCH - 72) hipLaunchKernelGGL(clock_overlap_kernel<1024>, dim3(j.G), dim3(128), 0, sw, a, span);
-        else hipLaunchKernelGGL(clock_overlap_kernel<RELAY_RX>, dim3(j.G), dim3(128), 0, sw, a, span);
+        const bool small = ov_small_ring && span + 8 <= 1024 - RELAY_XCH - 72;
+        if (!ov_guide) {
+            if (small) hipLaunchKernelGGL((clock_overlap_kernel<1024, 0>), dim3(j.G), dim3(128), 0, sw, a, span);
+            else hipLaunchKernelGGL((clock_overlap_kernel<RELAY_RX, 0>), dim3(j.G), dim3(128), 0, sw, a, span);
+        } else {
+            if (small) hipLaunchKernelGGL((clock_overlap_kernel<1024, 1>), dim3(j.G + 1), dim3(128), 0, sw, a, span);
+            else hipLaunchKernelGGL((clock_overlap_kernel<RELAY_RX, 1>), dim3(j.G + 1), dim3(128), 0, sw, a, span);
+            if (small) hipLaunchKernelGGL((clock_overlap_kernel<1024, 2>), dim3(j.G), dim3(128), 0, sw, a, span);
+            else hipLaunchKernelGGL((clock_overlap_kernel<RELAY_RX, 2>), dim3(j.G), dim3(128), 0, sw, a, span);
+        }
     }
     XR_HIP(hipGetLastError());
     XR_HIP(hipEventRecord(d.ev_walk, sw));
@@ -1721,6 +1740,8 @@
                     "joints: %d do not fit, largest distance %.3e sample; 2 Es/N0 = %.1f; %llu symbols%s\n",
             oj.G, oj.Ls, oj.hist, oj.w0_carried ? "walker 0 from the carried state" : "walker 0 warms up in the burst before", hs[0],
             hs[0] ? (double)hs[1] / hs[0] : 0.0, hc[CLK_CTL_OV_BAD_JOINTS], (double)ov_joint_max, (double)snr_estimate, (unsigned long long)r.n_symbols, r.ok ? "" : " -- NOT taken");
+    fprintf(stderr, "[xrit] overlap phases (XRIT_OV_GUIDE=%d): A %u steps, %.3f guess rounds per step; B %u steps, %.3f guess rounds per step\n",
+            ov_guide, hs[4], hs[4] ? (double)hs[5] / hs[4] : 0.0, hs[6], hs[6] ? (double)hs[7] / hs[6] : 0.0);
 #ifdef XRIT_RELAY_TIMING
     unsigned long long hd[16] = {0}, z[16] = {0};
     XR_HIP(hipMemcpyFromSymbol(hd, HIP_SYMBOL(relay_dbg), sizeof hd));
@@ -1729,6 +1750,13 @@
     fprintf(stderr, "[xrit] overlap walkers, cycles per step: ring wait %.0f, setup %.0f, guess rounds %.0f, literal step + verdict %.0f, "
                     "stage + commit %.0f, loop %.0f; sum %.0f (%llu steps)\n", hd[0] / st, hd[1] / st, hd[2] / st, hd[3] / st, hd[4] / st,
             hd[5] / st, (hd[0] + hd[1] + hd[2] + hd[3] + hd[4] + hd[5]) / st, hd[6]);
+    if (hd[14]) {
+        const unsigned long long *hb = hd + 8;
+        const double sb = (double)hb[6];
+        fprintf(stderr, "[xrit] overlap walkers, phase B, cycles per step: ring wait %.0f, setup %.0f, guess rounds %.0f, literal step + verdict %.0f, "
+                        "stage + commit %.0f, loop %.0f; sum %.0f (%llu steps)\n", hb[0] / sb, hb[1] / sb, hb[2] / sb, hb[3] / sb, hb[4] / sb,
+                hb[5] / sb, (hb[0] + hb[1] + hb[2] + hb[3] + hb[4] + hb[5]) / sb, hb[6]);
+    }
 #endif
     return XRIT_OK;
 }
diff --git a/xritdemod_amd/csrc/clock_overlap.h b/xritdemod_amd/csrc/clock_overlap.h
--- a/xritdemod_amd/csrc/clock_overlap.h
+++ b/xritdemod_amd/csrc/clock_overlap.h
@@ -18,6 +18,15 @@
     int pad_[2];
 };
 static_assert(sizeof(OverlapSeg) == 128, "OverlapSeg is a 128-byte record");
+
+struct OverlapHand {
+    ClockState T;
+    int n_st;
+    int flags;
+    int n_rec;
+    int pad_;
+};
+static_assert(sizeof(OverlapHand) == 64, "OverlapHand is a 64-byte record");
 
 struct OverlapArgs {
     const float2 *x;
@@ -36,6 +45,12 @@
     unsigned *stat;
     unsigned long long *moments;
     unsigned *simd_claim;
+    unsigned *rec;
+    int *anchor;
+    OverlapHand *hand;
+    int rec_stride, guide_cap;
+    int guide;
+    int guide_span;
 };
 
 __device__ __forceinline__ int overlap_bound(const OverlapArgs &a, int s)
@@ -43,35 +58,81 @@
     return s <= 0 ? a.store0 : (s >= a.G ? 0x7fffffff : a.first_bound + (s - 1) * a.Ls);
 }
 
-template <int RX>
+template <int RX, int PHASE>
 __global__ void __launch_bounds__(128) clock_overlap_kernel(OverlapArgs a, int span)
 {
+    constexpr bool GUIDED = PHASE == 2;
+    constexpr int NGA = RELAY_GR / OV_ANCHOR;
     __shared__ float table[(XR_MM_NSTEPS + 1) * XR_MM_NTAPS];
     __shared__ cf32 xr[RX + RELAY_XMIR];
-    __shared__ int sh_xhi, sh_pos_ii, sh_done, sh_simd[2], sh_swap, sh_claim;
+    __shared__ unsigned gr[GUIDED ? RELAY_GR : 1];
+    __shared__ int ga[GUIDED ? NGA : 1];
+    __shared__ int sh_xhi, sh_pos_ii, sh_done, sh_simd[2], sh_swap, sh_claim, sh_ghi, sh_pos_n;
     clock_table_to_lds(table, a.table);
     const int s = blockIdx.x, lane = threadIdx.x & 63;
     int role = __builtin_amdgcn_readfirstlane((int)(threadIdx.x >> 6));
-
-    ClockState T = a.start[s];
+    const bool guide_only = PHASE == 1 && s >= a.G;
+
+    ClockState T;
+    int n_st = 0;
+    bool exhausted = false, stuck = false;
+    if (PHASE == 2) {
+        const OverlapHand h = a.hand[s];
+        const int hf = __builtin_amdgcn_readfirstlane(h.flags);
+        if (hf & OV_EMPTY) return;
+        T = h.T;
+        n_st = __builtin_amdgcn_readfirstlane(h.n_st);
+        exhausted = (hf & OV_EXHAUSTED) != 0;
+        stuck = (hf & OV_STUCK) != 0;
+    } else {
+        T = a.start[s];
+    }
     T.ii = __builtin_amdgcn_readfirstlane((int)T.ii);
     T.mu = relay_lane(T.mu, 0); T.omega = relay_lane(T.omega, 0);
     T.p0 = cf32{relay_lane(T.p0.x, 0), relay_lane(T.p0.y, 0)}; T.p1 = cf32{relay_lane(T.p1.x, 0), relay_lane(T.p1.y, 0)};
     const int ni_w = (int)(a.ni < 0x7fffffffLL ? a.ni : 0x7fffffffLL);
-    const int lo = s == 0 ? a.store0 : overlap_bound(a, s) - a.early;
-    const int hi = overlap_bound(a, s + 1);
+    const int lo = guide_only ? 0x7fffffff : (s == 0 ? a.store0 : overlap_bound(a, s) - a.early);
+    const int hi = guide_only ? 0x7fffffff : overlap_bound(a, s + 1);
+    int stop = hi;
+    if (PHASE == 1 && !guide_only) stop = __builtin_amdgcn_readfirstlane(clock_ov_phase_a_end(hi, (long long)a.start[s + 1].ii));
+    if (guide_only) stop = __builtin_amdgcn_readfirstlane(clock_ov_phase_a_end(hi, (long long)T.ii + (long long)a.guide_span));
     const int x_lo = (int)(T.ii > 4 ? T.ii - 4 : 0);
-    if (threadIdx.x == 0) { sh_xhi = x_lo; sh_pos_ii = (int)T.ii; sh_done = 0; }
+    if (threadIdx.x == 0) { sh_xhi = x_lo; sh_pos_ii = (int)T.ii; sh_done = 0; sh_ghi = 0; sh_pos_n = 0; }
     __syncthreads();
-    if ((int)T.ii >= ni_w || (int)T.ii < 0) {
+    if (PHASE != 2 && ((int)T.ii >= ni_w || (int)T.ii < 0)) {
         if (threadIdx.x == 0) {
-            OverlapSeg e{};
-            e.end = T;
-            e.flags = OV_EMPTY;
-            a.segs[s] = e;
+            if (!guide_only) {
+                OverlapSeg e{};
+                e.end = T;
+                e.flags = OV_EMPTY;
+                a.segs[s] = e;
+            }
+            if (PHASE == 1) {
+                OverlapHand h{};
+                h.T = T;
+                h.flags = OV_EMPTY;
+                a.hand[s] = h;
+            }
         }
         return;
     }
+    int e0 = OV_NOALIGN, n_rec = 0;
+    const unsigned *recs_in = nullptr;
+    const int *anch_in = nullptr;
+    if (GUIDED && !exhausted && !stuck) {
+        const size_t ro = (size_t)(s + 1) * (size_t)a.rec_stride;
+        recs_in = a.rec + ro;
+        anch_in = a.anchor + ro / OV_ANCHOR;
+        n_rec = __builtin_amdgcn_readfirstlane(a.hand[s + 1].n_rec);
+        const int cap = s + 1 < a.G ? a.rec_stride : a.guide_cap;
+        n_rec = n_rec < 0 ? 0 : (n_rec > cap ? cap : n_rec);
+        e0 = __builtin_amdgcn_readfirstlane(clock_ov_align(anch_in, n_rec, (int)T.ii, a.par.omega_mid));
+    }
+    const bool use_rec = GUIDED && e0 != OV_NOALIGN;
+    const int e0s = e0 + (a.guide == 2 ? 1 : 0);
+    const int n_end = use_rec ? n_rec - e0s : 0;
+    const int n_anch = (n_rec + OV_ANCHOR - 1) / OV_ANCHOR;
+    const int wnom = (int)(a.par.omega_mid * 16777216.0f), wint_n = wnom >> 24, wfrac_n = wnom & 0xffffff;
     unsigned *claim = nullptr;
     if (a.simd_claim) {
         const unsigned hw = __builtin_amdgcn_s_getreg((4) | (0 << 6) | (31 << 11));
@@ -94,28 +155,48 @@
 
     if (role == 1) {
         const long long nlast = a.N > 0 ? a.N - 1 : 0;
-        const long long xend = hi < 0x7fffffff ? (long long)hi + span + 16 : nlast + span + 16;
-        int x_hi = x_lo;
+        const long long xend = stop < 0x7fffffff ? (long long)stop + span + 16 : nlast + span + 16;
+        int x_hi = x_lo, g_hi = 0;
         unsigned rounds = 0;
         while (!relay_ld(&sh_done)) {
             if (++rounds > (1u << 24)) { if (lane == 0) a.stat[2] = 0xc0000000u | (unsigned)s; break; }
             const int pii = relay_ld(&sh_pos_ii);
             const bool fx = x_hi + RELAY_XCH - RX <= pii && (long long)x_hi <= xend && (long long)x_hi <= nlast + span + 16;
-            if (!fx) { __builtin_amdgcn_s_sleep(4); continue; }
-            cf32 vx[RELAY_XCH / 64];
+            bool fg = false;
+            if (GUIDED && use_rec) fg = g_hi < n_end && g_hi + RELAY_GCH - RELAY_GR <= relay_ld(&sh_pos_n);
+            if (!fx && !fg) { __builtin_amdgcn_s_sleep(4); continue; }
+            if (fx) {
+                cf32 vx[RELAY_XCH / 64];
 #pragma unroll
-            for (int q = 0; q < RELAY_XCH / 64; ++q) {
-                const long long i = (long long)x_hi + lane + 64 * q;
-                vx[q] = xs[i < nlast ? i : nlast];
-            }
+                for (int q = 0; q < RELAY_XCH / 64; ++q) {
+                    const long long i = (long long)x_hi + lane + 64 * q;
+                    vx[q] = xs[i < nlast ? i : nlast];
+                }
 #pragma unroll
-            for (int q = 0; q < RELAY_XCH / 64; ++q) {
-                const int slot = (x_hi + lane + 64 * q) & (RX - 1);
-                xr[slot] = vx[q];
-                if (slot < RELAY_XMIR) xr[RX + slot] = vx[q];
-            }
-            x_hi += RELAY_XCH;
-            if (lane == 0) relay_st(&sh_xhi, x_hi);
+                for (int q = 0; q < RELAY_XCH / 64; ++q) {
+                    const int slot = (x_hi + lane + 64 * q) & (RX - 1);
+                    xr[slot] = vx[q];
+                    if (slot < RELAY_XMIR) xr[RX + slot] = vx[q];
+                }
+                x_hi += RELAY_XCH;
+                if (lane == 0) relay_st(&sh_xhi, x_hi);
+            }
+            if (GUIDED && fg) {
+                unsigned vg[RELAY_GCH / 64];
+#pragma unroll
+                for (int q = 0; q < RELAY_GCH / 64; ++q) {
+                    const int e = e0s + g_hi + lane + 64 * q;
+                    vg[q] = e >= 0 && e < n_rec ? recs_in[e] : RELAY_NOPOS;
+                }
+                const int k = clock_ov_block_anchor(e0, g_hi).k + lane;
+                int va = -16;
+                if (lane < RELAY_GCH / OV_ANCHOR && k >= 0 && k < n_anch) va = anch_in[k];
+#pragma unroll
+                for (int q = 0; q < RELAY_GCH / 64; ++q) gr[(g_hi + lane + 64 * q) & (RELAY_GR - 1)] = vg[q];
+                if (lane < RELAY_GCH / OV_ANCHOR) ga[k & (NGA - 1)] = va;
+                g_hi += RELAY_GCH;
+                if (lane == 0) relay_st(&sh_ghi, g_hi);
+            }
         }
         return;
     }
@@ -125,22 +206,39 @@
     const int stride = __builtin_amdgcn_readfirstlane(a.stride);
     float *stage = a.stage + (size_t)s * (size_t)stride;
     OverlapSeg *seg = a.segs + s;
-    int n_st = 0;
     unsigned steps = 0, rounds_total = 0;
-    bool exhausted = false, stuck = false;
-    int x_hi = x_lo;
-    float m1 = 0.f, m2 = 0.f;
+    int x_hi = x_lo, g_hi = 0;
+    int n = 0;
+    float rec_slope = 0.0f;
+    const int rcap = PHASE == 1 ? (s < a.G ? a.rec_stride : a.guide_cap) : 0;
+    unsigned *recs_out = PHASE == 1 ? a.rec + (size_t)s * (size_t)a.rec_stride : nullptr;
+    int *anch_out = PHASE == 1 ? a.anchor + (size_t)s * (size_t)a.rec_stride / OV_ANCHOR : nullptr;
+    const bool rec_wrong = __builtin_amdgcn_readfirstlane(a.guide) == 2;
+    unsigned long long m1 = 0ull, m2 = 0ull;
 #ifdef XRIT_RELAY_TIMING
     unsigned long long tacc[6] = {0, 0, 0, 0, 0, 0}, tlast = __builtin_amdgcn_s_memtime();
     unsigned n_refresh = 0, n_spin = 0;
 #endif
     for (;;) {
         RELAY_TICK(5);
+        if (exhausted || stuck) break;
         const int ii0 = (int)T.ii;
         if ((unsigned)ii0 >= (unsigned)ni_w) { exhausted = true; break; }
-        if (ii0 >= hi) break;
+        if (ii0 >= stop) break;
         ++steps;
         const int need_x = ii0 + span + 8;
+        const bool ask = GUIDED && use_rec && n + 64 <= n_end;
+        if (GUIDED && ask && g_hi < n + 64) {
+            int spins = 0;
+#pragma nounroll
+            while (g_hi < n + 64) {
+                g_hi = relay_ld(&sh_ghi);
+                if (g_hi >= n + 64) break;
+                __builtin_amdgcn_s_sleep(2);
+                if (++spins > (1 << 22)) { if (lane == 0) a.stat[2] = 0x90000000u | (unsigned)s; stuck = true; break; }
+            }
+            if (stuck) break;
+        }
         if (x_hi < need_x) {
             int spins = 0;
 #ifdef XRIT_RELAY_TIMING
@@ -166,6 +264,25 @@
         float cmu = (float)(fr0 & 0xffffff) * (1.0f / 16777216.0f), com = T.omega;
         if (lane == 0) cmu = T.mu;
         carm = (int)rintf(cmu * (float)XR_MM_NSTEPS);
+        int rinc = 0;
+        bool rec_block = false;
+        if (GUIDED && ask) {
+            const unsigned g = gr[(n + lane) & (RELAY_GR - 1)];
+            rec_block = !__any(g == RELAY_NOPOS);
+            if (rec_block) {
+                rinc = relay_scan((int)g, lane);
+                const int frg = mu0u + lane * wfrac_n + (rinc - (int)g) + (int)rintf(rec_slope * (float)lane);
+                const int gii = ii0 + lane * wint_n + (frg >> 24);
+                const ClockOvBlockAnchor b = clock_ov_block_anchor(e0, n);
+                const int anc = __builtin_amdgcn_readfirstlane(ga[b.k & (NGA - 1)]);
+                rec_block = clock_ov_lines_up(__builtin_amdgcn_readlane(gii, __builtin_amdgcn_readfirstlane(b.lane)), anc);
+                if (rec_block && lane != 0) {
+                    cii = gii;
+                    carm = ((frg & 0xffffff) + (1 << 16)) >> 17;
+                }
+            }
+            if (!rec_block) rec_slope = 0.0f;
+        }
         cf32 p0{0.f, 0.f};
         float mm = 0.f;
         ClockState hs{};
@@ -208,7 +325,7 @@
         const bool exists = (unsigned)cii < (unsigned)ni_w;
         const bool good = !stale && inrange;
         const bool ok = good && exists && lane < 63 && (int)st.ii == nxt_ii && st.mu == nxt_mu && st.omega == nxt_om;
-        const unsigned long long okm = __ballot(ok), exm = __ballot(exists), gdm = __ballot(good), him = __ballot(cii >= hi),
+        const unsigned long long okm = __ballot(ok), exm = __ballot(exists), gdm = __ballot(good), him = __ballot(cii >= stop),
                                  lom = __ballot(cii >= lo);
         const int m = ~okm ? __builtin_ctzll(~okm) : 64;
         const int e = ~exm ? __builtin_ctzll(~exm) : 64;
@@ -225,10 +342,16 @@
                 const int o = n_st + lane - l0;
                 if (o < stride) stage[o] = p0.x;
                 if (o < OV_HEAD) { seg->head_ii[o] = cii; seg->head_mu[o] = cmu; }
-                m1 += fabsf(p0.x);
-                m2 += p0.x * p0.x;
+                m1 += (unsigned long long)(unsigned)fminf(fabsf(p0.x) * 1048576.0f, 4.0e9f);
+                m2 += (unsigned long long)(unsigned)fminf(p0.x * p0.x * 1048576.0f, 4.0e9f);
             }
             if (l0 < nv) n_st += nv - l0;
+            if (PHASE == 1 && lane < nv && n + lane < rcap) {
+                const int o = n + lane;
+                const int dev = ((int)st.ii - cii - wint_n) * 16777216 + ((int)(st.mu * 16777216.0f) - (int)(cmu * 16777216.0f)) - wfrac_n;
+                recs_out[o] = rec_wrong ? (1u << 22) : ((unsigned)dev != RELAY_NOPOS ? (unsigned)dev : 0u);
+                if ((o & (OV_ANCHOR - 1)) == 0) anch_out[o / OV_ANCHOR] = cii;
+            }
             const int src = nv - 1;
             ClockState nt;
             nt.ii = __builtin_amdgcn_readlane((int)st.ii, src);
@@ -236,18 +359,28 @@
             nt.omega = relay_lane(st.omega, src);
             nt.p0 = cf32{relay_lane(st.p0.x, src), relay_lane(st.p0.y, src)};
             nt.p1 = cf32{relay_lane(st.p1.x, src), relay_lane(st.p1.y, src)};
+            if (GUIDED && rec_block) {
+                const int act = ((int)nt.ii - ii0 - nv * wint_n) * 16777216 + ((int)(nt.mu * 16777216.0f) - mu0u) - nv * wfrac_n;
+                const float over = (float)(act - __builtin_amdgcn_readlane(rinc, src));
+                rec_slope = nv == 64 ? over * (1.0f / 64.0f) : over / (float)nv;
+                if (!(fabsf(rec_slope) <= (float)OV_GUIDE_SLOPE_MAX)) rec_slope = 0.0f;
+            }
             T = nt;
-            if (lane == 0) relay_st(&sh_pos_ii, (int)T.ii);
+            n += nv;
+            if (lane == 0) {
+                relay_st(&sh_pos_ii, (int)T.ii);
+                if (GUIDED) relay_st(&sh_pos_n, n);
+            }
         }
         RELAY_TICK(4);
         if (exhausted || nv == 0) { exhausted = true; break; }
     }
 #ifdef XRIT_RELAY_TIMING
     if (lane == 0) {
-        for (int q = 0; q < 6; ++q) atomicAdd(&relay_dbg[q], tacc[q]);
-        atomicAdd(&relay_dbg[6], (unsigned long long)steps);
-        atomicAdd(&relay_dbg[7], (unsigned long long)n_refresh);
-        atomicAdd(&relay_dbg[8], (unsigned long long)n_spin);
+        const int o = PHASE == 2 ? 8 : 0;
+        for (int q = 0; q < 6; ++q) atomicAdd(&relay_dbg[o + q], tacc[q]);
+        atomicAdd(&relay_dbg[o + 6], (unsigned long long)steps);
+        (void)n_refresh; (void)n_spin;
     }
 #endif
     for (int off = 32; off > 0; off >>= 1) { m1 += __shfl_xor(m1, off, 64); m2 += __shfl_xor(m2, off, 64); }
@@ -256,14 +389,25 @@
         if (claim && sh_claim >= 0) atomicAnd(claim, ~(1u << sh_claim));
         atomicAdd(&a.stat[0], steps);
         atomicAdd(&a.stat[1], rounds_total);
-        atomicAdd(&a.stat[3], 1u);
-        atomicAdd(&a.moments[0], (unsigned long long)((double)m1 * 1048576.0));
-        atomicAdd(&a.moments[1], (unsigned long long)((double)m2 * 1048576.0));
+        if (PHASE != 0) { atomicAdd(&a.stat[PHASE == 1 ? 4 : 6], steps); atomicAdd(&a.stat[PHASE == 1 ? 5 : 7], rounds_total); }
+        if (PHASE != 2 && !guide_only) atomicAdd(&a.stat[3], 1u);
+        if (m1) atomicAdd(&a.moments[0], m1);
+        if (m2) atomicAdd(&a.moments[1], m2);
         T.c0 = cf32{T.p0.x > 0.f ? 1.f : 0.f, T.p0.y > 0.f ? 1.f : 0.f};
         T.c1 = cf32{T.p1.x > 0.f ? 1.f : 0.f, T.p1.y > 0.f ? 1.f : 0.f};
-        seg->end = T;
-        seg->count = n_st < stride ? n_st : stride;
-        seg->flags = (stuck ? OV_STUCK : 0) | (exhausted && !stuck ? OV_EXHAUSTED : 0) | (n_st > stride ? OV_STUCK : 0);
+        const int flags = (stuck ? OV_STUCK : 0) | (exhausted && !stuck ? OV_EXHAUSTED : 0);
+        if (PHASE == 1) {
+            OverlapHand h{};
+            h.T = T;
+            h.n_st = n_st;
+            h.flags = flags;
+            h.n_rec = n < rcap ? n : rcap;
+            a.hand[s] = h;
+        } else {
+            seg->end = T;
+            seg->count = n_st < stride ? n_st : stride;
+            seg->flags = flags | (n_st > stride ? OV_STUCK : 0);
+        }
     }
 }
 
@@ -272,21 +416,22 @@
                                            const float *__restrict__ table, long long ni, int padN, int hist, int G,
                                            int store0, int first_bound, int Ls, const ClockState *__restrict__ carried,
                                            int w0_carried, int w0_ii, int valid_lo, ClockState *__restrict__ S,
-                                           unsigned *__restrict__ stat, unsigned long long *__restrict__ moments)
+                                           unsigned *__restrict__ stat, unsigned long long *__restrict__ moments,
+                                           int n_guide, int guide_bound)
 {
     const int s = blockIdx.x * blockDim.x + threadIdx.x;
     if (blockIdx.x == 0) {
         if (threadIdx.x < 8) stat[threadIdx.x] = 0u;
         if (threadIdx.x < 2) moments[threadIdx.x] = 0ull;
     }
-    if (s >= G) return;
+    if (s >= G + n_guide) return;
     if (s == 0 && w0_carried) {
         ClockState c = carried[0];
         c.ii = w0_ii;
         S[0] = c;
         return;
     }
-    const int bound = s == 0 ? store0 : first_bound + (s - 1) * Ls;
+    const int bound = s >= G ? guide_bound : (s == 0 ? store0 : first_bound + (s - 1) * Ls);
     double t = (double)bound - (double)hist;
     if (t < (double)valid_lo + 3.0 + 2.0 * sps) t = (double)valid_lo + 3.0 + 2.0 * sps;
     const bool prev = t < (double)padN && cnt_prev != nullptr && nb_prev > 0;
diff --git a/xritdemod_amd/csrc/clock_plan.h b/xritdemod_amd/csrc/clock_plan.h
--- a/xritdemod_amd/csrc/clock_plan.h
+++ b/xritdemod_amd/csrc/clock_plan.h
@@ -65,6 +65,7 @@
     int ov_min_walkers = 240;
     bool ov_small_ring = false;
     double ov_lratio = 1.0;
+    int ov_guide = 0;
 };
 
 inline size_t clock_tile_bytes(int WS, int ngroups, int threads)
@@ -290,6 +291,62 @@
     return j;
 }
 
+#if defined(__HIPCC__)
+#define XR_PLAN_HD __host__ __device__
+#else
+#define XR_PLAN_HD
+#endif
+constexpr int OV_ANCHOR = 64;
+constexpr int OV_NOALIGN = 0x7fffffff;
+constexpr int OV_GUIDE_SLOPE_MAX = 1 << 17;
+
+XR_PLAN_HD inline int clock_ov_phase_a_end(int hi, long long next_start_ii)
+{
+    return next_start_ii < (long long)hi ? (int)(next_start_ii < 0 ? 0 : next_start_ii) : hi;
+}
+inline int clock_ov_guide_bound(const ClockOvPlan &j) { return (int)(j.N < 0x7fffffffLL ? j.N : 0x7fffffffLL); }
+struct ClockOvGuide { int rec_stride = 0, guide_cap = 0, guide_span = 0; size_t entries = 0, anchors = 0; };
+inline ClockOvGuide clock_ov_guide_plan(const ClockKnobs &k, const ClockOvPlan &j)
+{
+    const double wmin = (double)k.par.omega_mid - (double)k.par.omega_lim;
+    ClockOvGuide g;
+    long long cap = (long long)ceil(((double)j.hist + 16.0) / wmin) + 128;
+    cap = (cap + OV_ANCHOR - 1) / OV_ANCHOR * OV_ANCHOR;
+    long long rs = ((long long)j.stride + 64 + OV_ANCHOR - 1) / OV_ANCHOR * OV_ANCHOR;
+    if (rs > cap) rs = cap;
+    g.rec_stride = (int)rs;
+    g.guide_cap = (int)cap;
+    g.guide_span = j.G >= 2 && j.Ls < j.hist ? j.Ls : j.hist;
+    g.entries = (size_t)j.G * (size_t)rs + (size_t)cap;
+    g.anchors = g.entries / OV_ANCHOR;
+    return g;
+}
+XR_PLAN_HD inline int clock_ov_align(const int *anchor, int n_rec, int ii, float omega_mid)
+{
+    if (n_rec <= 0) return OV_NOALIGN;
+    const int na = (n_rec + OV_ANCHOR - 1) / OV_ANCHOR;
+    int lo = 0, hi = na - 1;
+    while (lo < hi) {
+        const int mid = (lo + hi + 1) / 2;
+        if (anchor[mid] <= ii) lo = mid; else hi = mid - 1;
+    }
+    int k = lo;
+    if (k + 1 < na && (long long)anchor[k + 1] - (long long)ii < (long long)ii - (long long)anchor[k]) ++k;
+    const double d = ((double)ii - (double)anchor[k]) / (double)omega_mid;
+    if (!(d > -1.0e9 && d < 1.0e9)) return OV_NOALIGN;
+    return OV_ANCHOR * k + (int)(d < 0 ? -floor(0.5 - d) : floor(d + 0.5));
+}
+struct ClockOvBlockAnchor { int k, lane; };
+XR_PLAN_HD inline ClockOvBlockAnchor clock_ov_block_anchor(int e0, int n)
+{
+    ClockOvBlockAnchor b;
+    const int e = e0 + n + OV_ANCHOR - 1;
+    b.k = e >= 0 ? e / OV_ANCHOR : -((-e + OV_ANCHOR - 1) / OV_ANCHOR);
+    b.lane = OV_ANCHOR * b.k - e0 - n;
+    return b;
+}
+XR_PLAN_HD inline bool clock_ov_lines_up(int guess_ii, int anchor_ii) { return guess_ii - anchor_ii <= 1 && anchor_ii - guess_ii <= 1; }
+
 inline bool clock_handoff_to_closure(const ClockKnobs &k, const int *ctl, int K, bool relay)
 {
     if (!((k.exact == 0 || k.exact <= -2) && K > 1 && !relay)) return false;
diff --git a/xritdemod_amd/csrc/guide_host_check.cpp b/xritdemod_amd/csrc/guide_host_check.cpp
--- /dev/null
+++ b/xritdemod_amd/csrc/guide_host_check.cpp
@@ -0,0 +1,168 @@
+#include <stdio.h>
+
+#include <vector>
+
+#include "clock_plan.h"
+
+using namespace xrit;
+
+static int failures = 0;
+#define CHECK(c)                                                                  \
+    do {                                                                          \
+        if (!(c)) { fprintf(stderr, "guide_host_check:%d: %s\n", __LINE__, #c); ++failures; } \
+    } while (0)
+
+static ClockKnobs knobs(bool hrit)
+{
+    ClockKnobs k;
+    const float sps = hrit ? 2.5e6f / 927000.0f : 1.25e6f / 293883.0f;
+    k.sps = sps;
+    k.par.omega_mid = sps;
+    k.par.omega_lim = sps * 0.005f;
+    k.par.gain_omega = (0.0037f * 0.0037f) / 4.0f;
+    k.par.gain_mu = 0.0037f;
+    return k;
+}
+
+struct Walk {
+    std::vector<int> ii, anchor;
+    Walk(double t0, double period, int n)
+    {
+        for (int e = 0; e < n; ++e) ii.push_back((int)floor(t0 + e * period + 0.02 * sin(0.001 * e)));
+        for (int e = 0; e < n; e += OV_ANCHOR) anchor.push_back(ii[e]);
+    }
+};
+
+static void check_phase_a_end()
+{
+    CHECK(clock_ov_phase_a_end(1000, 999) == 999);
+    CHECK(clock_ov_phase_a_end(1000, 1000) == 1000);
+    CHECK(clock_ov_phase_a_end(1000, 1001) == 1000);
+    CHECK(clock_ov_phase_a_end(1000, 0x7fffffffLL) == 1000);
+    CHECK(clock_ov_phase_a_end(0x7fffffff, 0x7fffffffLL) == 0x7fffffff);
+    CHECK(clock_ov_phase_a_end(0x7fffffff, 123456) == 123456);
+    CHECK(clock_ov_phase_a_end(1000, -5) == 0);
+    CHECK(clock_ov_phase_a_end(1000, 0) == 0);
+}
+
+static void check_plan(const ClockKnobs &k, size_t n, bool have_hist, const char *name)
+{
+    const ClockOvPlan j = clock_ov_plan(k, n, 19, have_hist, false);
+    CHECK(!j.err[0]);
+    const ClockOvGuide g = clock_ov_guide_plan(k, j);
+    const double wmin = (double)k.par.omega_mid - (double)k.par.omega_lim;
+    CHECK(g.rec_stride > 0 && g.rec_stride % OV_ANCHOR == 0 && g.guide_cap % OV_ANCHOR == 0 && g.rec_stride <= g.guide_cap);
+    CHECK(g.entries == (size_t)j.G * (size_t)g.rec_stride + (size_t)g.guide_cap && g.anchors * OV_ANCHOR == g.entries);
+    CHECK((double)g.guide_cap >= ((double)j.hist + 2.0 * k.par.omega_mid) / wmin);
+    CHECK(g.guide_span > 0 && g.guide_span <= j.hist && (j.G < 2 || g.guide_span <= j.Ls));
+    CHECK(g.guide_span == j.hist || (j.G >= 2 && g.guide_span == j.Ls && j.Ls < j.hist));
+    const double phase_a = (double)j.Ls / wmin + 8.0;
+    CHECK((double)g.rec_stride >= phase_a || g.rec_stride == g.guide_cap);
+    const int gb = clock_ov_guide_bound(j);
+    CHECK(gb == (int)j.N);
+    const long long last_bound = j.G >= 2 ? (long long)j.first_bound + (long long)(j.G - 2) * j.Ls : (long long)j.store0;
+    CHECK((long long)gb > last_bound);
+    const long long last_start = last_bound - j.hist, guide_start = (long long)gb - j.hist;
+    CHECK(guide_start > last_start);
+    if (guide_start > 0) CHECK(clock_ov_phase_a_end(0x7fffffff, guide_start) == (int)guide_start);
+    for (int s = 0; s + 1 < j.G; ++s) {
+        const long long hi = (long long)j.first_bound + (long long)s * j.Ls;
+        const long long own = s == 0 ? (j.w0_carried ? 0 : (long long)j.store0 - j.hist) : hi - j.Ls - j.hist;
+        const long long next = hi - j.hist;
+        CHECK(next > own && next < hi);
+        CHECK(clock_ov_phase_a_end((int)hi, next < 0 ? 0 : next) == (int)(next < 0 ? 0 : next));
+    }
+    if (j.w0_carried) CHECK(j.first_bound - j.hist >= 0);
+    printf("%s: %d walkers, %d record entries each, %d for the guide-only walker, %.1f MB of records\n", name, j.G, g.rec_stride,
+           g.guide_cap, (double)g.entries * 4.0 / 1048576.0);
+}
+
+static void check_plans()
+{
+    const size_t burst = (size_t)1 << 28;
+    const ClockKnobs lrit = knobs(false), hrit = knobs(true);
+    for (int warm = 0; warm < 2; ++warm) {
+        check_plan(lrit, burst / 5, warm != 0, warm ? "C2" : "C2 from the carried state");
+        check_plan(lrit, burst / 32, warm != 0, warm ? "C5" : "C5 from the carried state");
+        check_plan(lrit, burst, warm != 0, warm ? "C1" : "C1 from the carried state");
+        check_plan(hrit, burst, warm != 0, warm ? "C3" : "C3 from the carried state");
+        check_plan(lrit, (size_t)1 << 23, warm != 0, "the test shape, LRIT");
+        check_plan(hrit, (size_t)1 << 23, warm != 0, "the test shape, HRIT");
+    }
+    {
+        const ClockOvPlan c2 = clock_ov_plan(lrit, burst / 5, 19, true, false), c1 = clock_ov_plan(lrit, burst, 19, true, false);
+        const ClockOvGuide g2 = clock_ov_guide_plan(lrit, c2), g1 = clock_ov_guide_plan(lrit, c1);
+        CHECK(g2.entries * 4 > (size_t)40 << 20 && g2.entries * 4 < (size_t)64 << 20);
+        CHECK(g1.rec_stride == g1.guide_cap && (double)g1.rec_stride < 1.02 * 49152 + 256);
+        const ClockOvPlan c5 = clock_ov_plan(lrit, burst / 32, 19, true, false);
+        CHECK(g2.guide_span == c2.hist && g1.guide_span == c1.hist);
+        CHECK(clock_ov_guide_plan(lrit, c5).guide_span == c5.Ls && c5.Ls < c5.hist / 5);
+    }
+    {
+        const ClockOvPlan j = clock_ov_plan(lrit, 100000, 19, false, false);
+        CHECK(!j.err[0] && j.G == 1 && j.w0_carried && (long long)clock_ov_guide_bound(j) - j.hist < 0);
+        const ClockOvGuide g = clock_ov_guide_plan(lrit, j);
+        CHECK(g.rec_stride > 0 && g.rec_stride <= g.guide_cap && g.entries == (size_t)g.rec_stride + (size_t)g.guide_cap);
+        CHECK(clock_ov_phase_a_end(0x7fffffff, 11) == 11);
+    }
+}
+
+static void check_align()
+{
+    const float om = 1.25e6f / 293883.0f;
+    const Walk w(5000.3, om, 1000);
+    const int n_rec = (int)w.ii.size();
+    const int *an = w.anchor.data();
+    CHECK(clock_ov_align(an, 0, 5000, om) == OV_NOALIGN);
+    CHECK(clock_ov_align(nullptr, 0, 5000, om) == OV_NOALIGN);
+    CHECK(clock_ov_align(an, -3, 5000, om) == OV_NOALIGN);
+    for (int e = 0; e < n_rec; ++e)
+        for (int d = -1; d <= 1; ++d) CHECK(clock_ov_align(an, n_rec, w.ii[e] + d, om) == e);
+    for (int n : {1, 63, 64, 65, 127, 128, 129, 999})
+        for (int e = 0; e < n; ++e) CHECK(clock_ov_align(an, n, w.ii[e], om) == e);
+    for (int e = 30; e <= 34; ++e) CHECK(clock_ov_align(an, n_rec, w.ii[e], om) == e);
+    CHECK(clock_ov_align(an, n_rec, w.ii[0] + 2, om) == 0 && clock_ov_align(an, n_rec, w.ii[0] + 3, om) == 1);
+    CHECK(clock_ov_align(an, n_rec, w.ii[0] - 2, om) == 0 && clock_ov_align(an, n_rec, w.ii[0] - 3, om) == -1);
+    {
+        const Walk o(5000.3 + 0.04, om, 1000), o2(5000.3 - 0.04, om, 1000);
+        for (int e = 0; e < n_rec; ++e) CHECK(clock_ov_align(an, n_rec, o.ii[e], om) == e && clock_ov_align(an, n_rec, o2.ii[e], om) == e);
+    }
+    CHECK(clock_ov_align(an, n_rec, w.ii[0] - (int)(10 * om + 0.5f), om) == -10);
+    CHECK(clock_ov_align(an, n_rec, 0, om) < -1000);
+    CHECK(clock_ov_align(an, n_rec, w.ii[n_rec - 1] + (int)(20 * om + 0.5f), om) == n_rec + 19);
+    CHECK(clock_ov_align(an, n_rec, 0x7fffffff, om) >= n_rec);
+    const float omh = 2.5e6f / 927000.0f;
+    const Walk h(77.9, omh, 300), h1(77.9 + 0.04, omh, 300), h2(77.9 - 0.04, omh, 300);
+    for (int e = 0; e < 300; ++e) {
+        CHECK(clock_ov_align(h.anchor.data(), 300, h.ii[e], omh) == e);
+        CHECK(clock_ov_align(h.anchor.data(), 300, h1.ii[e], omh) == e && clock_ov_align(h.anchor.data(), 300, h2.ii[e], omh) == e);
+    }
+}
+
+static void check_blocks()
+{
+    for (int e0 = -200; e0 <= 200; ++e0)
+        for (int n = 0; n <= 300; n += 7) {
+            const ClockOvBlockAnchor b = clock_ov_block_anchor(e0, n);
+            CHECK(b.lane >= 0 && b.lane < OV_ANCHOR);
+            CHECK(OV_ANCHOR * b.k == e0 + n + b.lane);
+        }
+    for (int e0 : {-65, -64, -1, 0, 1, 63, 64}) {
+        const int k = clock_ov_block_anchor(e0, 256).k;
+        CHECK(OV_ANCHOR * k >= e0 + 256 && OV_ANCHOR * (k + 3) < e0 + 512);
+    }
+    CHECK(clock_ov_lines_up(100, 100) && clock_ov_lines_up(100, 101) && clock_ov_lines_up(101, 100));
+    CHECK(!clock_ov_lines_up(100, 102) && !clock_ov_lines_up(102, 100) && !clock_ov_lines_up(100, -16));
+    CHECK(!clock_ov_lines_up(1000, 1000 + (int)(1.25e6f / 293883.0f)) && !clock_ov_lines_up(1000 + (int)(2.5e6f / 927000.0f), 1000));
+}
+
+int main()
+{
+    check_phase_a_end();
+    check_plans();
+    check_align();
+    check_blocks();
+    if (failures) { fprintf(stderr, "guide_host_check: %d checks failed\n", failures); return 1; }
+    printf("guide_host_check: phase A ends, the guide-only walker, record sizes, alignment and block anchors: ok\n");
+    return 0;
+}
diff --git a/xritdemod_amd/csrc/kernels.h b/xritdemod_amd/csrc/kernels.h
--- a/xritdemod_amd/csrc/kernels.h
+++ b/xritdemod_amd/csrc/kernels.h
@@ -204,6 +204,7 @@
     } job;
     struct OvJob {
         DevBuf om, om_work, segs, S, stage, aux;
+        DevBuf rec, anchor, hand;
         hipEvent_t ev_walk = nullptr;
         hipEvent_t ev_guess = nullptr;
     } ov[NXB];
```

Result: slower. 151,500 (-1.9%).
